# lukifer23/Matrix0

Hardware: AMD Instinct MI355X
Metric: self-play games/sec at 800 sims/move, ResNet-24 53M; 1/2/4/8 MI355X (higher is better)
Workload: dtype f16

## Files before the change

include/m0_engine.h:

```cpp
#ifndef M0_ENGINE_H
#define M0_ENGINE_H

#include <stdint.h>

#ifdef __cplusplus
extern "C" {
#endif

#define M0_OK 0
#define M0_ERR_INVALID (-1)
#define M0_ERR_UNSUPPORTED (-2)
#define M0_ERR_HIP (-3)
#define M0_ERR_STATE (-4)
#define M0_ERR_NONFINITE (-5)

#define M0_POLICY_SIZE 4672
#define M0_PLANES 19

#define M0_ACT_RELU 1
#define M0_ACT_SILU 2
#define M0_ACT_LEAKY 3

#define M0_SSL_PIECE 1
#define M0_SSL_THREAT 2
#define M0_SSL_PIN 4
#define M0_SSL_FORK 8
#define M0_SSL_CONTROL 16

typedef struct m0_net_cfg {
    int planes;
    int channels;
    int blocks;
    int attention;
    int attention_heads;
    int attention_every_k;
    int attention_relbias;
    float attention_unmasked_mix;
    int se;
    float se_ratio;
    int chess_features;
    int piece_square_tables;
    int policy_factor_rank;
    int norm_group;
    int activation;
    int value_activation;
    int preact;
    int self_supervised;
    int ssl_tasks;
    int infer_attention_stride;
} m0_net_cfg;

typedef struct m0_net m0_net;

const char* m0_last_error(void);
const char* m0_version(void);
int m0_device_count(void);

m0_net* m0_net_create(const m0_net_cfg* cfg, int hip_device);
void m0_net_destroy(m0_net* net);
int m0_net_load_weight(m0_net* net, const char* name, const void* data, int dtype, const int64_t* shape, int ndim);
int m0_net_finalize(m0_net* net);
int m0_net_infer(m0_net* net, const float* planes, int B, float* policy, float* value, float* ssl);
int m0_net_ssl_channels(const m0_net* net);
int64_t m0_net_param_count(const m0_net* net);
double m0_net_flops_per_position(const m0_net* net, int with_ssl);
int m0_net_bench_forward(m0_net* net, int B, int iters, int with_ssl, float* ms_per_forward);
int m0_net_profile_enable(m0_net* net, int on);
int m0_net_profile_get(m0_net* net, double* conv_ms, double* conv_flop, int64_t* launches, int reset);
int m0_net_profile_get_tail(m0_net* net, double* tail_ms, int64_t* tail_launches);


typedef struct m0_dist m0_dist;
int m0_dist_unique_id(void* id128);
m0_dist* m0_dist_create(int rank, int world, const void* id128, int hip_device);
void m0_dist_destroy(m0_dist* d);
int m0_dist_rank(const m0_dist* d);
int m0_dist_world(const m0_dist* d);
int m0_net_broadcast_weights(m0_net* net, m0_dist* d, int root);

int m0_encode_fens(int hip_device, const char* const* fens, int n, float* planes, uint8_t* mask, int32_t* nlegal,
                   uint16_t* moves, int32_t* idx);
int m0_encode_fens_nhwc(int hip_device, const char* const* fens, int n, uint16_t* nhwc);
int m0_decode_move_fen(int hip_device, const char* fen, int action_idx, char* uci_out);
int m0_ssl_targets_fens(int hip_device, const char* const* fens, int n, float* out);
int m0_move_to_index_fen(int hip_device, const char* fen, const char* uci, int32_t* idx);

typedef struct m0_selfplay_cfg {
    int num_simulations;
    double cpuct, cpuct_start, cpuct_end;
    int cpuct_plies;
    int use_c_base; double cpuct_c_base, cpuct_c_init;
    double dirichlet_alpha, dirichlet_frac;
    int dirichlet_plies;
    double selection_jitter, fpu_reduction, draw_penalty, virtual_loss;
    int legal_softmax, enable_entropy_noise, no_instant_backtrack, value_from_white;
    int inference_batch_size;
    double playout_random_frac;
    int max_game_len, min_resign_plies, opening_random_plies;
    double resign_threshold; int resign_window, resign_consecutive_bad; double resign_min_entropy, resign_value_margin;
    double temperature_start, temperature_end; int temperature_moves;
    int low_visit_threshold;
    int draw_enabled, draw_min_plies, draw_window, draw_min_unique, draw_halfmove_cap, draw_material_threshold, draw_stalemate;
    int concurrent_games;
    int total_games;
    int first_game_index;
    int arena_nodes;
    uint64_t seed;
    int virtual_loss_active;
    int ssl_in_forward;
    int ssl_targets;
    int record_games;
    int arena_mode;
    double arena_temp;
    int arena_temp_plies;
    int fresh_tree_per_move;
    int tt_merge;
    int raw_legal_priors;
    int max_children;
    double min_child_prior;
    int root_reinfer;
    int eval_cache;
    int eval_cache_entries;
    int tail_split;
} m0_selfplay_cfg;

typedef struct m0_selfplay m0_selfplay;

typedef struct m0_selfplay_stats {
    uint64_t steps, evals, sims, plies, games_finished, games_started;
    double ms_total, ms_net, ms_tree, ms_host;
    uint64_t arena_overflows;
    uint64_t ssl_dropped;
    uint64_t evals_cached;
    int active_games;
    uint64_t rows_tail;
} m0_selfplay_stats;

typedef struct m0_game_record {
    int game_index, moves, resigned, resigner , draw, total_plies ;
    float result;
    float avg_policy_entropy, avg_sims;
    double secs;
    const float* s;
    const float* pi;
    const float* z;
    const uint8_t* legal_mask;
    const float* search_values;
    const uint16_t* played;
    const float* ssl;
    void* owner;
} m0_game_record;

m0_selfplay* m0_selfplay_create(m0_net* net, const m0_selfplay_cfg* cfg);
void m0_selfplay_destroy(m0_selfplay* sp);
int m0_selfplay_step(m0_selfplay* sp, int steps);
int m0_selfplay_stats_get(m0_selfplay* sp, m0_selfplay_stats* out);
int m0_selfplay_poll(m0_selfplay* sp, m0_game_record* out);
void m0_game_record_free(m0_game_record* rec);
int m0_selfplay_running(m0_selfplay* sp);
int m0_selfplay_set_openings(m0_selfplay* sp, const char* const* fens, int n);
int m0_selfplay_ext_select(m0_selfplay* sp, int* rows, float* planes, int max_rows);
int m0_selfplay_ext_expand(m0_selfplay* sp, const float* logits, const float* values, int rows);
int m0_selfplay_last_batch_nhwc(m0_selfplay* sp, uint16_t* nhwc, int max_rows, int* rows);

m0_selfplay* m0_arena_create(m0_net* net_a, m0_net* net_b, const m0_selfplay_cfg* cfg);
m0_selfplay* m0_arena_create_ext(const m0_selfplay_cfg* cfg);
int m0_arena_ext_select(m0_selfplay* sp, int* rows_a, int* rows_b, float* planes_a, float* planes_b, int max_rows);
int m0_arena_ext_expand(m0_selfplay* sp, const float* logits_a, const float* values_a, int rows_a, const float* logits_b,
                        const float* values_b, int rows_b);
int m0_arena_choose_move(const int32_t* visits, int n, double temp, int ply, int temp_plies, double u);
int m0_san_legal_fen(const char* fen, uint16_t* moves, char* san, int* nlegal);
int m0_san_game(const uint16_t* moves, int n, char* out, int cap);
int m0_fen_after(const char* fen, const char* const* ucis, int n, char* fen_out, int cap);

int m0_search_begin(m0_selfplay* sp, int g, const char* fen, int sims, int dirichlet, int game_uid);
int m0_search_select(m0_selfplay* sp, int* rows, float* planes, int max_rows);
int m0_search_expand(m0_selfplay* sp, const float* logits, const float* values, int rows);
int m0_search_result(m0_selfplay* sp, int g, int* nchild, int32_t* child_n, uint16_t* child_mv, int32_t* child_idx,
                     double* child_prior, double* child_q, double* root_q, int* root_n, int* finished);
int m0_search_advance(m0_selfplay* sp, int g, int slot, int sims, int dirichlet);

int m0_sample_move_index(const int32_t* visits, int n, double temperature, double u);
int m0_playout_cap(int sims, double frac, double u);
double m0_temperature_for(int fullmove_number, double t_start, double t_end, int t_moves);
int m0_rules_probe(const m0_selfplay_cfg* cfg, const char* fen, const char* const* ucis, int n, int* flags, float* result);

#ifdef __cplusplus
}
#endif
#endif
```

matrix0_amd/csrc/capi_selfplay.hip:

```cpp
#include <string.h>
#include <algorithm>
#include <memory>
#include "selfplay_engine.h"

using namespace m0;

static void fill_tree_cfg(const m0_selfplay_cfg& c, TreeCfg& t) {
    t.fpu_reduction = c.fpu_reduction; t.draw_penalty = c.draw_penalty; t.virtual_loss = c.virtual_loss;
    t.selection_jitter = c.selection_jitter; t.cpuct = c.cpuct; t.cpuct_start = c.cpuct_start; t.cpuct_end = c.cpuct_end;
    t.cpuct_plies = c.cpuct_plies; t.use_c_base = c.use_c_base; t.cpuct_c_base = c.cpuct_c_base; t.cpuct_c_init = c.cpuct_c_init;
    t.dirichlet_alpha = c.dirichlet_alpha; t.dirichlet_frac = c.dirichlet_frac; t.legal_softmax = c.legal_softmax;
    t.enable_entropy_noise = c.enable_entropy_noise; t.no_instant_backtrack = c.no_instant_backtrack;
    t.virtual_loss_active = c.virtual_loss_active; t.leaves_per_step = c.inference_batch_size;
    t.tt_merge = c.tt_merge; t.raw_legal_priors = c.raw_legal_priors; t.max_children = c.max_children;
    t.min_child_prior = c.min_child_prior;
    t.eval_cache = (c.eval_cache && c.legal_softmax && !c.raw_legal_priors && !c.tt_merge) ? 1 : 0;
}

static void alloc_tree_arenas(m0_selfplay* sp) {
    const m0_selfplay_cfg& c = sp->cfg;
    long want = c.arena_nodes > 0 ? c.arena_nodes : (long)(c.num_simulations * 1.3 + 64) * 96;
    if (want < 4096) want = 4096;
    sp->cap = (int)want;
    const size_t N = (size_t)sp->G * 2 * sp->cap;
    TreeArrays& t = sp->d.t;
    t.cap = sp->cap;
    t.prior = dalloc<double>(sp, N); t.w = dalloc<double>(sp, N); t.q = dalloc<double>(sp, N);
    t.n = dalloc<int>(sp, N); t.vl = dalloc<int>(sp, N); t.cbase = dalloc<int>(sp, N);
    t.nch = dalloc<int16_t>(sp, N); t.mv = dalloc<uint16_t>(sp, N); t.midx = dalloc<uint16_t>(sp, N);
    sp->d.games = dalloc<GameDev>(sp, sp->G);
    const size_t LS = (size_t)sp->L + 1;
    sp->d.samples = dalloc<Sample>(sp, (size_t)sp->G * LS);
    sp->d.paths = dalloc<int>(sp, (size_t)sp->G * LS * M0_MAX_DEPTH);
    sp->d.leaf_moves = dalloc<uint16_t>(sp, (size_t)sp->G * LS * M0_MAX_CHILDREN);
}

static bool alloc_position_tables(m0_selfplay* sp) {
    sp->d.tt_sides = 1;
    if (!sp->cfg.tt_merge) return true;
    const size_t LS = (size_t)sp->L + 1;
    int tc = 1024;
    while (tc < 2 * sp->cap) tc <<= 1;
    sp->d.tt_cap = tc;
    sp->d.tt_sides = sp->cfg.arena_mode ? 2 : 1;
    sp->d.search_nodes = (int)std::min<long>((long)sp->cfg.num_simulations * 48 + 4 * M0_MAX_CHILDREN, (long)sp->cap / 2);
    sp->d.epaths = dalloc<int>(sp, (size_t)sp->G * LS * M0_MAX_DEPTH);
    sp->d.tt_keys = dalloc<uint64_t>(sp, (size_t)sp->G * sp->d.tt_sides * tc);
    sp->d.tt_nodes = dalloc<int>(sp, (size_t)sp->G * sp->d.tt_sides * tc);
    if (sp->d.epaths && sp->d.tt_keys && sp->d.tt_nodes) return true;
    m0_set_error("hipMalloc failed for the position tables (tt_merge): lower concurrent_games or arena_nodes");
    return false;
}

static bool alloc_eval_cache(m0_selfplay* sp) {
    if (!sp->tc.eval_cache) return true;
    const size_t LS = (size_t)sp->L + 1;
    int entries = sp->cfg.eval_cache_entries > 0 ? sp->cfg.eval_cache_entries : 16384;
    int sets = 64;
    while (sets * 4 < entries) sets <<= 1;
    EvalCache& ec = sp->d.ec;
    ec.sets = sets;
    ec.keys = dalloc<uint64_t>(sp, (size_t)sp->G * sets * 4);
    ec.stamps = dalloc<uint32_t>(sp, (size_t)sp->G * sets * 4);
    ec.payload = dalloc<float>(sp, (size_t)sp->G * sets * 4 * M0_EC_WORDS);
    ec.hit_stage = dalloc<float>(sp, (size_t)sp->G * LS * M0_EC_WORDS);
    if (ec.keys && ec.stamps && ec.payload && ec.hit_stage) return true;
    m0_set_error("hipMalloc failed for the evaluation cache: lower eval_cache_entries or concurrent_games");
    return false;
}

static bool alloc_batch_buffers(m0_selfplay* sp) {
    const int nreg = sp->cfg.arena_mode ? 2 : 1;
    sp->d.hist = dalloc<uint64_t>(sp, (size_t)sp->G * M0_HIST_CAP);
    sp->d.results = dalloc<RootResult>(sp, sp->G);
    sp->d.row_counter = dalloc<int>(sp, 4);
    sp->d.x0 = dalloc<_Float16>(sp, (size_t)(nreg * sp->rows_max + 4) * 64 * 32);
    sp->logits_dev = dalloc<float>(sp, (size_t)nreg * sp->rows_max * 4672);
    sp->values_dev = dalloc<float>(sp, (size_t)nreg * sp->rows_max + 4);
    sp->d.net_row_base = sp->rows_max;
    if (sp->cfg.ssl_in_forward && sp->net && sp->net->ssl_channels_total() > 0)
        sp->ssl_dev = dalloc<float>(sp, (size_t)sp->rows_max * sp->net->ssl_channels_total() * 64);
    if (sp->cfg.ssl_targets) {
        sp->ssl_cap = sp->cfg.max_game_len > 0 ? sp->cfg.max_game_len + 1 : 513;
        sp->ssl_pos_dev = dalloc<Pos>(sp, sp->ssl_cap);
        sp->ssl_out_dev = dalloc<float>(sp, (size_t)sp->ssl_cap * 17 * 64);
        if (!sp->ssl_pos_dev || !sp->ssl_out_dev) {
            m0_set_error("hipMalloc failed for the SSL target staging buffers");
            return false;
        }
    }
    sp->ids_dev = dalloc<int>(sp, sp->G);
    sp->slots_dev = dalloc<int>(sp, sp->G);
    sp->d.logits = sp->logits_dev; sp->d.values = sp->values_dev;
    sp->d.G = sp->G; sp->d.L = sp->L;
    return true;
}

static bool make_tail_view(m0_selfplay* sp) {
    if (!(sp->cfg.tail_split && sp->net && !sp->cfg.arena_mode && sp->net->cfg().channels > 256 && sp->net->cfg().channels <= 320 &&
          sp->rows_max >= 2048)) return true;
    if (create_stream_cu_mask_env("M0_TAIL_CU_MASK", &sp->stream_tail) != hipSuccess ||
        hipEventCreateWithFlags(&sp->ev_sel, hipEventDisableTiming) != hipSuccess ||
        hipEventCreateWithFlags(&sp->ev_tail, hipEventDisableTiming) != hipSuccess) {
        m0_set_error("hipStreamCreate / hipEventCreate failed (tail split)");
        return false;
    }
    sp->net_tail = sp->net->shared_view(sp->stream_tail);
    std::string werr;
    sp->half_split = sp->cfg.tail_split == 2;
    if (sp->net_tail->ensure_workspace(sp->half_split ? sp->rows_max / 2 + 1024 : 1023, werr) != M0_OK) {
        m0_set_error("tail split: " + werr);
        return false;
    }
    return true;
}

static bool build_engine(m0_selfplay* sp) {
    alloc_tree_arenas(sp);
    if (!alloc_position_tables(sp) || !alloc_eval_cache(sp) || !alloc_batch_buffers(sp)) return false;
    if (sp->alloc_failed) {
        m0_set_error("hipMalloc failed for the search arenas (lower concurrent_games or arena_nodes)");
        return false;
    }
    sp->hg.assign(sp->G, GameDev());
    for (auto& g : sp->hg) memset(&g, 0, sizeof(GameDev));
    sp->games.assign(sp->G, HostGame());
    sp->hres.resize(sp->G);
    sp->hsamples.resize((size_t)sp->G * (sp->L + 1));
    sp->prev_done.assign(sp->G, 0);
    (void)hipEventCreate(&sp->ev0); (void)hipEventCreate(&sp->ev1); (void)hipEventCreate(&sp->ev2); (void)hipEventCreate(&sp->ev3);
    if (!make_tail_view(sp)) return false;
    std::string err;
    if (sp->net && sp->net->ensure_workspace(sp->rows_max, err) != M0_OK) { m0_set_error(err); return false; }
    if (sp->net && sp->net_b && sp->net_b->ensure_workspace(sp->rows_max, err) != M0_OK) { m0_set_error(err); return false; }
    if (hipStreamSynchronize(sp->stream) != hipSuccess) {
        m0_set_error(std::string("clearing the search arenas failed: ") + hipGetErrorString(hipGetLastError()));
        return false;
    }
    return true;
}

extern "C" {

static m0_selfplay* selfplay_create_impl(m0_net* nh, m0_net* nh_b, const m0_selfplay_cfg* cfg, bool arena = false) {
    if (!cfg) { m0_set_error("cfg is null"); return nullptr; }
    if (cfg->concurrent_games <= 0 || cfg->inference_batch_size <= 0 || cfg->num_simulations <= 0) {
        m0_set_error("concurrent_games, inference_batch_size and num_simulations must be positive");
        return nullptr;
    }
    int ndev = 0;
    if (hipGetDeviceCount(&ndev) != hipSuccess || ndev <= 0) { m0_set_error("no HIP device available (no CPU fallback)"); return nullptr; }
    std::unique_ptr<m0_selfplay, decltype(&m0_selfplay_destroy)> owner(new m0_selfplay(), &m0_selfplay_destroy);
    m0_selfplay* sp = owner.get();
    sp->cfg = *cfg;
    fill_tree_cfg(*cfg, sp->tc);
    sp->nethandle = nh;
    sp->nethandle_b = nh_b;
    sp->net = m0_net_impl(nh);
    sp->net_b = m0_net_impl(nh_b);
    sp->cfg.arena_mode = (nh_b || arena) ? 1 : 0;
    if (sp->cfg.arena_mode) { sp->cfg.eval_cache = 0; sp->tc.eval_cache = 0; }
    sp->device = nh ? m0_net_device(nh) : 0;
    if (nh) forward_gate_join(sp);
    (void)hipSetDevice(sp->device);
    if (nh) sp->stream = m0_net_stream(nh);
    else { (void)hipStreamCreateWithFlags(&sp->stream, hipStreamNonBlocking); sp->own_stream = true; }
    sp->G = cfg->concurrent_games;
    sp->L = cfg->inference_batch_size;
    sp->rows_max = (sp->G * (sp->L + 1) + 3) & ~3;
    memset(&sp->stats, 0, sizeof(sp->stats));
    memset(&sp->d, 0, sizeof(sp->d));
    return build_engine(sp) ? owner.release() : nullptr;
}

m0_selfplay* m0_selfplay_create(m0_net* nh, const m0_selfplay_cfg* cfg) { return selfplay_create_impl(nh, nullptr, cfg); }

m0_selfplay* m0_arena_create(m0_net* net_a, m0_net* net_b, const m0_selfplay_cfg* cfg) {
    if (!net_a || !net_b) { m0_set_error("m0_arena_create needs two networks"); return nullptr; }
    if (m0_net_device(net_a) != m0_net_device(net_b)) { m0_set_error("both networks must live on the same HIP device"); return nullptr; }
    if (cfg && (cfg->ssl_in_forward || cfg->ssl_targets)) { m0_set_error("arena games carry no SSL outputs"); return nullptr; }
    return selfplay_create_impl(net_a, net_b, cfg);
}

m0_selfplay* m0_arena_create_ext(const m0_selfplay_cfg* cfg) {
    if (cfg && (cfg->ssl_in_forward || cfg->ssl_targets)) { m0_set_error("arena games carry no SSL outputs"); return nullptr; }
    return selfplay_create_impl(nullptr, nullptr, cfg, true);
}

void m0_selfplay_destroy(m0_selfplay* sp) {
    if (!sp) return;
    forward_gate_leave(sp);
    (void)hipSetDevice(sp->device);
    if (sp->stream) (void)hipStreamSynchronize(sp->stream);
    if (sp->stream_tail) (void)hipStreamSynchronize(sp->stream_tail);
    delete sp->net_tail;
    if (sp->ev_sel) (void)hipEventDestroy(sp->ev_sel);
    if (sp->ev_tail) (void)hipEventDestroy(sp->ev_tail);
    if (sp->stream_tail) (void)hipStreamDestroy(sp->stream_tail);
    for (void* p : sp->allocs) (void)hipFree(p);
    for (auto& r : sp->done_meta) delete (GameRecordOwner*)r.owner;
    if (sp->ev0) { (void)hipEventDestroy(sp->ev0); (void)hipEventDestroy(sp->ev1); (void)hipEventDestroy(sp->ev2); (void)hipEventDestroy(sp->ev3); }
    if (sp->own_stream && sp->stream) (void)hipStreamDestroy(sp->stream);
    delete sp;
}

int m0_selfplay_set_openings(m0_selfplay* sp, const char* const* fens, int n) {
    if (!sp || n < 0 || (n > 0 && !fens)) { m0_set_error("invalid argument"); return M0_ERR_INVALID; }
    std::lock_guard<std::mutex> lk(sp->mu);
    if (sp->stats.games_started != 0) { m0_set_error("set the opening book before the first step"); return M0_ERR_STATE; }
    std::vector<Pos> book(n);
    for (int i = 0; i < n; ++i)
        if (!fens[i] || parse_fen(fens[i], book[i]) != 0) { m0_set_error(std::string("bad FEN at index ") + std::to_string(i)); return M0_ERR_INVALID; }
    sp->book.swap(book);
    return M0_OK;
}

static int leaf_planes(m0_selfplay* sp, int rows_a, float* planes_a, int rows_b, float* planes_b) {
    if (sync_games_d2h(sp) != 0) { m0_set_error("device sync failed"); return M0_ERR_HIP; }
    (void)hipMemcpy(sp->hsamples.data(), sp->d.samples, sizeof(Sample) * (size_t)sp->G * (sp->L + 1), hipMemcpyDeviceToHost);
    const int base = sp->d.net_row_base;
    for (int g = 0; g < sp->G; ++g) {
        if (!sp->hg[g].active) continue;
        for (int s = 0; s < sp->hg[g].nsamples; ++s) {
            const Sample& smp = sp->hsamples[(size_t)g * (sp->L + 1) + s];
            if (!sample_owns_row(smp.kind) || smp.row < 0) continue;
            if (smp.row < rows_a) encode_planes_f32(smp.pos, planes_a + (size_t)smp.row * 19 * 64);
            else if (smp.row >= base && smp.row < base + rows_b) encode_planes_f32(smp.pos, planes_b + (size_t)(smp.row - base) * 19 * 64);
        }
    }
    return M0_OK;
}

static void upload_eval(m0_selfplay* sp, size_t row_base, const float* logits, const float* values, int rows) {
    if (rows <= 0) return;
    (void)hipMemcpyAsync(sp->logits_dev + row_base * 4672, logits, (size_t)rows * 4672 * 4, hipMemcpyHostToDevice, sp->stream);
    (void)hipMemcpyAsync(sp->values_dev + row_base, values, (size_t)rows * 4, hipMemcpyHostToDevice, sp->stream);
}

static int ext_select_impl(m0_selfplay* sp, int* rows_a, int* rows_b, float* planes_a, float* planes_b, int max_rows) {
    (void)hipSetDevice(sp->device);
    if (sp->ext_pending) { m0_set_error("m0_selfplay_ext_expand outstanding"); return M0_ERR_STATE; }
    if (!planes_a || (sp->cfg.arena_mode && !planes_b) || max_rows < sp->G * (sp->L + 1)) {
        m0_set_error("planes buffer too small: concurrent_games * (inference_batch_size + 1) rows are required");
        return M0_ERR_INVALID;
    }
    int rc = start_first_games(sp);
    if (rc != M0_OK) return rc;
    int r = 0;
    if (run_select(sp, &r) != 0) { m0_set_error(std::string("select failed: ") + hipGetErrorString(hipGetLastError())); return M0_ERR_HIP; }
    const int rb = sp->cfg.arena_mode ? sp->rows2[1] : 0;
    if (r > sp->rows_max || rb > sp->rows_max) { m0_set_error("row counter overflow"); return M0_ERR_STATE; }
    *rows_a = r;
    if (rows_b) *rows_b = rb;
    sp->last_rows = r;
    sp->last_rows_b = rb;
    sp->ext_pending = true;
    if (r + rb > 0) return leaf_planes(sp, r, planes_a, rb, planes_b);
    return M0_OK;
}

static int ext_expand_impl(m0_selfplay* sp, const float* logits_a, const float* values_a, int rows_a, const float* logits_b,
                           const float* values_b, int rows_b) {
    (void)hipSetDevice(sp->device);
    if (!sp->ext_pending) { m0_set_error("no m0_selfplay_ext_select outstanding"); return M0_ERR_STATE; }
    if (rows_a != sp->last_rows || rows_b != sp->last_rows_b) { m0_set_error("rows does not match the last select"); return M0_ERR_INVALID; }
    if ((rows_a > 0 && (!logits_a || !values_a)) || (rows_b > 0 && (!logits_b || !values_b))) { m0_set_error("null argument"); return M0_ERR_INVALID; }
    upload_eval(sp, 0, logits_a, values_a, rows_a);
    upload_eval(sp, (size_t)sp->d.net_row_base, logits_b, values_b, rows_b);
    sp->ext_pending = false;
    std::string err;
    (void)hipEventRecord(sp->ev0, sp->stream); (void)hipEventRecord(sp->ev1, sp->stream);
    int rc = step_back(sp, rows_a + rows_b, now_ms(), err);
    if (rc != M0_OK) m0_set_error(err);
    return rc;
}

int m0_selfplay_ext_select(m0_selfplay* sp, int* rows, float* planes, int max_rows) {
    if (!sp || !rows) { m0_set_error("null argument"); return M0_ERR_INVALID; }
    std::lock_guard<std::mutex> lk(sp->mu);
    if (sp->cfg.arena_mode) { m0_set_error("a match engine has two evaluators: use m0_arena_ext_select"); return M0_ERR_STATE; }
    return ext_select_impl(sp, rows, nullptr, planes, nullptr, max_rows);
}

int m0_selfplay_ext_expand(m0_selfplay* sp, const float* logits, const float* values, int rows) {
    if (!sp) { m0_set_error("null argument"); return M0_ERR_INVALID; }
    std::lock_guard<std::mutex> lk(sp->mu);
    if (sp->cfg.arena_mode) { m0_set_error("a match engine has two evaluators: use m0_arena_ext_expand"); return M0_ERR_STATE; }
    return ext_expand_impl(sp, logits, values, rows, nullptr, nullptr, 0);
}

int m0_arena_ext_select(m0_selfplay* sp, int* rows_a, int* rows_b, float* planes_a, float* planes_b, int max_rows) {
    if (!sp || !rows_a || !rows_b) { m0_set_error("null argument"); return M0_ERR_INVALID; }
    std::lock_guard<std::mutex> lk(sp->mu);
    if (!sp->cfg.arena_mode) { m0_set_error("not a match engine"); return M0_ERR_STATE; }
    return ext_select_impl(sp, rows_a, rows_b, planes_a, planes_b, max_rows);
}

int m0_arena_ext_expand(m0_selfplay* sp, const float* logits_a, const float* values_a, int rows_a, const float* logits_b,
                        const float* values_b, int rows_b) {
    if (!sp) { m0_set_error("null argument"); return M0_ERR_INVALID; }
    std::lock_guard<std::mutex> lk(sp->mu);
    if (!sp->cfg.arena_mode) { m0_set_error("not a match engine"); return M0_ERR_STATE; }
    return ext_expand_impl(sp, logits_a, values_a, rows_a, logits_b, values_b, rows_b);
}

int m0_selfplay_step(m0_selfplay* sp, int steps) {
    if (!sp) { m0_set_error("sp is null"); return M0_ERR_INVALID; }
    std::lock_guard<std::mutex> lk(sp->mu);
    (void)hipSetDevice(sp->device);
    std::string err;
    if (sp->ext_pending) { m0_set_error("m0_selfplay_ext_expand outstanding"); return M0_ERR_STATE; }
    { int rc0 = start_first_games(sp); if (rc0 != M0_OK) return rc0; }
    for (int i = 0; i < steps; ++i) {
        if (sp->stats.active_games == 0 && sp->stats.steps > 0) break;
        int rc = one_step(sp, err);
        if (rc != M0_OK) { m0_set_error(err); return rc; }
    }
    return M0_OK;
}

int m0_selfplay_stats_get(m0_selfplay* sp, m0_selfplay_stats* out) {
    if (!sp || !out) { m0_set_error("null argument"); return M0_ERR_INVALID; }
    std::lock_guard<std::mutex> lk(sp->mu);
    *out = sp->stats;
    return M0_OK;
}

int m0_selfplay_poll(m0_selfplay* sp, m0_game_record* out) {
    if (!sp || !out) { m0_set_error("null argument"); return M0_ERR_INVALID; }
    std::lock_guard<std::mutex> lk(sp->mu);
    if (sp->done_meta.empty()) return 0;
    *out = sp->done_meta.front();
    sp->done_meta.pop_front();
    return 1;
}

void m0_game_record_free(m0_game_record* rec) {
    if (rec && rec->owner) { delete (GameRecordOwner*)rec->owner; rec->owner = nullptr; }
}

int m0_selfplay_running(m0_selfplay* sp) {
    if (!sp) return 0;
    std::lock_guard<std::mutex> lk(sp->mu);
    if (sp->stats.games_started == 0) return 1;
    if (sp->stats.active_games > 0) return 1;
    return (sp->cfg.total_games <= 0 || sp->next_game < sp->cfg.total_games) ? 1 : 0;
}

int m0_search_begin(m0_selfplay* sp, int g, const char* fen, int sims, int dirichlet, int game_uid) {
    if (!sp || !fen || g < 0 || g >= sp->G || sims <= 0) { m0_set_error("invalid argument"); return M0_ERR_INVALID; }
    std::lock_guard<std::mutex> lk(sp->mu);
    (void)hipSetDevice(sp->device);
    Pos p;
    if (parse_fen(fen, p) != 0) { m0_set_error("bad FEN"); return M0_ERR_INVALID; }
    if (sync_games_d2h(sp) != 0) { m0_set_error("device sync failed"); return M0_ERR_HIP; }
    HostGame& hgm = sp->games[g];
    hgm = HostGame();
    hgm.in_use = true; hgm.pos = p; hgm.game_index = game_uid;
    seed_game_dev(sp->hg[g], sp->cfg.seed, game_uid);
    sp->hg[g].evals = 0;
    arm_search(sp, g, p, hgm.win, sims, dirichlet != 0, true);
    std::vector<int> ids{g}, slots{-1};
    if (apply_advances(sp, ids, slots) != 0) { m0_set_error("advance failed"); return M0_ERR_HIP; }
    return M0_OK;
}

int m0_search_select(m0_selfplay* sp, int* rows, float* planes, int max_rows) {
    if (!sp || !rows) { m0_set_error("null argument"); return M0_ERR_INVALID; }
    std::lock_guard<std::mutex> lk(sp->mu);
    (void)hipSetDevice(sp->device);
    int r = 0;
    if (run_select(sp, &r) != 0) { m0_set_error(std::string("select failed: ") + hipGetErrorString(hipGetLastError())); return M0_ERR_HIP; }
    *rows = r;
    sp->last_rows = r;
    if (planes && r > 0) {
        if (r > max_rows) { m0_set_error("planes buffer too small"); return M0_ERR_INVALID; }
        return leaf_planes(sp, r, planes, 0, nullptr);
    }
    return M0_OK;
}

int m0_search_expand(m0_selfplay* sp, const float* logits, const float* values, int rows) {
    if (!sp) { m0_set_error("null argument"); return M0_ERR_INVALID; }
    std::lock_guard<std::mutex> lk(sp->mu);
    (void)hipSetDevice(sp->device);
    if (rows != sp->last_rows || rows > sp->rows_max) { m0_set_error("rows does not match the last select"); return M0_ERR_INVALID; }
    if (rows > 0 && (!logits || !values)) { m0_set_error("null argument"); return M0_ERR_INVALID; }
    upload_eval(sp, 0, logits, values, rows);
    if (launch_expand(sp->d, sp->tc, sp->stream) != hipSuccess) { m0_set_error("expand launch failed"); return M0_ERR_HIP; }
    if (sync_games_d2h(sp) != 0) { m0_set_error(std::string("expand failed: ") + hipGetErrorString(hipGetLastError())); return M0_ERR_HIP; }
    sp->stats.evals += (uint64_t)rows;
    return M0_OK;
}

int m0_search_result(m0_selfplay* sp, int g, int* nchild, int32_t* child_n, uint16_t* child_mv, int32_t* child_idx,
                     double* child_prior, double* child_q, double* root_q, int* root_n, int* finished) {
    if (!sp || g < 0 || g >= sp->G) { m0_set_error("invalid argument"); return M0_ERR_INVALID; }
    std::lock_guard<std::mutex> lk(sp->mu);
    (void)hipSetDevice(sp->device);
    if (finished) *finished = sp->hg[g].finished;
    if (!sp->hg[g].finished) { if (nchild) *nchild = 0; return M0_OK; }
    (void)hipMemcpy(&sp->hres[g], sp->d.results + g, sizeof(RootResult), hipMemcpyDeviceToHost);
    const RootResult& R = sp->hres[g];
    if (nchild) *nchild = R.nchild;
    for (int i = 0; i < R.nchild; ++i) {
        if (child_n) child_n[i] = R.child_n[i];
        if (child_mv) child_mv[i] = R.child_mv[i];
        if (child_idx) child_idx[i] = R.child_idx[i];
        if (child_prior) child_prior[i] = R.child_prior[i];
        if (child_q) child_q[i] = R.child_q[i];
    }
    if (root_q) *root_q = R.root_n > 0 ? R.root_q : sp->hg[g].root_v;
    if (root_n) *root_n = R.root_n;
    return M0_OK;
}

int m0_search_advance(m0_selfplay* sp, int g, int slot, int sims, int dirichlet) {
    if (!sp || g < 0 || g >= sp->G || sims <= 0) { m0_set_error("invalid argument"); return M0_ERR_INVALID; }
    std::lock_guard<std::mutex> lk(sp->mu);
    (void)hipSetDevice(sp->device);
    if (sync_games_d2h(sp) != 0) { m0_set_error("device sync failed"); return M0_ERR_HIP; }
    if (!sp->hg[g].finished) { m0_set_error("search not finished"); return M0_ERR_STATE; }
    (void)hipMemcpy(&sp->hres[g], sp->d.results + g, sizeof(RootResult), hipMemcpyDeviceToHost);
    const RootResult& R = sp->hres[g];
    if (slot < 0 || slot >= R.nchild) { m0_set_error("child slot out of range"); return M0_ERR_INVALID; }
    HostGame& hgm = sp->games[g];
    hgm.play(R.child_mv[slot]);
    const bool fresh = sp->cfg.fresh_tree_per_move || sp->cfg.tt_merge;
    arm_search(sp, g, hgm.pos, hgm.win, sims, dirichlet != 0, fresh);
    std::vector<int> ids{g}, slots{fresh ? -1 : slot};
    if (apply_advances(sp, ids, slots) != 0) { m0_set_error("advance failed"); return M0_ERR_HIP; }
    return M0_OK;
}

int m0_selfplay_last_batch_nhwc(m0_selfplay* sp, uint16_t* out, int max_rows, int* rows) {
    if (!sp || !out || !rows) { m0_set_error("null argument"); return M0_ERR_INVALID; }
    std::lock_guard<std::mutex> lk(sp->mu);
    (void)hipSetDevice(sp->device);
    const int r = sp->last_rows;
    if (r > max_rows) { m0_set_error("output buffer too small"); return M0_ERR_INVALID; }
    *rows = r;
    if (r > 0) {
        if (hipMemcpyAsync(out, sp->d.x0, (size_t)r * 64 * 32 * 2, hipMemcpyDeviceToHost, sp->stream) != hipSuccess ||
            hipStreamSynchronize(sp->stream) != hipSuccess) { m0_set_error("copy failed"); return M0_ERR_HIP; }
    }
    return M0_OK;
}

}
```

matrix0_amd/csrc/net.h:

```cpp
#pragma once
#include <hip/hip_runtime.h>
#include <stdint.h>
#include <map>
#include <string>
#include <vector>
#include "../../include/m0_engine.h"
#include "net_kernels.h"

struct HostTensor {
    std::vector<float> data;
    std::vector<int64_t> shape;
};

struct PackedGemm {
    _Float16* w = nullptr;
    float* bias = nullptr;
    int taps = 1, Cin = 0, N = 0;
    bool pp = false;
};

struct NormParams {
    float* gamma = nullptr;
    float* beta = nullptr;
};

struct ResBlockW {
    PackedGemm conv1, conv2;
    NormParams bn1, bn2;
    float *se_w1 = nullptr, *se_b1 = nullptr, *se_w2 = nullptr, *se_b2 = nullptr;
    void* se_wf = nullptr;
    int se_hidden = 0;
};

struct AttnW {
    PackedGemm qkv, proj;
    NormParams ln;
    float* rel_bias = nullptr;
    void* blk_w = nullptr;
    _Float16* blk_bias = nullptr;
};

struct TowerLayer {
    int kind;
    int index;
    bool skip;
    int next_bn1 = -1;
};

struct SslHeadW {
    PackedGemm c0, c1;
    NormParams n;
    int out_ch = 0;
};

struct ConvNormOpts {
    const float* posenc = nullptr;
    const _Float16* res = nullptr;
    const NormParams* next_bn1 = nullptr;
};

class Net {
public:
    explicit Net(const m0_net_cfg& cfg, int device, hipStream_t stream);
    ~Net();
    Net* shared_view(hipStream_t stream) const;
    static const char* check_supported(const m0_net_cfg& cfg);
    int load(const char* name, const void* data, int dtype, const int64_t* shape, int ndim, std::string& err);
    int finalize(std::string& err);
    bool ready() const { return finalized_; }
    const std::vector<void*>& device_buffers() const { return dev_allocs_; }
    const std::vector<size_t>& device_buffer_bytes() const { return dev_sizes_; }

    int forward(const float* planes_dev, const _Float16* nhwc_dev, int B, float* logits_dev, float* value_dev,
                float* ssl_dev, hipStream_t st, std::string& err);
    int ensure_workspace(int B, std::string& err);
    int ssl_channels_total() const;
    const m0_net_cfg& cfg() const { return cfg_; }
    size_t param_count() const { return nparams_; }
    double flops_per_position(bool with_ssl) const;
    _Float16* input_nhwc() { return X0_; }
    void set_profile(bool on) { profile_ = on; }
    void harvest_profile();
    double prof_conv_ms() const { return prof_ms_; }
    double prof_conv_flop() const { return prof_flop_; }
    long prof_conv_launches() const { return prof_launches_; }
    void reset_profile() { prof_ms_ = 0; prof_flop_ = 0; prof_launches_ = 0; prof_tail_ms_ = 0; prof_tail_launches_ = 0; }
    double prof_tail_ms() const { return prof_tail_ms_; }
    long prof_tail_launches() const { return prof_tail_launches_; }

private:
    m0_net_cfg cfg_;
    int device_;
    hipStream_t stream_ = nullptr;
    struct Switches { bool fuse_tail = true, fuse_attn = true; } sw_;
    struct Plan {
        bool fuse_tail = false;
        bool fuse_attn = false;
        bool gn_small = false;
        int act = 0, vact = 0;
        int first_bn1 = -1;
    } plan_;
    bool finalized_ = false;
    size_t nparams_ = 0;
    std::map<std::string, HostTensor> sd_;
    std::vector<void*> dev_allocs_;
    std::vector<size_t> dev_sizes_;
    std::vector<void*> ws_allocs_;

    int C_ = 0, Cs_ = 0 ;
    int Cp_ = 0;
    PackedGemm stem_;
    NormParams stem_n_;
    float* posenc_ = nullptr;
    PackedGemm pst_, inter_;
    NormParams pst_n_, inter_n_;
    std::vector<ResBlockW> res_;
    std::vector<AttnW> att_;
    std::vector<TowerLayer> tower_;
    PackedGemm ph_conv_, pfc1_, pfc2_;
    PackedGemm hv_;
    NormParams hv_n_;
    NormParams ph_n_;
    float logit_scale_ = 1.f;
    PackedGemm vh0_, vh3_, vfc1_, vfc2_, vgate_, vfc3_;
    NormParams vh1_n_, vh4_n_;
    std::vector<SslHeadW> ssl_;
    uint64_t* mask_dev_ = nullptr;

    bool profile_ = false;
    std::vector<hipEvent_t> pev_;
    std::vector<double> pflop_;
    std::vector<char> ptail_;
    size_t pev_used_ = 0;
    double prof_ms_ = 0, prof_flop_ = 0, prof_tail_ms_ = 0;
    long prof_launches_ = 0, prof_tail_launches_ = 0;

    int wsB_ = 0, wsM_ = 0;
    _Float16 *X0_ = nullptr, *XA_ = nullptr, *XB_ = nullptr, *T1_ = nullptr, *T2_ = nullptr, *QKV_ = nullptr,
             *O_ = nullptr, *AA_ = nullptr;
    float *S1_ = nullptr, *S2_ = nullptr, *G_ = nullptr;
    _Float16 *PH_ = nullptr, *PH2_ = nullptr, *VH_ = nullptr, *VH2_ = nullptr, *F1_ = nullptr, *F2_ = nullptr,
             *F3_ = nullptr, *F4_ = nullptr, *SH_ = nullptr, *SH2_ = nullptr, *SO_ = nullptr;
    float* VAL_ = nullptr;
    float* SPK_ = nullptr;

    const HostTensor* get(const std::string& k, std::string& err);
    int pack_gemm(PackedGemm& g, const std::string& wkey, const std::string& bkey, int taps, int Cin_real,
                  int Cin_pad, int N_real, int N_pad, int k_perm_ch, std::string& err, int qkv_heads = 0,
                  int qkv_heads_pad = 0);
    int pack_attn_block(AttnW& a, const std::string& prefix, std::string& err);
    int pack_chess_features(std::string& err);
    int pack_se(ResBlockW& r, const std::string& prefix, std::string& err);
    int pack_attn(AttnW& a, bool skip, const std::string& prefix, std::string& err);
    void upload_attn_mask();
    int pack_joint_head(std::string& err);
    int pack_ssl_heads(std::string& err);
    void make_plan();
    int upload_norm(NormParams& n, const std::string& prefix, int C_real, int C_pad, std::string& err);
    float* upload_f32(const std::vector<float>& v);
    void* dalloc(size_t bytes, bool ws);
    const NormParams* bn1(int res_index) const { return res_index < 0 ? nullptr : &res_[res_index].bn1; }
    template <class Launch>
    hipError_t profiled(bool on, hipStream_t st, double flop, bool tail, Launch&& launch);
    hipError_t run_gemm(const PackedGemm& g, GemmArgs a, hipStream_t st);
    hipError_t conv_norm_act(const PackedGemm& g, const NormParams& n, const _Float16* in, _Float16* out, _Float16* scratch,
                             int Mrows, hipStream_t st, const ConvNormOpts& o = ConvNormOpts());
    hipError_t se_gate(const ResBlockW& r, const float* stats, int boards, hipStream_t st);
};
```

matrix0_amd/csrc/net.hip:

```cpp
#include "net.h"
#include <math.h>
#include <string.h>
#include <algorithm>
#include <stdlib.h>

static inline int ceil_to(int v, int m) { return (v + m - 1) / m * m; }

static const char* kSslNames[5] = {"piece", "threat", "pin", "fork", "control"};
static const int kSslOut[5] = {13, 1, 1, 1, 3};

const char* Net::check_supported(const m0_net_cfg& c) {
    if (!c.norm_group) return "HIP path supports norm='group' only (BatchNorm configs are not built)";
    if (!c.preact) return "HIP path supports preact=true only";
    if (c.channels % 32 != 0 || c.channels < 32 || c.channels > 384) return "channels must be a multiple of 32 in [32,384]";
    if (c.planes < 1 || c.planes > 32) return "planes must be in [1,32]";
    if (c.attention && (c.attention_heads <= 0 || c.channels % c.attention_heads != 0 ||
                        c.channels / c.attention_heads != 16))
        return "attention head_dim (channels/attention_heads) must be 16";
    if (c.activation != M0_ACT_SILU && c.activation != M0_ACT_RELU) return "activation must be silu or relu";
    if (c.blocks < 1) return "blocks must be >= 1";
    if (c.policy_factor_rank < 0) return "policy_factor_rank must be >= 0";
    if (c.self_supervised && c.ssl_tasks && (c.channels / 2) % 16 != 0) return "ssl heads need channels/2 % 16 == 0";
    return nullptr;
}
// ... 171 lines not shown
    (void)hipMemcpy(a.blk_w, buf.data(), buf.size() * 2, hipMemcpyHostToDevice);
    std::vector<_Float16> bb((size_t)20 * 2 * 64 * 32, (_Float16)0.f);
    if (cfg_.attention_relbias) {
        const HostTensor* rb = get(prefix + ".rel_bias", err); if (!rb) return M0_ERR_INVALID;
        for (int h = 0; h < Hr; ++h)
            for (int qt = 0; qt < 2; ++qt)
                for (int lane = 0; lane < 64; ++lane)
                    for (int e = 0; e < 32; ++e) {
                        const int kt = e >> 4, r = e & 15;
                        const int q = qt * 32 + (lane & 31), key = kt * 32 + 8 * (r >> 2) + 4 * (lane >> 5) + (r & 3);
                        bb[(((size_t)h * 2 + qt) * 64 + lane) * 32 + e] =
                            (_Float16)(rb->data[((size_t)h * 64 + q) * 64 + key] * 1.44269504088896f);
                    }
    }
    a.blk_bias = (_Float16*)dalloc(bb.size() * 2, false);
    if (!a.blk_bias) { err = "hipMalloc failed"; return M0_ERR_HIP; }
    (void)hipMemcpy(a.blk_bias, bb.data(), bb.size() * 2, hipMemcpyHostToDevice);
    return M0_OK;
}

int Net::upload_norm(NormParams& n, const std::string& prefix, int C_real, int C_pad, std::string& err) {
    const HostTensor* g = get(prefix + ".weight", err);
    if (!g) return M0_ERR_INVALID;
    const HostTensor* b = get(prefix + ".bias", err);
    if (!b) return M0_ERR_INVALID;
    if ((int)g->data.size() != C_real || (int)b->data.size() != C_real) { err = "shape mismatch for " + prefix; return M0_ERR_INVALID; }
    nparams_ += 2 * (size_t)C_real;
    std::vector<float> gp(C_pad, 0.f), bp(C_pad, 0.f);
    std::copy(g->data.begin(), g->data.end(), gp.begin());
    std::copy(b->data.begin(), b->data.end(), bp.begin());
    n.gamma = upload_f32(gp);
    n.beta = upload_f32(bp);
    return M0_OK;
}

#define TRY(x) do { int rc_ = (x); if (rc_ != M0_OK) return rc_; } while (0)

int Net::pack_chess_features(std::string& err) {
    const int C = C_, P = Cp_;
    const HostTensor* pe = get("chess_features.position_encoding", err);
    if (!pe) return M0_ERR_INVALID;
    if ((int)pe->data.size() != C * 64) { err = "shape mismatch for position_encoding"; return M0_ERR_INVALID; }
    nparams_ += pe->data.size();
    std::vector<float> t((size_t)64 * P, 0.f);
    for (int c = 0; c < C; ++c)
        for (int n = 0; n < 64; ++n) t[(size_t)n * P + c] = pe->data[(size_t)c * 64 + n];
    posenc_ = upload_f32(t);
    if (cfg_.piece_square_tables) {
        TRY(pack_gemm(pst_, "chess_features.pst_conv.weight", "", 1, C, P, C, P, 0, err));
        TRY(upload_norm(pst_n_, "chess_features.pst_norm", C, P, err));
    }
    TRY(pack_gemm(inter_, "chess_features.interaction_conv.weight", "", 9, C, P, C, P, 0, err));
    return upload_norm(inter_n_, "chess_features.interaction_norm", C, P, err);
}

int Net::pack_se(ResBlockW& r, const std::string& p, std::string& err) {
    const int C = C_, P = Cp_;
    const int hd = std::max(8, (int)(C * cfg_.se_ratio));
    r.se_hidden = hd;
    const HostTensor* w1 = get(p + ".se_fc1.weight", err); if (!w1) return M0_ERR_INVALID;
    const HostTensor* b1 = get(p + ".se_fc1.bias", err); if (!b1) return M0_ERR_INVALID;
    const HostTensor* w2 = get(p + ".se_fc2.weight", err); if (!w2) return M0_ERR_INVALID;
    const HostTensor* b2 = get(p + ".se_fc2.bias", err); if (!b2) return M0_ERR_INVALID;
    if ((int)w1->data.size() != hd * C || (int)w2->data.size() != hd * C || (int)b1->data.size() != hd ||
        (int)b2->data.size() != C) { err = "shape mismatch for " + p + ".se_*"; return M0_ERR_INVALID; }
    nparams_ += (size_t)2 * hd * C + hd + C;
    std::vector<float> w1t((size_t)P * hd, 0.f);
    for (int j = 0; j < hd; ++j)
        for (int c = 0; c < C; ++c) w1t[(size_t)c * hd + j] = w1->data[(size_t)j * C + c];
    r.se_w1 = upload_f32(w1t);
    r.se_b1 = upload_f32(b1->data);
    std::vector<float> w2t((size_t)hd * P, 0.f);
    for (int c = 0; c < C; ++c)
        for (int j = 0; j < hd; ++j) w2t[(size_t)j * P + c] = w2->data[(size_t)c * hd + j];
    r.se_w2 = upload_f32(w2t);
    if (P == 320 && hd <= TAIL_SE_HMAX) {
        const int NT1 = (hd + 15) / 16, KS2 = (hd + 31) / 32;
        std::vector<_Float16> wf((size_t)(10 * NT1 + 20 * KS2) * 512, (_Float16)0.f);
        for (int nt = 0; nt < NT1; ++nt)
            for (int ks = 0; ks < 10; ++ks)
                for (int l = 0; l < 64; ++l)
                    for (int e = 0; e < 8; ++e) {
                        const int c = 32 * ks + 8 * (l >> 4) + e, j = 16 * nt + (l & 15);
                        if (j < hd) wf[((size_t)(nt * 10 + ks) * 64 + l) * 8 + e] = (_Float16)w1t[(size_t)c * hd + j];
                    }
        for (int nt = 0; nt < 20; ++nt)
            for (int ks = 0; ks < KS2; ++ks)
                for (int l = 0; l < 64; ++l)
                    for (int e = 0; e < 8; ++e) {
                        const int j = 32 * ks + 8 * (l >> 4) + e, c = 16 * nt + (l & 15);
                        if (j < hd) wf[((size_t)(10 * NT1 + nt * KS2 + ks) * 64 + l) * 8 + e] = (_Float16)w2t[(size_t)j * P + c];
                    }
        r.se_wf = dalloc(wf.size() * 2, false);
        if (!r.se_wf) { err = "hipMalloc failed"; return M0_ERR_HIP; }
        (void)hipMemcpy(r.se_wf, wf.data(), wf.size() * 2, hipMemcpyHostToDevice);
    }
    std::vector<float> b2p(P, 0.f);
    std::copy(b2->data.begin(), b2->data.end(), b2p.begin());
    r.se_b2 = upload_f32(b2p);
    return M0_OK;
}

int Net::pack_attn(AttnW& a, bool skip, const std::string& p, std::string& err) {
    const int C = C_, P = Cp_;
    if (skip) {
        for (const char* k : {".qkv.weight", ".proj.weight", ".norm.weight", ".norm.bias", ".rel_bias"}) {
            auto it = sd_.find(p + k);
            if (it != sd_.end()) nparams_ += it->second.data.size();
        }
        return M0_OK;
    }
    TRY(pack_gemm(a.qkv, p + ".qkv.weight", "", 1, C, P, 3 * C, 3 * P, 0, err, P != C ? cfg_.attention_heads : 0, P / 16));
    TRY(pack_gemm(a.proj, p + ".proj.weight", "", 1, C, P, C, P, 0, err));
    TRY(upload_norm(a.ln, p + ".norm", C, P, err));
    if (P == 320) TRY(pack_attn_block(a, p, err));
    if (cfg_.attention_relbias) {
        const HostTensor* rb = get(p + ".rel_bias", err); if (!rb) return M0_ERR_INVALID;
        if ((int)rb->data.size() != cfg_.attention_heads * 4096) { err = "shape mismatch for rel_bias"; return M0_ERR_INVALID; }
        nparams_ += rb->data.size();
        std::vector<float> rbs((size_t)(P / 16) * 4096, 0.f);
        for (size_t i = 0; i < rb->data.size(); ++i) rbs[i] = rb->data[i] * 1.44269504088896f;
        a.rel_bias = upload_f32(rbs);
    }
    return M0_OK;
}

void Net::upload_attn_mask() {
    std::vector<uint64_t> m(64, 0);
    for (int i = 0; i < 64; ++i)
        for (int j = 0; j < 64; ++j) {
            int dr = i / 8 - j / 8, dc = i % 8 - j % 8;
            int adr = abs(dr), adc = abs(dc);
            bool vis = dr == 0 || dc == 0 || adr == adc || (adr == 2 && adc == 1) || (adr == 1 && adc == 2) ||
                       (adr <= 1 && adc <= 1);
            if (vis) m[i] |= (1ull << j);
        }
    mask_dev_ = (uint64_t*)dalloc(64 * 8, false);
    (void)hipMemcpy(mask_dev_, m.data(), 64 * 8, hipMemcpyHostToDevice);
}

int Net::pack_joint_head(std::string& err) {
    const int nch = Cp_ / 32;
    std::vector<_Float16> a((size_t)nch * 64 * 32), b((size_t)nch * 128 * 32), c((size_t)nch * 192 * 32);
    (void)hipMemcpy(a.data(), ph_conv_.w, a.size() * 2, hipMemcpyDeviceToHost);
    (void)hipMemcpy(b.data(), vh0_.w, b.size() * 2, hipMemcpyDeviceToHost);
    for (int ch = 0; ch < nch; ++ch) {
        std::copy(a.begin() + (size_t)ch * 64 * 32, a.begin() + (size_t)(ch + 1) * 64 * 32, c.begin() + (size_t)ch * 192 * 32);
        std::copy(b.begin() + (size_t)ch * 128 * 32, b.begin() + (size_t)(ch + 1) * 128 * 32, c.begin() + ((size_t)ch * 192 + 64) * 32);
    }
    hv_.w = (_Float16*)dalloc(c.size() * 2, false);
    if (!hv_.w) { err = "hipMalloc failed"; return M0_ERR_HIP; }
    (void)hipMemcpy(hv_.w, c.data(), c.size() * 2, hipMemcpyHostToDevice);
    hv_.taps = 1; hv_.Cin = Cp_; hv_.N = 192; hv_.pp = false; hv_.bias = nullptr;
    std::vector<float> g(192), be(192);
    (void)hipMemcpy(g.data(), ph_n_.gamma, 64 * 4, hipMemcpyDeviceToHost);
    (void)hipMemcpy(g.data() + 64, vh1_n_.gamma, 128 * 4, hipMemcpyDeviceToHost);
    (void)hipMemcpy(be.data(), ph_n_.beta, 64 * 4, hipMemcpyDeviceToHost);
    (void)hipMemcpy(be.data() + 64, vh1_n_.beta, 128 * 4, hipMemcpyDeviceToHost);
    hv_n_.gamma = upload_f32(g); hv_n_.beta = upload_f32(be);
    if (!hv_n_.gamma || !hv_n_.beta) { err = "hipMalloc failed"; return M0_ERR_HIP; }
    return M0_OK;
}

int Net::pack_ssl_heads(std::string& err) {
    for (int t = 0; t < 5; ++t) {
        if (!(cfg_.ssl_tasks & (1 << t))) continue;
        SslHeadW h;
        h.out_ch = kSslOut[t];
        std::string p = std::string("ssl_heads.") + kSslNames[t];
        TRY(pack_gemm(h.c0, p + ".0.weight", "", 1, C_, Cp_, C_ / 2, Cs_, 0, err));
        TRY(upload_norm(h.n, p + ".1", C_ / 2, Cs_, err));
        TRY(pack_gemm(h.c1, p + ".3.weight", "", 1, C_ / 2, Cs_, h.out_ch, 32, 0, err));
        ssl_.push_back(h);
    }
    return M0_OK;
}

void Net::make_plan() {
    const bool big = conv_gemm_tile_n(Cp_, Cp_) == 320;
    plan_.fuse_tail = big && sw_.fuse_tail &&
                      (!cfg_.se || (res_[0].se_hidden <= TAIL_SE_HMAX && res_[0].se_hidden % 4 == 0));
    plan_.fuse_attn = big && sw_.fuse_attn;
    plan_.gn_small = Cp_ % 64 == 0;
    plan_.act = cfg_.activation == M0_ACT_SILU ? ACT_SILU : ACT_RELU;
    plan_.vact = cfg_.value_activation == M0_ACT_SILU ? ACT_SILU : (cfg_.value_activation == M0_ACT_LEAKY ? ACT_LEAKY : ACT_RELU);
    int next = -1;
    for (size_t i = tower_.size(); i-- > 0;) {
        TowerLayer& L = tower_[i];
        if (L.kind == 1 && L.skip) continue;
        L.next_bn1 = next;
        next = L.kind == 0 ? L.index : -1;
    }
    plan_.first_bn1 = next;
}

int Net::finalize(std::string& err) {
    if (finalized_) return M0_OK;
    if (hipSetDevice(device_) != hipSuccess) { err = "hipSetDevice failed"; return M0_ERR_HIP; }
    const int C = C_, P = Cp_;
    nparams_ = 0;
    TRY(pack_gemm(stem_, "stem.0.weight", "", 9, cfg_.planes, 32, C, P, 0, err));
    TRY(upload_norm(stem_n_, "stem.1", C, P, err));
    if (cfg_.chess_features) TRY(pack_chess_features(err));
    int ti = 0;
    for (auto& L : tower_) {
        std::string p = "tower." + std::to_string(ti++);
        if (L.kind == 0) {
            ResBlockW& r = res_[L.index];
            TRY(pack_gemm(r.conv1, p + ".conv1.weight", "", 9, C, P, C, P, 0, err));
            TRY(pack_gemm(r.conv2, p + ".conv2.weight", "", 9, C, P, C, P, 0, err));
            TRY(upload_norm(r.bn1, p + ".bn1", C, P, err));
            TRY(upload_norm(r.bn2, p + ".bn2", C, P, err));
            if (cfg_.se) TRY(pack_se(r, p, err));
        } else {
            TRY(pack_attn(att_[L.index], L.skip, p, err));
        }
    }
    upload_attn_mask();
    TRY(pack_gemm(ph_conv_, "policy_head.0.weight", "", 1, C, P, 64, 64, 0, err));
    TRY(upload_norm(ph_n_, "policy_head.1", 64, 64, err));
    if (cfg_.policy_factor_rank > 0) {
        int r = cfg_.policy_factor_rank, rp = ceil_to(r, 32);
        TRY(pack_gemm(pfc1_, "policy_fc1.weight", "policy_fc1.bias", 1, 4096, 4096, r, rp, 64, err));
        TRY(pack_gemm(pfc2_, "policy_fc2.weight", "policy_fc2.bias", 1, r, rp, M0_POLICY_SIZE, M0_POLICY_SIZE, 0, err));
    } else {
        TRY(pack_gemm(pfc1_, "policy_fc.weight", "policy_fc.bias", 1, 4096, 4096, M0_POLICY_SIZE, M0_POLICY_SIZE, 64, err));
    }
    {
        const HostTensor* ls = get("_policy_logit_scale_raw", err); if (!ls) return M0_ERR_INVALID;
        nparams_ += 1;
        double raw = ls->data.empty() ? 0.0 : ls->data[0];
        double sp = raw > 20.0 ? raw : log1p(exp(raw));
        logit_scale_ = (float)std::min(5.0, sp + 1e-3);
    }
    TRY(pack_gemm(vh0_, "value_head.0.weight", "", 1, C, P, 128, 128, 0, err));
    TRY(upload_norm(vh1_n_, "value_head.1", 128, 128, err));
    TRY(pack_gemm(vh3_, "value_head.3.weight", "", 1, 128, 128, 128, 128, 0, err));
    TRY(upload_norm(vh4_n_, "value_head.4", 128, 128, err));
    TRY(pack_joint_head(err));
    const int h1 = 2 * C, h1p = ceil_to(h1, 32), h2 = C, h2p = ceil_to(C, 32);
    TRY(pack_gemm(vfc1_, "value_fc1.weight", "value_fc1.bias", 1, 8192, 8192, h1, h1p, 128, err));
    TRY(pack_gemm(vfc2_, "value_fc2.weight", "value_fc2.bias", 1, h1, h1p, h2, h2p, 0, err));
    TRY(pack_gemm(vgate_, "value_gate.0.weight", "value_gate.0.bias", 1, h2, h2p, h2, h2p, 0, err));
    TRY(pack_gemm(vfc3_, "value_fc3.weight", "value_fc3.bias", 1, h2, h2p, 1, 32, 0, err));
    if (cfg_.self_supervised) TRY(pack_ssl_heads(err));
    sd_.clear();
    (void)hipDeviceSynchronize();
    make_plan();
    finalized_ = true;
    return M0_OK;
}

int Net::ssl_channels_total() const {
    int n = 0;
    for (auto& h : ssl_) n += h.out_ch;
    return n;
}

double Net::flops_per_position(bool with_ssl) const {
    const double C = C_;
    double mac = 64.0 * cfg_.planes * 9 * C;
    if (cfg_.chess_features) mac += 64.0 * C * C * (cfg_.piece_square_tables ? 1 : 0) + 64.0 * C * C * 9;
    for (auto& L : tower_) {
        if (L.kind == 0) {
            mac += 2 * 64.0 * C * C * 9;
            if (cfg_.se) mac += 2.0 * C * res_[L.index].se_hidden;
        } else if (!L.skip) {
            mac += 64.0 * C * 3 * C + 64.0 * C * C;
            double nb = (cfg_.attention_unmasked_mix > 0.f && cfg_.attention_unmasked_mix < 1.f) ? 2.0 : 1.0;
            mac += 64.0 * 64.0 * C * (1.0 + nb);
        }
    }
    mac += 64.0 * C * 64;
    if (cfg_.policy_factor_rank > 0) mac += 4096.0 * cfg_.policy_factor_rank + (double)cfg_.policy_factor_rank * M0_POLICY_SIZE;
    else mac += 4096.0 * M0_POLICY_SIZE;
    mac += 64.0 * C * 128 + 64.0 * 128 * 128 + 8192.0 * 2 * C + 2.0 * C * C + C * C + C;
    if (with_ssl) for (auto& h : ssl_) mac += 64.0 * C * (C / 2) + 64.0 * (C / 2) * h.out_ch;
    return 2.0 * mac;
}

int Net::ensure_workspace(int B, std::string& err) {
    const int Bp = ceil_to(B, 4);
    const int Mfc = ceil_to(B, 256);
    if (Bp <= wsB_ && Mfc <= wsM_) return M0_OK;
    if (hipSetDevice(device_) != hipSuccess) { err = "hipSetDevice failed"; return M0_ERR_HIP; }
    (void)hipDeviceSynchronize();
    for (void* p : ws_allocs_) (void)hipFree(p);
    ws_allocs_.clear();
    const size_t C = Cp_;
    const size_t nb = Bp, nh = std::max(Bp, Mfc);
    const size_t Cst = std::max<size_t>(C, 128);
    auto H = [&](size_t elems) { return (_Float16*)dalloc(elems * 2, true); };
    auto F = [&](size_t elems) { return (float*)dalloc(elems * 4, true); };
    X0_ = H(nb * 64 * 32);
    XA_ = H(nb * 64 * C); XB_ = H(nb * 64 * C); T1_ = H(nb * 64 * C); T2_ = H(nb * 64 * C); AA_ = H(nb * 64 * C);
    QKV_ = H(nb * 64 * 3 * C); O_ = H(nb * 64 * C);
    S1_ = F(nb * Cst * 2); S2_ = F(nb * Cst * 2); G_ = F(nb * Cst);
    PH_ = H(nh * 64 * 64); PH2_ = H(nh * 64 * 64);
    VH_ = H(nh * 64 * 128); VH2_ = H(nh * 64 * 128);
    const size_t rp = cfg_.policy_factor_rank > 0 ? ceil_to(cfg_.policy_factor_rank, 32) : 32;
    F1_ = H((size_t)Mfc * rp);
    F2_ = H((size_t)Mfc * ceil_to(2 * C_, 32)); F3_ = H((size_t)Mfc * ceil_to(C_, 32)); F4_ = H((size_t)Mfc * ceil_to(C_, 32));
    SH_ = H(nb * 64 * Cs_); SH2_ = H(nb * 64 * Cs_); SO_ = H(nb * 64 * 32);
    VAL_ = F((size_t)Mfc * 32);
    SPK_ = F((size_t)8 * Mfc * ceil_to(2 * C_, 32));
    if (!X0_ || !XA_ || !XB_ || !AA_ || !T1_ || !T2_ || !QKV_ || !O_ || !S1_ || !S2_ || !PH_ || !PH2_ || !VH_ ||
        !VH2_ || !F1_ || !F2_ || !F3_ || !F4_ || !SH_ || !SH2_ || !SO_ || !VAL_ || !SPK_) {
        err = "workspace hipMalloc failed";
        wsB_ = wsM_ = 0;
        return M0_ERR_HIP;
    }
    if (hipStreamSynchronize(stream_) != hipSuccess || hipGetLastError() != hipSuccess) {
        err = "workspace clear failed"; wsB_ = wsM_ = 0; return M0_ERR_HIP;
    }
    wsB_ = Bp; wsM_ = Mfc;
    return M0_OK;
}

static GemmArgs gemm_args(const PackedGemm& g, const _Float16* in, void* out, int Mrows, int epi_act = ACT_NONE) {
    GemmArgs a;
    memset(&a, 0, sizeof(a));
    a.in = in; a.w = g.w; a.out = out; a.bias = g.bias;
    a.Mrows = Mrows; a.Mvalid = Mrows; a.Cin = g.Cin; a.N = g.N; a.Npad = g.N; a.ldo = g.N;
    a.epi_act = epi_act; a.out_scale = 1.f; a.w_pp = g.pp ? 1 : 0;
    return a;
}

static EwArgs ew_args(const _Float16* t, _Float16* y, int C, int act) {
    EwArgs e;
    memset(&e, 0, sizeof(e));
    e.t = t; e.y = y; e.C = C; e.act = act;
    return e;
}
static void ew_next_bn1(EwArgs& e, const NormParams* next_bn1, _Float16* y2) {
    if (next_bn1) { e.y2 = y2; e.gn2_gamma = next_bn1->gamma; e.gn2_beta = next_bn1->beta; }
}

static double conv3x3_flop(const PackedGemm& g, int rows) { return 2.0 * (double)rows * (double)g.N * (double)g.Cin * 9.0; }

template <class Launch>
hipError_t Net::profiled(bool on, hipStream_t st, double flop, bool tail, Launch&& launch) {
    if (!on) return launch();
    if (pev_used_ + 2 > pev_.size()) {
        for (int i = 0; i < 2; ++i) { hipEvent_t e; if (hipEventCreate(&e) != hipSuccess) return hipErrorOutOfMemory; pev_.push_back(e); }
    }
    (void)hipEventRecord(pev_[pev_used_], st);
    hipError_t rc = launch();
    (void)hipEventRecord(pev_[pev_used_ + 1], st);
    pev_used_ += 2;
    pflop_.push_back(flop);
    ptail_.push_back(tail ? 1 : 0);
    return rc;
}

hipError_t Net::run_gemm(const PackedGemm& g, GemmArgs a, hipStream_t st) {
    const bool big = conv_gemm_tile_n(g.Cin, g.N) == 320;
    const bool splitk = g.taps == 1 && big && g.Cin >= 4096 && (g.Cin >> 6) % 8 == 0 && !a.gn_gamma && !a.mul && !a.out_stats &&
                        !a.out_f32 && a.out_scale == 1.f && SPK_ != nullptr && (size_t)g.N <= (size_t)ceil_to(2 * C_, 32) &&
                        a.Mrows <= wsM_;
    return profiled(profile_ && g.taps == 9 && big, st, conv3x3_flop(g, a.Mvalid), false, [&]() -> hipError_t {
        if (!splitk) return launch_conv_gemm(a, g.taps, st);
        _Float16* out = (_Float16*)a.out;
        const int act = a.epi_act;
        a.out = SPK_; a.bias = nullptr; a.epi_act = ACT_NONE; a.out_f32 = 1; a.ksplit = 8;
        hipError_t rc = launch_conv_gemm(a, g.taps, st);
        return rc != hipSuccess ? rc : launch_splitk_reduce(SPK_, 8, a.Mrows, g.N, g.bias, act, out, st);
    });
}

hipError_t Net::se_gate(const ResBlockW& r, const float* stats, int boards, hipStream_t st) {
    SeGateArgs g;
    g.t_stats = stats; g.w1 = r.se_w1; g.b1 = r.se_b1; g.w2 = r.se_w2; g.b2 = r.se_b2;
    g.gate = G_; g.B = boards; g.C = Cp_; g.hidden = r.se_hidden; g.act = plan_.act;
    return launch_se_gate(g, st);
}

hipError_t Net::conv_norm_act(const PackedGemm& g, const NormParams& n, const _Float16* in, _Float16* out, _Float16* scratch,
                              int Mrows, hipStream_t st, const ConvNormOpts& o) {
    const bool big = conv_gemm_tile_n(g.Cin, g.N) == 320;
    GemmArgs a = gemm_args(g, in, out, Mrows);
    if (big && o.res && plan_.fuse_tail) {
        a.epi_act = plan_.act; a.res = o.res; a.pre_gamma = n.gamma; a.pre_beta = n.beta;
        if (o.next_bn1) { a.y2 = AA_; a.gn_gamma = o.next_bn1->gamma; a.gn_beta = o.next_bn1->beta; }
        return launch_conv_gemm(a, g.taps, st);
    }
    const bool epilogue = big ? g.taps == 9
                              : plan_.gn_small && (g.taps == 9 ? g.Cin == 32 : g.N == 32 || g.N == 64 || g.N == 128 || g.N == 160);
    if (epilogue && !o.res && !o.next_bn1) {
        a.gn_gamma = n.gamma; a.gn_beta = n.beta; a.epi_act = plan_.act; a.posenc = o.posenc;
        return run_gemm(g, a, st);
    }
    a.out = scratch; a.out_stats = S1_;
    hipError_t rc = run_gemm(g, a, st);
    if (rc != hipSuccess) return rc;
    EwArgs e = ew_args(scratch, out, g.N, plan_.act);
    e.t_stats = S1_; e.gn_gamma = n.gamma; e.gn_beta = n.beta; e.res = o.res; e.posenc = o.posenc;
    ew_next_bn1(e, o.next_bn1, AA_);
    return launch_ew_board(e, Mrows / 64, st);
}

void Net::harvest_profile() {
    for (size_t i = 0; i + 1 < pev_used_; i += 2) {
        float ms = 0.f;
        if (hipEventElapsedTime(&ms, pev_[i], pev_[i + 1]) == hipSuccess) {
            prof_ms_ += ms; prof_flop_ += pflop_[i / 2]; prof_launches_++;
            if (ptail_[i / 2]) { prof_tail_ms_ += ms; prof_tail_launches_++; }
        }
    }
    pev_used_ = 0;
    pflop_.clear();
    ptail_.clear();
}

#define KCHK(x)                                                                           \
    do {                                                                                  \
        hipError_t e_ = (x);                                                              \
        if (e_ != hipSuccess) {                                                           \
            err = std::string("kernel launch failed: ") + #x + ": " + hipGetErrorString(e_); \
            return M0_ERR_HIP;                                                            \
        }                                                                                 \
    } while (0)

int Net::forward(const float* planes_dev, const _Float16* nhwc_dev, int B, float* logits_dev, float* value_dev,
                 float* ssl_dev, hipStream_t st, std::string& err) {
    if (!finalized_) { err = "weights not finalized"; return M0_ERR_STATE; }
    if (B <= 0) { err = "batch must be positive"; return M0_ERR_INVALID; }
    TRY(ensure_workspace(B, err));
    const int Bp = ceil_to(B, 4);
    const int Mc = Bp * 64;
    const int Mfc = ceil_to(B, 256);
    const int act = plan_.act, vact = plan_.vact;
    const int C = Cp_;

    const _Float16* x0 = nhwc_dev;
    if (!x0) {
        if (!planes_dev) { err = "no input"; return M0_ERR_INVALID; }
        KCHK(launch_planes_to_nhwc(planes_dev, X0_, B, cfg_.planes, st));
        x0 = X0_;
    }
    _Float16* xa = XA_;
    _Float16* xb = XB_;
    const NormParams* first_bn1 = bn1(plan_.first_bn1);
    ConvNormOpts so;
    if (cfg_.chess_features) so.posenc = posenc_; else so.next_bn1 = first_bn1;
    KCHK(conv_norm_act(stem_, stem_n_, x0, xa, T1_, Mc, st, so));
    if (cfg_.chess_features) {
        if (cfg_.piece_square_tables) {
            ConvNormOpts po;
            po.res = xa;
            KCHK(conv_norm_act(pst_, pst_n_, xa, xb, T1_, Mc, st, po));
            std::swap(xa, xb);
        }
        ConvNormOpts io;
        io.res = xa; io.next_bn1 = first_bn1;
        KCHK(conv_norm_act(inter_, inter_n_, xa, xb, T1_, Mc, st, io));
        std::swap(xa, xb);
    }
    for (const TowerLayer& L : tower_) {
        const NormParams* next_bn1 = bn1(L.next_bn1);
        if (L.kind == 0) {
            const ResBlockW& r = res_[L.index];
            KCHK(conv_norm_act(r.conv1, r.bn2, AA_, T1_, T2_, Mc, st));
            if (plan_.fuse_tail) {
                GemmArgs a = gemm_args(r.conv2, T1_, xb, Mc, act);
                a.res = xa;
                if (next_bn1) { a.y2 = AA_; a.gn_gamma = next_bn1->gamma; a.gn_beta = next_bn1->beta; }
                if (cfg_.se) { a.se_w1 = r.se_w1; a.se_b1 = r.se_b1; a.se_w2 = r.se_w2; a.se_b2 = r.se_b2; a.se_hidden = r.se_hidden;
                               a.se_wf = r.se_wf; }
                KCHK(profiled(profile_, st, conv3x3_flop(r.conv2, Mc), true, [&] { return launch_conv_gemm(a, 9, st); }));
            } else {
                GemmArgs a = gemm_args(r.conv2, T1_, T2_, Mc);
                a.out_stats = S2_;
                KCHK(run_gemm(r.conv2, a, st));
                EwArgs e = ew_args(T2_, xb, C, act);
                e.t_stats = S2_; e.res = xa;
                if (cfg_.se) { KCHK(se_gate(r, S2_, Bp, st)); e.gate = G_; }
                ew_next_bn1(e, next_bn1, AA_);
                KCHK(launch_ew_board(e, Bp, st));
            }
        } else {
            if (L.skip) continue;
            const AttnW& w = att_[L.index];
            const float inv_sqrt_d = 1.f / sqrtf((float)(C_ / cfg_.attention_heads));
            if (plan_.fuse_attn && w.blk_w != nullptr) {
                AttnBlockArgs ab;
                memset(&ab, 0, sizeof(ab));
                ab.x = xa; ab.wpack = w.blk_w; ab.bias = w.blk_bias; ab.mask = mask_dev_;
                ab.ln_g = w.ln.gamma; ab.ln_b = w.ln.beta; ab.y = xb;
                if (next_bn1) { ab.y2 = AA_; ab.gn2_gamma = next_bn1->gamma; ab.gn2_beta = next_bn1->beta; }
                ab.B = Bp; ab.ln_count = C_; ab.act = act; ab.mix = cfg_.attention_unmasked_mix; ab.inv_sqrt_d = inv_sqrt_d;
                KCHK(launch_attn_block(ab, st));
            } else {
                KCHK(run_gemm(w.qkv, gemm_args(w.qkv, xa, QKV_, Mc), st));
                AttnArgs aa;
                aa.qkv = QKV_; aa.rel_bias = w.rel_bias; aa.mask = mask_dev_; aa.o = O_;
                aa.B = Bp; aa.H = C / 16; aa.C = C; aa.mix = cfg_.attention_unmasked_mix;
                aa.inv_sqrt_d = inv_sqrt_d;
                KCHK(launch_attn_core(aa, st));
                KCHK(run_gemm(w.proj, gemm_args(w.proj, O_, T1_, Mc), st));
                EwArgs e = ew_args(T1_, xb, C, act);
                e.res = xa; e.ln_g = w.ln.gamma; e.ln_b = w.ln.beta; e.ln_count = C_;
                ew_next_bn1(e, next_bn1, AA_);
                KCHK(launch_ew_board(e, Bp, st));
            }
        }
        std::swap(xa, xb);
    }
    const bool joint = plan_.gn_small;
    if (joint) {
        GemmArgs a = gemm_args(hv_, xa, PH2_, Mc, act);
        a.gn_gamma = hv_n_.gamma; a.gn_beta = hv_n_.beta;
        a.ldo = 64; a.out2 = VH2_; a.ldo2 = 128; a.nsplit = 64;
        KCHK(launch_conv_gemm(a, 1, st));
    } else {
        KCHK(conv_norm_act(ph_conv_, ph_n_, xa, PH2_, PH_, Mc, st));
    }
    const bool factored = cfg_.policy_factor_rank > 0;
    if (factored) KCHK(run_gemm(pfc1_, gemm_args(pfc1_, PH2_, F1_, Mfc, ACT_RELU), st));
    const PackedGemm& plast = factored ? pfc2_ : pfc1_;
    GemmArgs pl = gemm_args(plast, factored ? F1_ : PH2_, logits_dev, Mfc);
    pl.Mvalid = B; pl.out_f32 = 1; pl.out_scale = logit_scale_;
    KCHK(run_gemm(plast, pl, st));
    if (!joint) KCHK(conv_norm_act(vh0_, vh1_n_, xa, VH2_, VH_, Mc, st));
    _Float16* vflat = joint ? VH_ : VH2_;
    KCHK(conv_norm_act(vh3_, vh4_n_, VH2_, vflat, VH_, Mc, st));
    KCHK(run_gemm(vfc1_, gemm_args(vfc1_, vflat, F2_, Mfc, vact), st));
    KCHK(run_gemm(vfc2_, gemm_args(vfc2_, F2_, F3_, Mfc, vact), st));
    GemmArgs vg = gemm_args(vgate_, F3_, F4_, Mfc, ACT_SIGMOID);
    vg.mul = F3_;
    KCHK(run_gemm(vgate_, vg, st));
    GemmArgs v3 = gemm_args(vfc3_, F4_, VAL_, Mfc, ACT_TANH);
    v3.out_f32 = 1;
    KCHK(run_gemm(vfc3_, v3, st));
    KCHK(hipMemcpy2DAsync(value_dev, 4, VAL_, 32 * 4, 4, B, hipMemcpyDeviceToDevice, st));
    if (ssl_dev && !ssl_.empty()) {
        const int ctot = ssl_channels_total();
        int coff = 0;
        for (auto& h : ssl_) {
            KCHK(conv_norm_act(h.c0, h.n, xa, SH2_, SH_, Mc, st));
            KCHK(run_gemm(h.c1, gemm_args(h.c1, SH2_, SO_, Mc), st));
            KCHK(launch_nhwc_to_nchw_f32(SO_, ssl_dev, B, 32, h.out_ch, ctot, coff, st));
            coff += h.out_ch;
        }
    }
    return M0_OK;
}
```

matrix0_amd/csrc/net_kernels.h:

```cpp
#pragma once
#include <hip/hip_runtime.h>
#include <stdint.h>

enum { ACT_NONE = 0, ACT_RELU = 1, ACT_SILU = 2, ACT_LEAKY = 3, ACT_SIGMOID = 4, ACT_TANH = 5 };

constexpr int TAIL_SE_HMAX = 96;

struct GemmArgs {
    const _Float16* in;
    const _Float16* w;
    void* out;
    const float* gn_gamma;
    const float* gn_beta;
    const float* bias;
    const _Float16* mul;
    float* out_stats;
    int Mrows;
    int Mvalid;
    int Cin;
    int N;
    int Npad;
    int ldo;
    int epi_act;
    int out_f32;
    float out_scale;
    int ksplit;
    int w_pp;
    const _Float16* res;
    const float* pre_gamma;
    const float* pre_beta;
    _Float16* y2;
    const float* se_w1;
    const float* se_b1;
    const float* se_w2;
    const float* se_b2;
    int se_hidden;
    const void* se_wf;
    const float* posenc;
    void* out2;
    int ldo2;
    int nsplit;
};

struct EwArgs {
    const _Float16* t;
    const float* t_stats;
    const float* gn_gamma;
    const float* gn_beta;
    const float* gate;
    const _Float16* res;
    const float* posenc;
    const float* ln_g;
    const float* ln_b;
    int ln_count;
    _Float16* y;
    float* out_stats;
    _Float16* y2;
    const float* gn2_gamma;
    const float* gn2_beta;
    int C;
    int act;
};

struct SeGateArgs {
    const float* t_stats;
    const float* w1;
    const float* b1;
    const float* w2;
    const float* b2;
    float* gate;
    int B, C, hidden, act;
};

struct AttnArgs {
    const _Float16* qkv;
    const float* rel_bias;
    const uint64_t* mask;
    _Float16* o;
    int B, H, C;
    float mix;
    float inv_sqrt_d;
};

struct AttnBlockArgs {
    const _Float16* x;
    const void* wpack;
    const _Float16* bias;
    const uint64_t* mask;
    const float* ln_g;
    const float* ln_b;
    const float* gn2_gamma;
    const float* gn2_beta;
    _Float16* y;
    _Float16* y2;
    int B;
    int ln_count;
    int act;
    float mix;
    float inv_sqrt_d;
};
hipError_t launch_attn_block(const AttnBlockArgs& a, hipStream_t st);
hipError_t launch_splitk_reduce(const float* part, int splits, int M, int N, const float* bias, int act, _Float16* out,
                                hipStream_t st);
size_t attn_block_pack_bytes();

hipError_t launch_conv_gemm(const GemmArgs& a, int taps, hipStream_t st);
int conv_gemm_tile_n(int Cin, int Npad);
int conv_gemm_kc(int Cin, int Npad);
hipError_t launch_ew_board(const EwArgs& a, int boards, hipStream_t st);
hipError_t launch_se_gate(const SeGateArgs& a, hipStream_t st);
hipError_t launch_attn_core(const AttnArgs& a, hipStream_t st);
hipError_t launch_planes_to_nhwc(const float* x, void* y, int B, int P, hipStream_t st);
hipError_t launch_nhwc_to_nchw_f32(const void* x, float* y, int B, int ld, int n, int ctot, int coff, hipStream_t st);
```

matrix0_amd/csrc/net_kernels.hip:

```cpp
#include "kernel_common.h"
#include "conv_epilogue.h"

template <int TAPS, int WN, int NT, int KC, int EPI = 0, int ACT = 0>
__global__ __launch_bounds__(256 * WN) void conv_gemm_kernel(GemmArgs a) {
    constexpr int NB = WN * NT * 32;
    constexpr int NTHR = 256 * WN;
    constexpr int AST = KC + 8;
    constexpr int APIX = (TAPS == 9) ? 100 : 64;
    constexpr int A_ELEMS = 4 * APIX * AST;
    constexpr int W_ELEMS = NB * AST;
    constexpr int A_PIECES = 4 * 64 * KC / 8;
    constexpr int W_PIECES = NB * KC / 8;
    constexpr int A_PER = (A_PIECES + NTHR - 1) / NTHR;
    constexpr int W_PER = (W_PIECES + NTHR - 1) / NTHR;
    constexpr int K8 = KC / 8;

    extern __shared__ __attribute__((aligned(16))) char smem[];
    _Float16* A_lds = reinterpret_cast<_Float16*>(smem);
    _Float16* W_lds = A_lds + A_ELEMS;

    const int tid = threadIdx.x;
    const int lane = tid & 63;
    const int wave = tid >> 6;
    const int wm = wave % 4;
    const int wn = wave / 4;
    const int m0 = blockIdx.x * 256;
    const int n0 = blockIdx.y * NB;
    const int Cin = a.Cin;
    const int nchunk = Cin / KC;
    const int Npad = a.Npad;

    if (TAPS == 9) {
        for (int i = tid; i < A_ELEMS / 8; i += NTHR)
            reinterpret_cast<uint4*>(A_lds)[i] = make_uint4(0, 0, 0, 0);
    }
    __syncthreads();

    float16v acc[2][NT];
    static_for<0, 2>([&](auto mi) __attribute__((always_inline)) {
        static_for<0, NT>([&](auto ni) __attribute__((always_inline)) {
            acc[decltype(mi)::value][decltype(ni)::value] = float16v{0.f, 0.f, 0.f, 0.f, 0.f, 0.f, 0.f, 0.f,
                                                                      0.f, 0.f, 0.f, 0.f, 0.f, 0.f, 0.f, 0.f};
        });
    });

    int apix[2];
#pragma unroll
    for (int mi = 0; mi < 2; ++mi) {
        int px = mi * 32 + (lane & 31);
        if (TAPS == 9) apix[mi] = wm * 100 + ((px >> 3) + 1) * 10 + (px & 7) + 1;
        else apix[mi] = wm * 64 + px;
    }
    const int khalf = 8 * (lane >> 5);

    uint4 areg[A_PER];
    uint4 wreg[W_PER];

    auto load_A = [&](int chunk) {
#pragma unroll
        for (int i = 0; i < A_PER; ++i) {
            int p = tid + i * NTHR;
            if (A_PIECES % NTHR == 0 || p < A_PIECES) {
                int row = p / K8, c8 = p % K8;
                areg[i] = *reinterpret_cast<const uint4*>(a.in + (size_t)(m0 + row) * Cin + chunk * KC + c8 * 8);
            }
        }
    };
    auto store_A = [&](int chunk) {
#pragma unroll
        for (int i = 0; i < A_PER; ++i) {
            int p = tid + i * NTHR;
            if (A_PIECES % NTHR == 0 || p < A_PIECES) {
                int row = p / K8, c8 = p % K8;
                int b = row >> 6, px = row & 63;
                uint4 v = areg[i];
                int pix = (TAPS == 9) ? (b * 100 + ((px >> 3) + 1) * 10 + (px & 7) + 1) : row;
                *reinterpret_cast<uint4*>(A_lds + pix * AST + c8 * 8) = v;
            }
        }
    };
    auto load_W = [&](int step) {
        int chunk = step / TAPS, tap = step % TAPS;
        const _Float16* src = a.w + ((size_t)(tap * nchunk + chunk) * Npad + n0) * KC;
#pragma unroll
        for (int i = 0; i < W_PER; ++i) {
            int p = tid + i * NTHR;
            if (W_PIECES % NTHR == 0 || p < W_PIECES)
                wreg[i] = *reinterpret_cast<const uint4*>(src + (size_t)p * 8);
        }
    };
    auto store_W = [&](int buf) {
#pragma unroll
        for (int i = 0; i < W_PER; ++i) {
            int p = tid + i * NTHR;
            if (W_PIECES % NTHR == 0 || p < W_PIECES) {
                int n = p / K8, k8 = p % K8;
                *reinterpret_cast<uint4*>(W_lds + buf * W_ELEMS + n * AST + k8 * 8) = wreg[i];
            }
        }
    };

    const int nsteps = nchunk * TAPS;
    load_A(0);
    load_W(0);
    for (int s = 0; s < nsteps; ++s) {
        const int chunk = s / TAPS, tap = s % TAPS;
        if (tap == 0) {
            if (s > 0) __syncthreads();
            store_A(chunk);
        }
        store_W(s & 1);
        __syncthreads();
        if (s + 1 < nsteps) {
            load_W(s + 1);
            if ((s + 1) % TAPS == 0) load_A((s + 1) / TAPS);
        }
        const int tapoff = (TAPS == 9) ? ((tap / 3 - 1) * 10 + (tap % 3 - 1)) : 0;
        const _Float16* Wb = W_lds + (s & 1) * W_ELEMS + (wn * NT * 32 + (lane & 31)) * AST + khalf;
        static_for<0, KC / 16>([&](auto kk_) __attribute__((always_inline)) {
            constexpr int kk = decltype(kk_)::value;
            half8 af0 = *reinterpret_cast<const half8*>(A_lds + (apix[0] + tapoff) * AST + kk * 16 + khalf);
            half8 af1 = *reinterpret_cast<const half8*>(A_lds + (apix[1] + tapoff) * AST + kk * 16 + khalf);
            static_for<0, NT>([&](auto ni_) __attribute__((always_inline)) {
                constexpr int ni = decltype(ni_)::value;
                half8 bf = *reinterpret_cast<const half8*>(Wb + ni * 32 * AST + kk * 16);
                acc[0][ni] = __builtin_amdgcn_mfma_f32_32x32x16_f16(af0, bf, acc[0][ni], 0, 0, 0);
                acc[1][ni] = __builtin_amdgcn_mfma_f32_32x32x16_f16(af1, bf, acc[1][ni], 0, 0, 0);
            });
        });
    }

    if constexpr (EPI == 1) {
        __syncthreads();
        char* lds_wave = smem + wave * (64 * 64 * NT);
        const int cb = n0 + wn * NT * 32;
        const int r31 = lane & 31, half = lane >> 5;
        GemmArgs o = a;
        int lc = cb;
        if (a.out2 != nullptr && cb >= a.nsplit) { o.out = a.out2; o.ldo = a.ldo2; lc = cb - a.nsplit; }
        o.out = reinterpret_cast<_Float16*>(o.out) + lc;
        char* wbase = conv_stage_base<NT>(lds_wave, lane);
        static_for<0, NT>([&](auto ni_) __attribute__((always_inline)) {
            constexpr int ni = decltype(ni_)::value;
            const int col = cb + ni * 32 + r31;
            float s = 0.f, ss = 0.f;
            static_for<0, 2>([&](auto mi_) __attribute__((always_inline)) {
                const float16v av = acc[decltype(mi_)::value][ni];
                static_for<0, 16>([&](auto r_) __attribute__((always_inline)) { const float v = av[decltype(r_)::value]; s += v; ss += v * v; });
            });
#pragma unroll
            for (int o2 = 1; o2 <= 8; o2 <<= 1) { s += __shfl_xor(s, o2); ss += __shfl_xor(ss, o2); }
            s += __shfl_xor(s, 32); ss += __shfl_xor(ss, 32);
            const float mean = s * (1.f / 1024.f);
            float var = ss * (1.f / 1024.f) - mean * mean;
            var = var > 0.f ? var : 0.f;
            const float g = rsqrtf(var + 1e-5f) * a.gn_gamma[col];
            const float sh = a.gn_beta[col] - mean * g;
            static_for<0, 2>([&](auto mi_) __attribute__((always_inline)) {
                constexpr int mi = decltype(mi_)::value;
                float v[16];
                static_for<0, 16>([&](auto r_) __attribute__((always_inline)) {
                    constexpr int r = decltype(r_)::value;
                    v[r] = act_fast<ACT>(acc[mi][ni][r] * g + sh);
                });
                if (a.posenc != nullptr) {
                    static_for<0, 16>([&](auto r_) __attribute__((always_inline)) {
                        constexpr int r = decltype(r_)::value;
                        const int sq = mi * 32 + (r & 3) + 8 * (r >> 2) + 4 * half;
                        v[r] += a.posenc[(size_t)sq * a.N + col];
                    });
                }
                conv_stage_tile<NT, mi, ni>(v, wbase, lane);
            });
        });
        conv_stage_flush<NT>(o, lds_wave, m0, 0, wm, 0, lane);
        return;
    }
    const int ldo = a.ldo;
    const int rowbase = m0 + wm * 64 + 4 * (lane >> 5);
    const int colbase = n0 + wn * NT * 32 + (lane & 31);
    const int epi_act = a.epi_act;
    const float oscale = a.out_scale;
    const bool has_mul = a.mul != nullptr;
    const bool f32out = a.out_f32 != 0;
    const bool want_stats = a.out_stats != nullptr;
    static_for<0, NT>([&](auto ni_) __attribute__((always_inline)) {
        constexpr int ni = decltype(ni_)::value;
        const int col = colbase + ni * 32;
        const float bias = a.bias != nullptr ? a.bias[col] : 0.f;
        float s = 0.f, ss = 0.f;
        static_for<0, 2>([&](auto mi_) __attribute__((always_inline)) {
            constexpr int mi = decltype(mi_)::value;
            const float16v av = acc[mi][ni];
            static_for<0, 16>([&](auto r_) __attribute__((always_inline)) {
                constexpr int r = decltype(r_)::value;
                const int row = rowbase + mi * 32 + (r & 3) + 8 * (r >> 2);
                float v = av[r] + bias;
                if (epi_act != ACT_NONE) v = act_apply(v, epi_act);
                if (has_mul) v *= (float)a.mul[(size_t)row * ldo + col];
                v *= oscale;
                s += v; ss += v * v;
                if (row < a.Mvalid) {
                    if (f32out) reinterpret_cast<float*>(a.out)[(size_t)row * ldo + col] = v;
                    else reinterpret_cast<_Float16*>(a.out)[(size_t)row * ldo + col] = (_Float16)v;
                }
            });
        });
        if (want_stats) {
            s += __shfl_xor(s, 32);
            ss += __shfl_xor(ss, 32);
            if (lane < 32) {
                float* st = a.out_stats + ((size_t)(m0 / 64 + wm) * a.N + col) * 2;
                st[0] = s; st[1] = ss;
            }
        }
    });
}


template <int TAPS, int WN, int NT, int KC>
static size_t conv_gemm_lds(int Cin) {
    constexpr int NB = WN * NT * 32;
    constexpr int AST = KC + 8;
    constexpr int APIX = (TAPS == 9) ? 100 : 64;
    (void)Cin;
    const size_t main_loop = (size_t)(4 * APIX * AST + 2 * NB * AST) * 2 + 64;
    const size_t staging = (size_t)WN * 4 * 64 * 64 * NT;
    return main_loop > staging ? main_loop : staging;
}

template <int TAPS, int WN, int NT, int KC, int EPI = 0, int ACT = 0>
static hipError_t launch_conv_gemm_t(const GemmArgs& a, hipStream_t st) {
    constexpr int NB = WN * NT * 32;
    size_t lds = conv_gemm_lds<TAPS, WN, NT, KC>(a.Cin);
    static DeviceOnce once;
    hipError_t e = once.run([] {
        return hipFuncSetAttribute(reinterpret_cast<const void*>(&conv_gemm_kernel<TAPS, WN, NT, KC, EPI, ACT>),
                                   hipFuncAttributeMaxDynamicSharedMemorySize, 160 * 1024);
    });
    if (e != hipSuccess) return e;
    dim3 grid(a.Mrows / 256, a.Npad / NB);
    hipLaunchKernelGGL((conv_gemm_kernel<TAPS, WN, NT, KC, EPI, ACT>), grid, dim3(256 * WN), lds, st, a);
    return hipGetLastError();
}
template <int ACT>
static hipError_t launch_conv_gemm_gn(const GemmArgs& a, int taps, hipStream_t st) {
    if (a.bias != nullptr || a.mul != nullptr || a.out_stats != nullptr || a.out_f32 || a.out_scale != 1.f || a.Npad != a.N)
        return hipErrorInvalidValue;
    if (taps == 9) return a.Npad % 64 == 0 && a.out2 == nullptr ? launch_conv_gemm_t<9, 1, 2, 32, 1, ACT>(a, st) : hipErrorInvalidValue;
    if (a.posenc != nullptr) return hipErrorInvalidValue;
    if (a.out2 != nullptr) return a.Npad == 192 && a.nsplit == 64 ? launch_conv_gemm_t<1, 3, 2, 32, 1, ACT>(a, st) : hipErrorInvalidValue;
    if (a.Npad == 160) return launch_conv_gemm_t<1, 1, 5, 32, 1, ACT>(a, st);
    if (a.Npad == 128) return launch_conv_gemm_t<1, 2, 2, 32, 1, ACT>(a, st);
    if (a.Npad == 64) return launch_conv_gemm_t<1, 1, 2, 32, 1, ACT>(a, st);
    if (a.Npad == 32) return launch_conv_gemm_t<1, 1, 1, 32, 1, ACT>(a, st);
    return hipErrorInvalidValue;
}

hipError_t launch_conv_big(const GemmArgs& a, int taps, hipStream_t st);
hipError_t launch_conv_zs(const GemmArgs& a, hipStream_t st);

int conv_gemm_tile_n(int Cin, int Npad) {
    return (Npad % 320 == 0 && Cin % 64 == 0) ? 320 : 32;
}
int conv_gemm_kc(int Cin, int Npad) {
    return (Npad % 320 == 0 && Cin % 64 == 0) ? 64 : 32;
}

hipError_t launch_conv_gemm(const GemmArgs& a, int taps, hipStream_t st) {
    if (a.Mrows % 256 != 0 || a.Cin % 32 != 0 || a.Npad % 32 != 0) return hipErrorInvalidValue;
    const bool big = conv_gemm_tile_n(a.Cin, a.Npad) == 320;
    if (a.gn_gamma != nullptr && !big) {
        if (a.epi_act == ACT_SILU) return launch_conv_gemm_gn<ACT_SILU>(a, taps, st);
        if (a.epi_act == ACT_RELU) return launch_conv_gemm_gn<ACT_RELU>(a, taps, st);
        return hipErrorInvalidValue;
    }
    if (taps == 9) {
        if (big) {
            if (!a.w_pp) return hipErrorInvalidValue;
            return launch_conv_zs(a, st);
        }
        return launch_conv_gemm_t<9, 1, 1, 32>(a, st);
    } else if (taps == 1) {
        if (big) return a.w_pp ? hipErrorInvalidValue : launch_conv_big(a, 1, st);
        if (a.Mrows / 256 >= 256 && a.Npad % 64 == 0) return launch_conv_gemm_t<1, 1, 2, 32>(a, st);
        return launch_conv_gemm_t<1, 1, 1, 32>(a, st);
    }
    return hipErrorInvalidValue;
}

__global__ __launch_bounds__(768) void ew_board_kernel(EwArgs a) {
    extern __shared__ __attribute__((aligned(16))) char smem[];
    const int C = a.C, NC = C >> 3;
    float* sc = reinterpret_cast<float*>(smem);
    float* sh = sc + C;
    float* tot = sh + C;
    float* rowbuf = tot + 2 * C;
    float* red = rowbuf + 128;
    const int tid = threadIdx.x, lane = tid & 63, wave = tid >> 6;
    const int nthr = blockDim.x, nw = nthr >> 6;
    const int chunk = tid % NC, sg = tid / NC;
    const int c0 = chunk * 8;
    const int b = blockIdx.x;
    const _Float16* t = a.t + (size_t)b * 64 * C + (size_t)(sg * 4) * C + c0;
    const _Float16* res = a.res ? a.res + (size_t)b * 64 * C + (size_t)(sg * 4) * C + c0 : nullptr;
    const float* tst = a.t_stats ? a.t_stats + (size_t)b * C * 2 : nullptr;

    const bool gn = a.gn_gamma != nullptr;
    const bool se = (!gn) && a.gate != nullptr;
    float gatev[8];
    {
        const float4 g0 = se ? *reinterpret_cast<const float4*>(a.gate + (size_t)b * C + c0) : make_float4(1.f, 1.f, 1.f, 1.f);
        const float4 g1 = se ? *reinterpret_cast<const float4*>(a.gate + (size_t)b * C + c0 + 4) : make_float4(1.f, 1.f, 1.f, 1.f);
        gatev[0] = g0.x; gatev[1] = g0.y; gatev[2] = g0.z; gatev[3] = g0.w;
        gatev[4] = g1.x; gatev[5] = g1.y; gatev[6] = g1.z; gatev[7] = g1.w;
    }
    float g2w = 0.f, g2b = 0.f;
    if (a.y2 != nullptr && tid < C) { g2w = a.gn2_gamma[tid]; g2b = a.gn2_beta[tid]; }
    half8 tv[4], rv[4];
    static_for<0, 4>([&](auto k_) __attribute__((always_inline)) {
        constexpr int k = decltype(k_)::value;
        tv[k] = *reinterpret_cast<const half8*>(t + k * C);
        rv[k] = res ? *reinterpret_cast<const half8*>(res + k * C) : half8{0, 0, 0, 0, 0, 0, 0, 0};
    });

    if (gn) {
        for (int c = tid; c < C; c += nthr) {
            const int g0 = (c >> 4) << 4;
            float s = 0.f, ss = 0.f;
            for (int j = 0; j < 16; ++j) { s += tst[2 * (g0 + j)]; ss += tst[2 * (g0 + j) + 1]; }
            const float mean = s * (1.f / 1024.f);
            float var = ss * (1.f / 1024.f) - mean * mean;
            var = var > 0.f ? var : 0.f;
            const float g = a.gn_gamma[c] * rsqrtf(var + 1e-5f);
            sc[c] = g;
            sh[c] = a.gn_beta[c] - mean * g;
        }
    }
    __syncthreads();

    float scl[8], shl[8];
    static_for<0, 8>([&](auto i_) __attribute__((always_inline)) {
        constexpr int i = decltype(i_)::value;
        scl[i] = gn ? sc[c0 + i] : gatev[i];
        shl[i] = gn ? sh[c0 + i] : 0.f;
    });
    float x[4][8];
    float pe[4][8];
    if (a.posenc) {
        static_for<0, 4>([&](auto k_) __attribute__((always_inline)) {
            constexpr int k = decltype(k_)::value;
            const float4 p0 = *reinterpret_cast<const float4*>(a.posenc + (sg * 4 + k) * C + c0);
            const float4 p1 = *reinterpret_cast<const float4*>(a.posenc + (sg * 4 + k) * C + c0 + 4);
            pe[k][0] = p0.x; pe[k][1] = p0.y; pe[k][2] = p0.z; pe[k][3] = p0.w;
            pe[k][4] = p1.x; pe[k][5] = p1.y; pe[k][6] = p1.z; pe[k][7] = p1.w;
        });
    }
    static_for<0, 4>([&](auto k_) __attribute__((always_inline)) {
        constexpr int k = decltype(k_)::value;
        static_for<0, 8>([&](auto i_) __attribute__((always_inline)) {
            constexpr int i = decltype(i_)::value;
            float v = (float)tv[k][i];
            if (gn) v = act_apply(v * scl[i] + shl[i], a.act);
            else if (se) v *= scl[i];
            v += (float)rv[k][i];
            if (a.posenc) v += pe[k][i];
            x[k][i] = v;
        });
    });
    if (a.ln_g != nullptr) {
        float2* part = reinterpret_cast<float2*>(red);
        static_for<0, 4>([&](auto k_) __attribute__((always_inline)) {
            constexpr int k = decltype(k_)::value;
            float rs = 0.f, rss = 0.f;
            static_for<0, 8>([&](auto i_) __attribute__((always_inline)) { const float v = x[k][decltype(i_)::value]; rs += v; rss += v * v; });
            part[(sg * 4 + k) * NC + chunk] = make_float2(rs, rss);
        });
        __syncthreads();
        float2* rowp = reinterpret_cast<float2*>(rowbuf);
        for (int u = tid; u < 512; u += nthr) {
            const int sq = u >> 3, p8 = u & 7;
            float rs = 0.f, rss = 0.f;
            for (int ch = p8; ch < NC; ch += 8) { const float2 v = part[sq * NC + ch]; rs += v.x; rss += v.y; }
#pragma unroll
            for (int o = 1; o < 8; o <<= 1) { rs += __shfl_xor(rs, o); rss += __shfl_xor(rss, o); }
            if (p8 == 0) {
                const float cnt = (float)(a.ln_count > 0 ? a.ln_count : C);
                const float mean = rs / cnt;
                float var = rss / cnt - mean * mean;
                var = var > 0.f ? var : 0.f;
                rowp[sq] = make_float2(mean, rsqrtf(var + 1e-5f));
            }
        }
        __syncthreads();
        float lg[8], lb[8];
        static_for<0, 8>([&](auto i_) __attribute__((always_inline)) {
            constexpr int i = decltype(i_)::value;
            lg[i] = a.ln_g[c0 + i]; lb[i] = a.ln_b[c0 + i];
        });
        static_for<0, 4>([&](auto k_) __attribute__((always_inline)) {
            constexpr int k = decltype(k_)::value;
            const float2 mr = rowp[sg * 4 + k];
            static_for<0, 8>([&](auto i_) __attribute__((always_inline)) {
                constexpr int i = decltype(i_)::value;
                x[k][i] = (x[k][i] - mr.x) * mr.y * lg[i] + lb[i];
            });
        });
        __syncthreads();
    }

    _Float16* y = a.y + (size_t)b * 64 * C + (size_t)(sg * 4) * C + c0;
    half8 yv[4];
    float csum[8], csq[8];
    static_for<0, 8>([&](auto i_) __attribute__((always_inline)) { csum[decltype(i_)::value] = 0.f; csq[decltype(i_)::value] = 0.f; });
    static_for<0, 4>([&](auto k_) __attribute__((always_inline)) {
        constexpr int k = decltype(k_)::value;
        static_for<0, 8>([&](auto i_) __attribute__((always_inline)) {
            constexpr int i = decltype(i_)::value;
            yv[k][i] = (_Float16)x[k][i];
            csum[i] += x[k][i]; csq[i] += x[k][i] * x[k][i];
        });
        *reinterpret_cast<half8*>(y + k * C) = yv[k];
    });
    if (a.out_stats == nullptr && a.y2 == nullptr) return;
    static_for<0, 8>([&](auto i_) __attribute__((always_inline)) {
        constexpr int i = decltype(i_)::value;
        reinterpret_cast<float2*>(red)[sg * C + c0 + i] = make_float2(csum[i], csq[i]);
    });
    __syncthreads();
    for (int c = tid; c < C; c += nthr) {
        float s = 0.f, ss = 0.f;
        for (int g = 0; g < 16; ++g) { const float2 v = reinterpret_cast<const float2*>(red)[g * C + c]; s += v.x; ss += v.y; }
        tot[2 * c] = s; tot[2 * c + 1] = ss;
        if (a.out_stats != nullptr) {
            a.out_stats[((size_t)b * C + c) * 2] = s;
            a.out_stats[((size_t)b * C + c) * 2 + 1] = ss;
        }
    }
    if (a.y2 == nullptr) return;
    __syncthreads();
    if (tid < C) {
        const int c = tid, g0 = (c >> 4) << 4;
        float s = 0.f, ss = 0.f;
        for (int j = 0; j < 16; ++j) { s += tot[2 * (g0 + j)]; ss += tot[2 * (g0 + j) + 1]; }
        const float mean = s * (1.f / 1024.f);
        float var = ss * (1.f / 1024.f) - mean * mean;
        var = var > 0.f ? var : 0.f;
        const float g = g2w * rsqrtf(var + 1e-5f);
        sc[c] = g;
        sh[c] = g2b - mean * g;
    }
    __syncthreads();
    _Float16* y2 = a.y2 + (size_t)b * 64 * C + (size_t)(sg * 4) * C + c0;
    static_for<0, 8>([&](auto i_) __attribute__((always_inline)) { constexpr int i = decltype(i_)::value; scl[i] = sc[c0 + i]; shl[i] = sh[c0 + i]; });
    static_for<0, 4>([&](auto k_) __attribute__((always_inline)) {
        constexpr int k = decltype(k_)::value;
        half8 ov;
        static_for<0, 8>([&](auto i_) __attribute__((always_inline)) {
            constexpr int i = decltype(i_)::value;
            ov[i] = (_Float16)act_apply((float)yv[k][i] * scl[i] + shl[i], a.act);
        });
        *reinterpret_cast<half8*>(y2 + k * C) = ov;
    });
}

hipError_t launch_ew_board(const EwArgs& a, int boards, hipStream_t st) {
    if (a.C > 384 || a.C % 32 != 0) return hipErrorInvalidValue;
    const int nthr = 2 * a.C;
    const size_t lds = (size_t)(4 * a.C + 128 + 32 * a.C) * 4;
    hipLaunchKernelGGL(ew_board_kernel, dim3(boards), dim3(nthr), lds, st, a);
    return hipGetLastError();
}

__global__ __launch_bounds__(384) void se_gate_kernel(SeGateArgs a) {
    extern __shared__ __attribute__((aligned(16))) char smem[];
    const int C = a.C, Hd = a.hidden;
    float* pool = reinterpret_cast<float*>(smem);
    float* part = pool + 8 * C;
    float* hid = part + 8 * C;
    const int tid = threadIdx.x, nthr = blockDim.x;
    const int b0 = blockIdx.x * 8;
    const int nb = a.B - b0 < 8 ? a.B - b0 : 8;
    for (int q = 0; q < 8; ++q)
        pool[q * C + tid] = q < nb ? a.t_stats[((size_t)(b0 + q) * C + tid) * 2] * (1.f / 64.f) : 0.f;
    __syncthreads();
    const int parts = nthr / Hd;
    {
        const int j = tid % Hd, p = tid / Hd;
        if (p < parts) {
            const int cpp = (C + parts - 1) / parts;
            const int cbeg = p * cpp, cend = cbeg + cpp < C ? cbeg + cpp : C;
            float s[8] = {0.f, 0.f, 0.f, 0.f, 0.f, 0.f, 0.f, 0.f};
            for (int cb = cbeg; cb < cend; cb += 16) {
                float w[16];
#pragma unroll
                for (int u = 0; u < 16; ++u) w[u] = cb + u < cend ? a.w1[(size_t)(cb + u) * Hd + j] : 0.f;
#pragma unroll
                for (int u = 0; u < 16; ++u) {
                    const int c = cb + u < cend ? cb + u : cbeg;
#pragma unroll
                    for (int q = 0; q < 8; ++q) s[q] = __builtin_fmaf(w[u], pool[q * C + c], s[q]);
                }
            }
#pragma unroll
            for (int q = 0; q < 8; ++q) part[(p * 8 + q) * Hd + j] = s[q];
        }
    }
    __syncthreads();
    for (int i = tid; i < 8 * Hd; i += nthr) {
        const int q = i / Hd, j = i - q * Hd;
        float s = a.b1[j];
        for (int p = 0; p < parts; ++p) s += part[(p * 8 + q) * Hd + j];
        hid[q * Hd + j] = act_apply(s, a.act);
    }
    __syncthreads();
    {
        const int c = tid;
        const float bias = a.b2[c];
        float s[8] = {bias, bias, bias, bias, bias, bias, bias, bias};
        for (int jb = 0; jb < Hd; jb += 16) {
            float w[16];
#pragma unroll
            for (int u = 0; u < 16; ++u) w[u] = jb + u < Hd ? a.w2[(size_t)(jb + u) * C + c] : 0.f;
#pragma unroll
            for (int u = 0; u < 16; ++u) {
                const int j = jb + u < Hd ? jb + u : 0;
#pragma unroll
                for (int q = 0; q < 8; ++q) s[q] = __builtin_fmaf(w[u], hid[q * Hd + j], s[q]);
            }
        }
        for (int q = 0; q < nb; ++q) a.gate[(size_t)(b0 + q) * C + c] = 1.f / (1.f + __expf(-s[q]));
    }
}

hipError_t launch_se_gate(const SeGateArgs& a, hipStream_t st) {
    if (a.C > 384 || a.C % 32 != 0 || a.hidden < 1 || a.hidden > a.C) return hipErrorInvalidValue;
    const size_t lds = (size_t)(8 * a.C + 8 * a.C + 8 * a.hidden) * 4;
    hipLaunchKernelGGL(se_gate_kernel, dim3((a.B + 7) / 8), dim3(a.C), lds, st, a);
    return hipGetLastError();
}

#define ATT_BOARDS 16
__global__ __launch_bounds__(256) void attn_core_kernel(AttnArgs a) {
    constexpr int VROW = 68;
    __shared__ __attribute__((aligned(16))) _Float16 Vt[4][16][VROW];
    __shared__ __attribute__((aligned(16))) _Float16 Bs[4][64][VROW];
    __shared__ __attribute__((aligned(16))) _Float16 Ms[64][VROW];
    const int tid = threadIdx.x, lane = tid & 63, wave = tid >> 6;
    const int H = a.H, C = a.C;
    const int hgroups = (H + 3) >> 2;
    const int hg = blockIdx.x % hgroups, bgroup = blockIdx.x / hgroups;
    const int h = hg * 4 + wave;
    const bool hlive = h < H;
    const int r31 = lane & 31, half = lane >> 5;
    if (a.rel_bias != nullptr) {
        for (int i = tid; i < 4 * 64 * 16; i += 256) {
            const int hh = i >> 10, q = (i >> 4) & 63, k4 = (i & 15) * 4;
            if (hg * 4 + hh < H) {
                const float4 v = *reinterpret_cast<const float4*>(a.rel_bias + ((size_t)(hg * 4 + hh) * 64 + q) * 64 + k4);
                typedef _Float16 half4s __attribute__((ext_vector_type(4)));
                *reinterpret_cast<half4s*>(&Bs[hh][q][k4]) = half4s{(_Float16)v.x, (_Float16)v.y, (_Float16)v.z, (_Float16)v.w};
            }
        }
    }
    for (int i = tid; i < 64 * 16; i += 256) {
        const int q = i >> 4, k4 = (i & 15) * 4;
        const uint64_t m = a.mask[q] >> k4;
        typedef _Float16 half4s __attribute__((ext_vector_type(4)));
        *reinterpret_cast<half4s*>(&Ms[q][k4]) = half4s{(_Float16)(float)(m & 1), (_Float16)(float)((m >> 1) & 1),
                                                        (_Float16)(float)((m >> 2) & 1), (_Float16)(float)((m >> 3) & 1)};
    }
    __syncthreads();
    for (int it = 0; it < ATT_BOARDS; ++it) {
    const int b = bgroup * ATT_BOARDS + it;
// ... 143 lines not shown
```

matrix0_amd/csrc/selfplay.hip:

```cpp
#include <math.h>
#include <string.h>
#include <atomic>
#include "selfplay_engine.h"

namespace m0 {

static bool nn_cache_miss(m0_selfplay* sp, uint64_t key) {
    auto it = sp->nn_map.find(key);
    if (it != sp->nn_map.end()) {
        sp->nn_lru.splice(sp->nn_lru.end(), sp->nn_lru, it->second);
        return false;
    }
    sp->nn_lru.push_back(key);
    sp->nn_map[key] = std::prev(sp->nn_lru.end());
    if (sp->nn_lru.size() > 10000) { sp->nn_map.erase(sp->nn_lru.front()); sp->nn_lru.pop_front(); }
    return true;
}

void seed_game_dev(GameDev& g, uint64_t base, int uid) {
    g.seed_jitter = derive_seed(base, uid, PURPOSE_JITTER);
    g.seed_noise = derive_seed(base, uid, PURPOSE_NOISE);
    g.seed_dir = derive_seed(base, uid, PURPOSE_DIRICHLET);
    g.ctr_jitter = g.ctr_noise = g.ctr_dir = 0;
}
// ... 57 lines not shown
                (void)hipMemcpyAsync(sp->ssl_pos_dev, hgm.rec_pos.data(), sizeof(Pos) * T, hipMemcpyHostToDevice, sp->stream);
                (void)launch_ssl_targets(sp->ssl_pos_dev, T, sp->ssl_out_dev, sp->stream);
                (void)hipMemcpyAsync(o->ssl.data(), sp->ssl_out_dev, (size_t)T * 17 * 64 * 4, hipMemcpyDeviceToHost, sp->stream);
                (void)hipStreamSynchronize(sp->stream);
            }
        }
        m0_game_record r;
        memset(&r, 0, sizeof(r));
        r.game_index = hgm.game_index; r.moves = hgm.nstates; r.resigned = resigned ? 1 : 0; r.resigner = resigner;
        r.draw = z == 0.0f ? 1 : 0; r.total_plies = (int)hgm.history.size(); r.result = z;
        r.avg_policy_entropy = (float)(hgm.entropy_sum / (double)(hgm.entropy_count > 0 ? hgm.entropy_count : 1));
        double ss = 0; for (int v : hgm.sims_used) ss += v;
        r.avg_sims = hgm.sims_used.empty() ? 0.f : (float)(ss / (double)hgm.sims_used.size());
        r.secs = (now_ms() - hgm.t0) / 1000.0;
        r.s = o->s.data(); r.pi = o->pi.data(); r.z = o->z.data(); r.legal_mask = o->legal_mask.data();
        r.search_values = o->search_values.data(); r.played = o->played.data(); r.owner = o;
        r.ssl = o->ssl.empty() ? nullptr : o->ssl.data();
        sp->done_meta.push_back(r);
    }
    hgm.in_use = false;
    sp->hg[slot].active = 0;
}

static void begin_move(m0_selfplay* sp, int slot, int child_slot, std::vector<int>& adv_ids, std::vector<int>& adv_slots) {
    HostGame& hgm = sp->games[slot];
    const m0_selfplay_cfg& c = sp->cfg;
    DrawCfg dc = draw_cfg_from(c);
    if (is_game_over(hgm.pos, hgm.win, c.arena_mode != 0) || hgm.nstates >= c.max_game_len ||
        should_adjudicate_draw(hgm.pos, hgm.win, hgm.history, dc)) {
        finish_game(sp, slot, false, 0, false, 0.f);
        return;
    }
    if (c.arena_mode) {
        child_slot = -1;
        sp->hg[slot].net_id = ((hgm.pos.turn == WHITE) == hgm.a_is_white) ? 0 : 1;
    }
    const bool cap_draws = c.playout_random_frac > 0.0 && c.num_simulations > 0;
    int sims = playout_cap(c.num_simulations, c.playout_random_frac, cap_draws ? hgm.rng.next() : 0.0);
    hgm.cur_sims = sims;
    if (c.fresh_tree_per_move || c.tt_merge) child_slot = -1;
    if (c.arena_mode && c.tt_merge) child_slot = hgm.nstates == 0 ? -3 : -2;
    const bool dir = c.dirichlet_plies < 0 || hgm.nstates < c.dirichlet_plies;
    arm_search(sp, slot, hgm.pos, hgm.win, sims, dir, child_slot < 0);
    adv_ids.push_back(slot);
    adv_slots.push_back(child_slot);
}

static void start_game(m0_selfplay* sp, int slot, std::vector<int>& adv_ids, std::vector<int>& adv_slots) {
    HostGame& hgm = sp->games[slot];
    hgm = HostGame();
    hgm.in_use = true;
    hgm.game_index = sp->cfg.first_game_index + sp->next_game++;
    sp->stats.games_started++;
    parse_fen(START_FEN, hgm.pos);
    hgm.rng = HStream(derive_seed(sp->cfg.seed, hgm.game_index, PURPOSE_GAME));
    if (!sp->book.empty()) {
        size_t k = (size_t)(hgm.rng.next() * (double)sp->book.size());
        if (k >= sp->book.size()) k = sp->book.size() - 1;
        hgm.pos = sp->book[k];
    }
    hgm.t0 = now_ms();
    hgm.a_is_white = (hgm.game_index % 2) == 0;
    seed_game_dev(sp->hg[slot], sp->cfg.seed, hgm.game_index);
    sp->hg[slot].evals = 0;
    for (int i = 0; i < sp->cfg.opening_random_plies; ++i) {
        if (is_game_over(hgm.pos, hgm.win, false)) break;
        Move mv[M0_MAX_MOVES];
        int n = gen_legal(hgm.pos, mv);
        if (n <= 0) break;
        int k = (int)(hgm.rng.next() * n);
        if (k >= n) k = n - 1;
        hgm.play(mv[k]);
    }
    begin_move(sp, slot, -1, adv_ids, adv_slots);
}

static void finish_search(m0_selfplay* sp, int slot, std::vector<int>& adv_ids, std::vector<int>& adv_slots) {
    HostGame& hgm = sp->games[slot];
    const m0_selfplay_cfg& c = sp->cfg;
    const RootResult& R = sp->hres[slot];
    const GameDev& g = sp->hg[slot];
    const int k = R.nchild;
    long total = 0;
    int maxv = 0;
    for (int i = 0; i < k; ++i) { total += R.child_n[i]; if (R.child_n[i] > maxv) maxv = R.child_n[i]; }
    if (k <= 0 || total <= 0) {
        sp->stats.arena_overflows++;
        hgm.nstates = 0;
        hgm.states.clear(); hgm.pis.clear(); hgm.masks.clear(); hgm.search_values.clear(); hgm.turns.clear();
        hgm.sims_used.clear(); hgm.rec_pos.clear();
        finish_game(sp, slot, false, 0, true, 0.f);
        return;
    }
    const double root_q = R.root_n > 0 ? R.root_q : g.root_v;
    const size_t T = (size_t)hgm.nstates;
    if (c.record_games) {
        hgm.pis.resize((T + 1) * 4672, 0.f);
        float* pi = hgm.pis.data() + T * 4672;
        for (int i = 0; i < k; ++i) pi[R.child_idx[i]] = (float)((double)R.child_n[i] / (double)total);
        hgm.states.resize((T + 1) * 19 * 64);
        encode_planes_f32(hgm.pos, hgm.states.data() + T * 19 * 64);
        if (c.ssl_targets) hgm.rec_pos.push_back(hgm.pos);
        hgm.masks.resize((T + 1) * 4672, 0);
        uint8_t* mk = hgm.masks.data() + T * 4672;
        if (c.max_children > 0 || c.min_child_prior > 0.0) {
            Move lm[M0_MAX_MOVES];
            const int nl = gen_legal(hgm.pos, lm);
            for (int i = 0; i < nl; ++i) mk[move_to_index(hgm.pos, lm[i])] = 1;
        } else {
            for (int i = 0; i < k; ++i) mk[R.child_idx[i]] = 1;
        }
    }
    {
        double ent = 0.0;
        for (int i = 0; i < k; ++i) {
            double p = (double)(float)((double)R.child_n[i] / (double)total);
            if (p < 1e-12) p = 1e-12;
            ent -= p * log(p);
        }
        ent -= (double)(4672 - k) * (1e-12 * log(1e-12));
        hgm.entropy_sum += ent; hgm.entropy_count++;
        hgm.resign.recent_entropies.push_back(ent);
        if ((int)hgm.resign.recent_entropies.size() > c.resign_window) hgm.resign.recent_entropies.erase(hgm.resign.recent_entropies.begin());
    }
    double temp = temperature_for(hgm.pos.fullmove, c.temperature_start, c.temperature_end, c.temperature_moves);
    if (c.low_visit_threshold > 0 && maxv < c.low_visit_threshold && temp < 0.8) temp = 0.8;
    std::vector<int32_t> visits(R.child_n, R.child_n + k);
    int pick;
    if (c.arena_mode) {
        const bool sampling = c.arena_temp > 1e-3 && hgm.nstates < c.arena_temp_plies;
        pick = arena_choose_move(visits.data(), k, c.arena_temp, hgm.nstates, c.arena_temp_plies, sampling ? hgm.rng.next() : 0.0);
    } else {
        pick = sample_move_index(visits.data(), k, temp, sample_move_draws(visits.data(), k, temp) ? hgm.rng.next() : 0.0);
    }
    const Move mv = R.child_mv[pick];
    hgm.search_values.push_back((float)root_q);
    hgm.turns.push_back(hgm.pos.turn == WHITE ? 1 : -1);
    hgm.sims_used.push_back(hgm.cur_sims);
    hgm.nstates++;
    sp->stats.plies++;
    if (!c.arena_mode && resign_update(hgm.resign, root_q, hgm.nstates, c)) {
        const bool white = hgm.pos.turn == WHITE;
        finish_game(sp, slot, true, white ? 1 : 2, true, white ? -1.f : 1.f);
        return;
    }
    hgm.play(mv);
    begin_move(sp, slot, pick, adv_ids, adv_slots);
}

int run_select(m0_selfplay* sp, int* rows_out) {
    if (hipMemsetAsync(sp->d.row_counter, 0, 8, sp->stream) != hipSuccess) return -1;
    if (launch_select(sp->d, sp->tc, sp->stream) != hipSuccess) return -1;
    if (hipMemcpyAsync(sp->rows2, sp->d.row_counter, 8, hipMemcpyDeviceToHost, sp->stream) != hipSuccess) return -1;
    if (hipStreamSynchronize(sp->stream) != hipSuccess) return -1;
    *rows_out = sp->rows2[0];
    return 0;
}

int apply_advances(m0_selfplay* sp, std::vector<int>& ids, std::vector<int>& slots) {
    if (sync_games_h2d(sp) != 0) return -1;
    if (!ids.empty()) {
        (void)hipMemcpyAsync(sp->ids_dev, ids.data(), ids.size() * 4, hipMemcpyHostToDevice, sp->stream);
        (void)hipMemcpyAsync(sp->slots_dev, slots.data(), slots.size() * 4, hipMemcpyHostToDevice, sp->stream);
        if (launch_advance(sp->d, sp->ids_dev, sp->slots_dev, (int)ids.size(), sp->stream) != hipSuccess) return -1;
        if (hipStreamSynchronize(sp->stream) != hipSuccess) return -1;
        if (sp->d.tt_sides == 2) {
            if (sync_games_d2h(sp) != 0) return -1;
            bool any = false;
            for (size_t k = 0; k < ids.size(); ++k) {
                if (slots[k] > -2) continue;
                GameDev& g = sp->hg[ids[k]];
                const uint64_t salt = (g.net_id & 1) ? 0x9E3779B97F4A7C15ull : 0ull;
                const uint64_t gsalt = (uint64_t)(uint32_t)sp->games[ids[k]].game_index * 0xD6E8FEB86659FD93ull;
                g.reinfer = (g.root_found && nn_cache_miss(sp, tkey(g.root_pos) ^ salt ^ gsalt)) ? 1 : 0;
                any = any || g.reinfer;
            }
            if (any && sync_games_h2d(sp) != 0) return -1;
        }
    }
    return 0;
}

static void count_active_games(m0_selfplay* sp) {
    int act = 0;
    for (int s = 0; s < sp->G; ++s) act += sp->games[s].in_use ? 1 : 0;
    sp->stats.active_games = act;
}

int start_first_games(m0_selfplay* sp) {
    if (sp->stats.games_started != 0) return M0_OK;
    std::vector<int> ids, slots;
    if (sync_games_d2h(sp) != 0) { m0_set_error("device sync failed"); return M0_ERR_HIP; }
    for (int s = 0; s < sp->G; ++s) {
        if (sp->cfg.total_games > 0 && sp->next_game >= sp->cfg.total_games) break;
        start_game(sp, s, ids, slots);
    }
    if (apply_advances(sp, ids, slots) != 0) { m0_set_error("advance failed"); return M0_ERR_HIP; }
    count_active_games(sp);
    return M0_OK;
}

static constexpr int M0_MAX_DEVICES = 16;
static std::mutex g_forward_gate[M0_MAX_DEVICES];
static std::atomic<int> g_engines_with_net[M0_MAX_DEVICES];
static bool forward_gate_enabled() {
    static const bool on = [] { const char* v = getenv("M0_FORWARD_GATE"); return v && v[0] == '1'; }();
    return on;
}

struct ForwardGate {
    std::mutex* m = nullptr;
    hipStream_t st = nullptr;
    ForwardGate(int device, hipStream_t stream, bool has_rows) : st(stream) {
        if (has_rows && forward_gate_enabled() && (unsigned)device < (unsigned)M0_MAX_DEVICES &&
            g_engines_with_net[device].load(std::memory_order_relaxed) > 1) {
            m = &g_forward_gate[device];
            m->lock();
        }
    }
    void release() {
        if (m) { (void)hipStreamSynchronize(st); m->unlock(); m = nullptr; }
    }
    ~ForwardGate() { release(); }
};

void forward_gate_join(m0_selfplay* sp) {
    if ((unsigned)sp->device < (unsigned)M0_MAX_DEVICES) { g_engines_with_net[sp->device].fetch_add(1); sp->counted = true; }
}
void forward_gate_leave(m0_selfplay* sp) {
    if (sp->counted) g_engines_with_net[sp->device].fetch_sub(1);
}

int step_back(m0_selfplay* sp, int rows, double t0, std::string& err) {
    (void)hipEventRecord(sp->ev2, sp->stream);
    if (launch_expand(sp->d, sp->tc, sp->stream) != hipSuccess) { err = "expand launch failed"; return M0_ERR_HIP; }
    (void)hipEventRecord(sp->ev3, sp->stream);
    if (sync_games_d2h(sp) != 0) { err = std::string("step failed: ") + hipGetErrorString(hipGetLastError()); return M0_ERR_HIP; }
    if (sp->net) sp->net->harvest_profile();
    if (sp->net_b) sp->net_b->harvest_profile();
    float ms_sel = 0, ms_net = 0, ms_exp = 0;
    (void)hipEventElapsedTime(&ms_sel, sp->ev0, sp->ev1);
    (void)hipEventElapsedTime(&ms_net, sp->ev1, sp->ev2);
    (void)hipEventElapsedTime(&ms_exp, sp->ev2, sp->ev3);
    sp->stats.ms_net += ms_net; sp->stats.ms_tree += ms_sel + ms_exp;
    sp->stats.steps++; sp->stats.evals += (uint64_t)rows;
    const double t1 = now_ms();
    bool any = false;
    if (sp->tc.eval_cache) {
        uint64_t h = 0;
        for (int s = 0; s < sp->G; ++s) h += sp->hg[s].cache_hits;
        sp->stats.evals_cached = h;
    }
    for (int s = 0; s < sp->G; ++s) {
        if (!sp->hg[s].active) continue;
        const int delta = sp->hg[s].sims_done - sp->prev_done[s];
        if (delta > 0) { sp->stats.sims += (uint64_t)delta; sp->prev_done[s] = sp->hg[s].sims_done; }
        if (sp->hg[s].finished) any = true;
    }
    std::vector<int> ids, slots;
    if (any) {
        (void)hipMemcpy(sp->hres.data(), sp->d.results, sizeof(RootResult) * sp->G, hipMemcpyDeviceToHost);
        for (int s = 0; s < sp->G; ++s) {
            if (!(sp->hg[s].active && sp->hg[s].finished)) continue;
            if (sp->hg[s].overflow) sp->stats.arena_overflows++;
            finish_search(sp, s, ids, slots);
        }
        for (int s = 0; s < sp->G; ++s) {
            if (sp->games[s].in_use) continue;
            if (sp->cfg.total_games > 0 && sp->next_game >= sp->cfg.total_games) continue;
            start_game(sp, s, ids, slots);
        }
        if (apply_advances(sp, ids, slots) != 0) { err = "advance failed"; return M0_ERR_HIP; }
    }
    count_active_games(sp);
    const double t2 = now_ms();
    sp->stats.ms_host += t2 - t1;
    sp->stats.ms_total += t2 - t0;
    return M0_OK;
}

struct RowSplit { int main_rows, tail_rows; };
static RowSplit split_rows(int rows, bool have_tail, bool half_split) {
    int main_rows = rows;
    if (have_tail && rows >= 2048 && (rows & 1023) != 0) main_rows = rows & ~1023;
    if (have_tail && half_split && rows >= 4096) main_rows = ((rows / 2) + 1023) & ~1023;
    return {main_rows, rows - main_rows};
}

int one_step(m0_selfplay* sp, std::string& err) {
    const double t0 = now_ms();
    (void)hipEventRecord(sp->ev0, sp->stream);
    int rows = 0;
    if (run_select(sp, &rows) != 0) { err = std::string("select failed: ") + hipGetErrorString(hipGetLastError()); return M0_ERR_HIP; }
    (void)hipEventRecord(sp->ev1, sp->stream);
    if (rows > sp->rows_max || sp->rows2[1] > sp->rows_max) { err = "row counter overflow"; return M0_ERR_STATE; }
    ForwardGate gate(sp->device, sp->stream, rows > 0 || sp->rows2[1] > 0);
    if (rows > 0) {
        if (!sp->net) { err = "m0_selfplay_step needs a network (use the split-step API without one)"; return M0_ERR_STATE; }
        const auto [main_rows, tail_rows] = split_rows(rows, sp->net_tail != nullptr, sp->half_split);
        float* ssl = sp->cfg.ssl_in_forward ? sp->ssl_dev : nullptr;
        m0_net_lock(sp->nethandle);
        int rc = M0_OK;
        if (tail_rows > 0) (void)hipEventRecord(sp->ev_sel, sp->stream);
        rc = sp->net->forward(nullptr, sp->d.x0, main_rows, sp->logits_dev, sp->values_dev, ssl, sp->stream, err);
        if (rc == M0_OK && tail_rows > 0) {
            (void)hipStreamWaitEvent(sp->stream_tail, sp->ev_sel, 0);
            const size_t sslw = ssl ? (size_t)sp->net->ssl_channels_total() * 64 : 0;
            rc = sp->net_tail->forward(nullptr, sp->d.x0 + (size_t)main_rows * 64 * 32, tail_rows, sp->logits_dev + (size_t)main_rows * 4672,
                                       sp->values_dev + main_rows, ssl ? ssl + (size_t)main_rows * sslw : nullptr, sp->stream_tail, err);
            (void)hipEventRecord(sp->ev_tail, sp->stream_tail);
            (void)hipStreamWaitEvent(sp->stream, sp->ev_tail, 0);
        }
        m0_net_unlock(sp->nethandle);
        if (rc != M0_OK) return rc;
        sp->stats.rows_tail += (uint64_t)tail_rows;
    }
    if (sp->rows2[1] > 0) {
        if (!sp->net_b) { err = "rows for a second network without one"; return M0_ERR_STATE; }
        const size_t b = (size_t)sp->d.net_row_base;
        m0_net_lock(sp->nethandle_b);
        int rc = sp->net_b->forward(nullptr, sp->d.x0 + b * 64 * 32, sp->rows2[1], sp->logits_dev + b * 4672,
                                    sp->values_dev + b, nullptr, sp->stream, err);
        m0_net_unlock(sp->nethandle_b);
        if (rc != M0_OK) return rc;
        rows += sp->rows2[1];
    }
    gate.release();
    return step_back(sp, rows, t0, err);
}

}
```

matrix0_amd/csrc/selfplay_engine.h:

```cpp
#pragma once
#include <hip/hip_runtime.h>
#include <chrono>
#include <deque>
#include <list>
#include <mutex>
#include <string>
#include <unordered_map>
#include <vector>
#include "../../include/m0_engine.h"
#include "capi_common.h"
#include "chess_core.h"
#include "host_rules.h"
#include "net.h"
#include "tree.h"

namespace m0 {

inline double now_ms() {
    return std::chrono::duration<double, std::milli>(std::chrono::steady_clock::now().time_since_epoch()).count();
}

struct GameRecordOwner {
    std::vector<float> s, pi, z, search_values, ssl;
    std::vector<uint8_t> legal_mask;
    std::vector<uint16_t> played;
};

struct HostGame : Line {
    bool in_use = false;
    int game_index = 0;
    std::vector<Pos> rec_pos;
    std::vector<float> states, pis, search_values;
    std::vector<int8_t> turns;
    std::vector<uint8_t> masks;
    std::vector<int> sims_used;
    int nstates = 0;
    double entropy_sum = 0.0;
    int entropy_count = 0;
    ResignState resign;
    HStream rng;
    double t0 = 0.0;
    int cur_sims = 0;
    bool a_is_white = true;
};

}

struct m0_selfplay {
    m0_selfplay_cfg cfg;
    TreeCfg tc;
    m0_net* nethandle = nullptr;
    m0_net* nethandle_b = nullptr;
    Net* net = nullptr;
    Net* net_b = nullptr;
    Net* net_tail = nullptr;
    hipStream_t stream_tail = nullptr;
    hipEvent_t ev_sel = nullptr, ev_tail = nullptr;
    bool half_split = false;
    int device = 0;
    hipStream_t stream = nullptr;
    bool own_stream = false;
    int G = 0, L = 0, cap = 0, rows_max = 0;
    TreeDev d;
    std::vector<void*> allocs;
    bool alloc_failed = false;
    std::vector<GameDev> hg;
    std::vector<m0::HostGame> games;
    std::vector<RootResult> hres;
    float* logits_dev = nullptr;
    float* values_dev = nullptr;
    float* ssl_dev = nullptr;
    m0::Pos* ssl_pos_dev = nullptr;
    float* ssl_out_dev = nullptr;
    int ssl_cap = 0;
    int* ids_dev = nullptr;
    int* slots_dev = nullptr;
    std::deque<m0_game_record> done_meta;
    m0_selfplay_stats stats;
    int next_game = 0;
    hipEvent_t ev0 = nullptr, ev1 = nullptr, ev2 = nullptr, ev3 = nullptr;
    std::mutex mu;
    std::vector<Sample> hsamples;
    std::vector<int> prev_done;
    int last_rows = 0, last_rows_b = 0;
    int rows2[2] = {0, 0};
    std::vector<m0::Pos> book;
    std::list<uint64_t> nn_lru;
    std::unordered_map<uint64_t, std::list<uint64_t>::iterator> nn_map;
    bool ext_pending = false;
    bool counted = false;
};

namespace m0 {

template <typename T>
T* dalloc(m0_selfplay* sp, size_t count) {
    void* p = nullptr;
    size_t bytes = count * sizeof(T);
    if (bytes == 0) bytes = 16;
    if (hipMalloc(&p, bytes) != hipSuccess) { sp->alloc_failed = true; return nullptr; }
    (void)hipMemsetAsync(p, 0, bytes, sp->stream);
    sp->allocs.push_back(p);
    return (T*)p;
}

void forward_gate_join(m0_selfplay* sp);
void forward_gate_leave(m0_selfplay* sp);
void seed_game_dev(GameDev& g, uint64_t base, int uid);
int sync_games_d2h(m0_selfplay* sp);
void arm_search(m0_selfplay* sp, int slot, const Pos& pos, const RepWindow& win, int sims, bool dirichlet, bool fresh);
int apply_advances(m0_selfplay* sp, std::vector<int>& ids, std::vector<int>& slots);
int start_first_games(m0_selfplay* sp);
int run_select(m0_selfplay* sp, int* rows_out);
int one_step(m0_selfplay* sp, std::string& err);
int step_back(m0_selfplay* sp, int rows, double t0, std::string& err);

}
```

matrix0_amd/csrc/tree.h:

```cpp
#pragma once
#include <hip/hip_runtime.h>
#include <stdint.h>
#include "chess_core.h"
#include "../../include/m0_engine.h"

#define M0_MAX_DEPTH 256
#define M0_HIST_CAP 192
#define M0_MAX_CHILDREN 256
constexpr int M0_NHWC_C = 32;

struct TreeCfg {
    double fpu_reduction;
    double draw_penalty;
    double virtual_loss;
    double selection_jitter;
    double cpuct;
    double cpuct_start, cpuct_end;
    int cpuct_plies;
    int use_c_base;
    double cpuct_c_base, cpuct_c_init;
    double dirichlet_alpha, dirichlet_frac;
    int legal_softmax;
    int enable_entropy_noise;
    int no_instant_backtrack;
    int virtual_loss_active;
    int leaves_per_step;
    int tt_merge;
    int raw_legal_priors;
    int max_children;
    double min_child_prior;
    int eval_cache;
};

#define M0_EC_MAXLEGAL 64
#define M0_EC_WORDS 66
struct EvalCache {
    uint64_t* keys;
    uint32_t* stamps;
    float* payload;
    float* hit_stage;
    int sets;
};

struct GameDev {
    m0::Pos root_pos;
    int root;
    int next;
    int arena;
    int active;
    int sims_done, sims_target;
    int need_dirichlet;
    int root_q_from_v;
    int flip_root_v;
    int root_fresh;
    int hist_len;
    int nsamples;
    int overflow;
    int finished;
    int root_n;
    double root_q;
    double root_v;
    uint64_t seed_jitter, seed_noise, seed_dir;
    uint64_t ctr_jitter, ctr_noise, ctr_dir;
    uint64_t evals;
    int net_id;
    int reinfer;
    uint64_t cache_hits;
    uint32_t cache_clock;
    int side_next[2];
    int root_found;
};

enum SampleKind : int {
    SK_NONE = 0,
    SK_EVAL = 1,
    SK_ROOT_INIT = 2,
    SK_TERMINAL = 3,
    SK_ROOT_VALUE = 4,
    SK_CACHED = 5,
    SK_SHARED = 6,
};
M0_HD bool sample_owns_row(int kind) { return kind == SK_EVAL || kind == SK_ROOT_INIT || kind == SK_ROOT_VALUE; }
M0_HD bool sample_holds_inflight(int kind) { return kind == SK_EVAL || kind == SK_TERMINAL || kind == SK_CACHED || kind == SK_SHARED; }

struct Sample {
    m0::Pos pos;
    int kind;
    uint64_t ckey;
    int leaf;
    int depth;
    int row;
    int nlegal;
};
static_assert(sizeof(Sample) == 104, "the host copies Sample arrays device-to-host: the layout must not move");

struct TreeArrays {
    double* prior;
    double* w;
    double* q;
    int* n;
    int* vl;
    int* cbase;
    int16_t* nch;
    uint16_t* mv;
    uint16_t* midx;
    int cap;
};

struct RootResult {
    int nchild;
    int root_n;
    double root_q;
    int child_node[M0_MAX_CHILDREN];
    int child_n[M0_MAX_CHILDREN];
    uint16_t child_mv[M0_MAX_CHILDREN];
    uint16_t child_idx[M0_MAX_CHILDREN];
    double child_prior[M0_MAX_CHILDREN];
    double child_q[M0_MAX_CHILDREN];
};

struct TreeDev {
    TreeArrays t;
    GameDev* games;
    Sample* samples;
    int* paths;
    int* epaths;
    uint64_t* tt_keys;
    int* tt_nodes;
    int tt_cap;
    EvalCache ec;
    int search_nodes;
    int tt_sides;
    uint16_t* leaf_moves;
    uint64_t* hist;
    RootResult* results;
    int* row_counter;
    int net_row_base;
    _Float16* x0;
    const float* logits;
    const float* values;
    int G;
    int L;
};

hipError_t launch_select(const TreeDev& d, const TreeCfg& c, hipStream_t st);
hipError_t launch_expand(const TreeDev& d, const TreeCfg& c, hipStream_t st);
hipError_t launch_advance(const TreeDev& d, const int* game_ids_dev, const int* child_slots_dev, int count, hipStream_t st);

hipError_t launch_encode_positions(const m0::Pos* pos_dev, int n, float* planes_f32_dev ,
                                   _Float16* nhwc_dev , uint8_t* mask_dev ,
                                   int32_t* nlegal_dev, uint16_t* moves_dev , int32_t* idx_dev ,
                                   hipStream_t st);

hipError_t launch_ssl_targets(const m0::Pos* pos_dev, int n, float* out_dev, hipStream_t st);
```

matrix0_amd/csrc/tree_expand.hip:

```cpp
#include "tree_device.h"
#include "eval_cache.h"

struct ExpandScratch {
    float pr[M0_MAX_CHILDREN];
    uint8_t keep[M0_MAX_CHILDREN];
    float total;
    int bad;
};

struct ExpandEnv {
    Arena A;
    int cap;
    GameDev* gd;
    uint64_t* TK; int* TN; int tt_cap;
    ExpandScratch* X;
    int lane;
};
struct LeafLogits {
    const float* row;
    const float* legal;
    float* store;
};
__device__ __forceinline__ LeafLogits logits_of_row(const float* row, float* store) { return LeafLogits{row, nullptr, store}; }
__device__ __forceinline__ LeafLogits logits_of_cache(const float* payload) { return LeafLogits{nullptr, payload + EC_LOGITS, nullptr}; }
constexpr int CPL = M0_MAX_CHILDREN / 64;
static_assert(M0_POLICY_SIZE % 4 == 0, "logit rows are read as 16-byte pieces");

static __device__ float np_sum_f32_dev(const float* a, int n) {
    auto block = [&](const float* b, int m) -> float {
        if (m < 8) { float r = 0.f; for (int i = 0; i < m; ++i) r += b[i]; return r; }
        float r[8];
        for (int j = 0; j < 8; ++j) r[j] = b[j];
        int i;
        for (i = 8; i < m - (m % 8); i += 8)
            for (int j = 0; j < 8; ++j) r[j] += b[i + j];
        float res = ((r[0] + r[1]) + (r[2] + r[3])) + ((r[4] + r[5]) + (r[6] + r[7]));
        for (; i < m; ++i) res += b[i];
        return res;
    };
    if (n <= 128) return block(a, n);
    int n2 = n / 2;
    n2 -= n2 % 8;
    return block(a, n2) + block(a + n2, n - n2);
}

__device__ __forceinline__ bool row_nonfinite(const float* lg, int lane) {
    constexpr int N4 = M0_POLICY_SIZE / 4, PER_LANE = (N4 + 63) / 64;
    const uint4* lg4 = reinterpret_cast<const uint4*>(lg);
    uint4 v[PER_LANE];
#pragma unroll
    for (int k = 0; k < PER_LANE; ++k) { const int j = lane + 64 * k; v[k] = lg4[j < N4 ? j : N4 - 1]; }
    uint32_t acc = 0;
#pragma unroll
    for (int k = 0; k < PER_LANE; ++k) {
        acc |= (uint32_t)((v[k].x & 0x7f800000u) == 0x7f800000u) | (uint32_t)((v[k].y & 0x7f800000u) == 0x7f800000u) |
               (uint32_t)((v[k].z & 0x7f800000u) == 0x7f800000u) | (uint32_t)((v[k].w & 0x7f800000u) == 0x7f800000u);
    }
    return acc != 0;
}

__device__ __forceinline__ void priors_raw(const float* lg, const int (&idx)[CPL], int n, int lane, ExpandScratch* X, float (&pr)[CPL]) {
#pragma unroll
    for (int k = 0; k < CPL; ++k) { const int i = lane + 64 * k; if (i < n) X->pr[i] = lg[idx[k]]; }
    __syncthreads();
    if (lane == 0) X->total = np_sum_f32_dev(X->pr, n);
    __syncthreads();
    const float total = X->total;
    const bool ok = isfinite(total) && total > 0.f;
#pragma unroll
    for (int k = 0; k < CPL; ++k) { const int i = lane + 64 * k; pr[k] = i < n ? (ok ? X->pr[i] / total : 1.0f / (float)n) : 0.f; }
    __syncthreads();
}

__device__ __forceinline__ void priors_uniform(int n, float (&pr)[CPL]) {
#pragma unroll
    for (int k = 0; k < CPL; ++k) pr[k] = 1.0f / (float)n;
}

__device__ __forceinline__ void priors_legal_softmax(const LeafLogits& src, const int (&idx)[CPL], int n, int lane, GameDev* gd,
                                                     const TreeCfg& c, float (&pr)[CPL]) {
    float mx = -3.0e38f;
    double ent = 0.0;
    float l[CPL];
#pragma unroll
    for (int k = 0; k < CPL; ++k) {
        const int i = lane + 64 * k;
        l[k] = i < n ? (src.legal ? src.legal[i] : src.row[idx[k]]) : -3.0e38f;
        mx = fmaxf(mx, l[k]);
        if (src.store && i < n && i < M0_EC_MAXLEGAL) src.store[EC_LOGITS + i] = l[k];
    }
    mx = wave_max_f(mx);
    double e[CPL], sum = 0.0;
#pragma unroll
    for (int k = 0; k < CPL; ++k) { const int i = lane + 64 * k; e[k] = i < n ? exp((double)(l[k] - mx)) : 0.0; sum += e[k]; }
    sum = wave_sum_d(sum);
#pragma unroll
    for (int k = 0; k < CPL; ++k) {
        const int i = lane + 64 * k;
        pr[k] = (float)(e[k] / sum);
        if (i < n) ent -= (double)pr[k] * log((double)pr[k] + 1e-8);
    }
    ent = wave_sum_d(ent);
    const double ratio = ent / fmax(1e-9, log((double)(n > 1 ? n : 1)));
    if (c.enable_entropy_noise && ratio > 0.9) {
        const uint64_t ctr = gd->ctr_noise;
        const uint64_t seed = gd->seed_noise;
        double dd[CPL], ds = 0.0;
#pragma unroll
        for (int k = 0; k < CPL; ++k) {
            const int i = lane + 64 * k;
            dd[k] = 0.0;
            if (i < n) { dd[k] = fmax((double)pr[k] + 0.1 * normal_at(seed, ctr + 2ull * (uint64_t)i), 1e-8); ds += dd[k]; }
        }
        ds = wave_sum_d(ds);
#pragma unroll
        for (int k = 0; k < CPL; ++k) pr[k] = (float)(dd[k] / ds);
        if (lane == 0) gd->ctr_noise = ctr + 2ull * (uint64_t)n;
    }
}

__device__ __forceinline__ void priors_full_softmax(const float* lg, const int (&idx)[CPL], int n, int lane, GameDev* gd,
                                                    const TreeCfg& c, float (&pr)[CPL]) {
    float mx = -3.0e38f;
    double ent = 0.0;
    for (int j = lane; j < M0_POLICY_SIZE; j += 64) mx = fmaxf(mx, lg[j]);
    mx = wave_max_f(mx);
    double sum = 0.0;
    for (int j = lane; j < M0_POLICY_SIZE; j += 64) sum += exp((double)(lg[j] - mx));
    sum = wave_sum_d(sum);
    const double fsum = sum;
    for (int j = lane; j < M0_POLICY_SIZE; j += 64) {
        const double pj = (double)(float)(exp((double)(lg[j] - mx)) / sum);
        ent -= pj * log(pj + 1e-8);
    }
#pragma unroll
    for (int k = 0; k < CPL; ++k) { const int i = lane + 64 * k; pr[k] = i < n ? (float)(exp((double)(lg[idx[k]] - mx)) / sum) : 0.f; }
    ent = wave_sum_d(ent);
    const double ratio = ent / fmax(1e-9, log((double)(n > 1 ? n : 1)));
    if (c.enable_entropy_noise && ratio > 0.9) {
        const uint64_t ctr = gd->ctr_noise;
        const uint64_t seed = gd->seed_noise;
        double ds = 0.0;
        for (int j = lane; j < M0_POLICY_SIZE; j += 64)
            ds += fmax((double)(float)(exp((double)(lg[j] - mx)) / fsum) + 0.1 * normal_at(seed, ctr + 2ull * (uint64_t)j), 1e-8);
        ds = wave_sum_d(ds);
#pragma unroll
        for (int k = 0; k < CPL; ++k) {
            const int i = lane + 64 * k;
            if (i < n) {
                const int j = idx[k];
                pr[k] = (float)(fmax((double)pr[k] + 0.1 * normal_at(seed, ctr + 2ull * (uint64_t)j), 1e-8) / ds);
            }
        }
        if (lane == 0) gd->ctr_noise = ctr + 2ull * (uint64_t)M0_POLICY_SIZE;
    }
}

__device__ __forceinline__ void priors_renormalise(int n, int lane, float (&pr)[CPL]) {
    double tot = 0.0;
#pragma unroll
    for (int k = 0; k < CPL; ++k) { const int i = lane + 64 * k; if (i < n) { if (!(pr[k] >= 0.f) || !isfinite(pr[k])) pr[k] = 0.f; tot += (double)pr[k]; } }
    tot = wave_sum_d(tot);
    const float totf = (float)tot;
    if (totf > 0.f && isfinite(totf)) {
#pragma unroll
        for (int k = 0; k < CPL; ++k) pr[k] = pr[k] / totf;
    } else priors_uniform(n, pr);
}

__device__ __forceinline__ int prune_children(const TreeCfg& c, const float (&pr)[CPL], int n, int lane, ExpandScratch* X, int (&slot)[CPL]) {
#pragma unroll
    for (int k = 0; k < CPL; ++k) slot[k] = lane + 64 * k;
    if (!(c.max_children > 0 || c.min_child_prior > 0.0)) return n;
#pragma unroll
    for (int k = 0; k < CPL; ++k) {
        const int i = lane + 64 * k;
        if (i < n) { X->pr[i] = pr[k]; X->keep[i] = (c.min_child_prior > 0.0 && !((double)pr[k] >= c.min_child_prior)) ? 0 : 1; }
    }
    __syncthreads();
    int kept = 0;
    for (int j = 0; j < n; ++j) kept += X->keep[j];
    const bool topk = c.max_children > 0 && kept > c.max_children;
    const int nkeep = topk ? c.max_children : kept;
#pragma unroll
    for (int k = 0; k < CPL; ++k) {
        const int i = lane + 64 * k;
        slot[k] = -1;
        if (i < n && X->keep[i]) {
            int r = 0;
            if (topk) { for (int j = 0; j < n; ++j) r += (X->keep[j] && (X->pr[j] > pr[k] || (X->pr[j] == pr[k] && j < i))) ? 1 : 0; }
            else { for (int j = 0; j < i; ++j) r += X->keep[j]; }
            if (r < nkeep) slot[k] = r;
        }
    }
    __syncthreads();
    return nkeep;
}

__device__ __forceinline__ bool write_children(const ExpandEnv& E, int leaf, const Pos& pos, const Move (&mvv)[CPL], const int (&idx)[CPL],
                                               const float (&pr)[CPL], const int (&slot)[CPL], int n, int nkeep, bool reg_children) {
    const Arena& A = E.A;
    GameDev* gd = E.gd;
    const int lane = E.lane;
    const int cb = gd->next;
    if (cb + nkeep > E.cap) { if (lane == 0) gd->overflow = 1; return false; }
#pragma unroll
    for (int k = 0; k < CPL; ++k) {
        const int i = lane + 64 * k;
        if (i < n && slot[k] >= 0) {
            const int ci = cb + slot[k];
            node_reset(A, ci, (double)pr[k], mvv[k], (uint16_t)idx[k]);
            if (E.TK && reg_children) {
                Pos q = pos;
                make_move(q, mvv[k]);
                tt_insert(E.TK, E.TN, E.tt_cap, tt_key_of(q), ci);
            }
        }
    }
    if (E.TK && !reg_children && lane == 0) tt_insert(E.TK, E.TN, E.tt_cap, tt_key_of(pos), leaf);
    if (lane == 0) { A.cbase[leaf] = cb; A.nch[leaf] = (int16_t)nkeep; gd->next = cb + nkeep; }
    __syncthreads();
    return true;
}

__device__ __forceinline__ bool expand_node(const ExpandEnv& E, const TreeCfg& c, int leaf, const Pos& pos, const uint16_t* smoves, int n,
                                   const LeafLogits& src, bool is_root, bool reg_children) {
    const int lane = E.lane;
    if (n <= 0) return true;
    bool bad = false;
    if (!src.legal) bad = row_nonfinite(src.row, lane);
    bad = __any(bad);
    if (lane == 0) E.X->bad = bad ? 1 : 0;
    float pr[CPL];
    int idx[CPL];
    Move mvv[CPL];
#pragma unroll
    for (int k = 0; k < CPL; ++k) {
        const int i = lane + 64 * k;
        pr[k] = 0.f; idx[k] = 0; mvv[k] = 0;
        if (i < n) { mvv[k] = smoves[i]; idx[k] = move_to_index(pos, mvv[k]); }
    }
    if (c.raw_legal_priors && c.legal_softmax && !is_root) priors_raw(src.row, idx, n, lane, E.X, pr);
    else if (bad) priors_uniform(n, pr);
    else {
        if (c.legal_softmax) priors_legal_softmax(src, idx, n, lane, E.gd, c, pr);
        else priors_full_softmax(src.row, idx, n, lane, E.gd, c, pr);
        priors_renormalise(n, lane, pr);
    }
    int slot[CPL];
    const int nkeep = prune_children(c, pr, n, lane, E.X, slot);
    return write_children(E, leaf, pos, mvv, idx, pr, slot, n, nkeep, reg_children);
}

__device__ __forceinline__ void expand_evaluated(const TreeDev& d, const TreeCfg& c, const ExpandEnv& E, int g, const Sample& smp,
                                                 const uint16_t* moves, const float* lg, float v) {
    const Arena& A = E.A;
    GameDev* gd = E.gd;
    const int lane = E.lane, kind = smp.kind, leaf = smp.leaf;
    const Pos pos = smp.pos;
    float* cw = nullptr;
    size_t ce = 0;
    const uint64_t ckey = kind == SK_EVAL ? smp.ckey : 0ull;
    if (ckey != 0 && isfinite(v)) {
        ce = ec_choose_victim(d.ec, g, ckey, lane);
        cw = ec_payload(d.ec, ce);
        ec_invalidate(d.ec, ce, lane);
    }
    const bool ok = expand_node(E, c, leaf, pos, moves, smp.nlegal, logits_of_row(lg, cw), kind == SK_ROOT_INIT,
                                !(kind == SK_ROOT_INIT && gd->root_fresh));
    if (c.eval_cache && kind == SK_EVAL && lane == 0 && A.nch[leaf] < 0) A.cbase[leaf] = -1;
    const int sig = cw ? legal_sig(moves, smp.nlegal, lane) : 0;
    if (cw && lane == 0) {
        if (ok && !E.X->bad) ec_publish(d.ec, gd, ce, ckey, v, sig);
    }
}

__device__ __forceinline__ void release_inflight(const TreeDev& d, const TreeCfg& c, const Arena& A, int g, const Sample* S, const int* P,
                                                 int ns, int lane) {
    for (int s = lane; s < ns; s += 64) {
        if (sample_holds_inflight(S[s].kind)) {
            const int* path = (c.tt_merge ? d.epaths + (size_t)g * (d.L + 1) * M0_MAX_DEPTH : P) + (size_t)s * M0_MAX_DEPTH;
            for (int dd = 1; dd <= S[s].depth; ++dd) atomicSub(&A.vl[path[dd]], 1);
        }
    }
}

__device__ __forceinline__ void write_root_result(RootResult* R, const Arena& A, int root, int lane) {
    const int k = A.nch[root] > 0 ? A.nch[root] : 0;
    const int cb = A.cbase[root];
    for (int i = lane; i < k; i += 64) {
        R->child_node[i] = cb + i; R->child_n[i] = A.n[cb + i];
        R->child_mv[i] = A.mv[cb + i]; R->child_idx[i] = A.midx[cb + i];
        R->child_prior[i] = A.prior[cb + i]; R->child_q[i] = A.q[cb + i];
    }
    if (lane == 0) { R->nchild = k; R->root_n = A.n[root]; R->root_q = A.q[root]; }
}

__global__ __launch_bounds__(64) void expand_kernel(TreeDev d, TreeCfg c) {
    __shared__ ExpandScratch X;
    const int g = blockIdx.x, lane = threadIdx.x;
    GameDev* gd = &d.games[g];
    if (!gd->active) return;
    uint64_t* TK = c.tt_merge ? d.tt_keys + tt_table_of(d, g, gd) : nullptr;
    int* TN = c.tt_merge ? d.tt_nodes + tt_table_of(d, g, gd) : nullptr;
    const uint16_t* LM = d.leaf_moves + (size_t)g * (d.L + 1) * M0_MAX_CHILDREN;
    const int ns = gd->nsamples;
    if (ns <= 0) return;
    const Arena A = arena_of(d.t, g, gd->arena);
    const ExpandEnv E{A, d.t.cap, gd, TK, TN, d.tt_cap, &X, lane};
    const Sample* S = d.samples + (size_t)g * (d.L + 1);
    const int* P = d.paths + (size_t)g * (d.L + 1) * M0_MAX_DEPTH;
    const bool may_repeat = c.tt_merge != 0;
    int sims = 0;
    uint64_t evals = 0, hits = 0;
    for (int s = 0; s < ns; ++s) {
        const int kind = S[s].kind;
        const int* path = P + (size_t)s * M0_MAX_DEPTH;
        const uint16_t* moves = LM + (size_t)s * M0_MAX_CHILDREN;
        if (kind == SK_SHARED) {
            const float v = d.values[S[s].row];
            backprop(A, path, S[s].depth, (double)v, lane, may_repeat, NoMirror{});
            ++sims; ++hits;
            __syncthreads();
        } else if (kind == SK_CACHED) {
            const int leaf = S[s].leaf, depth = S[s].depth;
            const float* pay = ec_hit_stage(d, g, s);
            const float v = pay[EC_VALUE];
            if (A.nch[leaf] < 0) {
                const Pos pos = S[s].pos;
                expand_node(E, c, leaf, pos, moves, S[s].nlegal, logits_of_cache(pay), false, true);
            }
            backprop(A, path, depth, (double)v, lane, may_repeat, NoMirror{});
            ++sims; ++hits;
            __syncthreads();
        } else if (kind == SK_EVAL || kind == SK_ROOT_INIT) {
            const int leaf = S[s].leaf, depth = S[s].depth, row = S[s].row;
            const float* lg = d.logits + (size_t)row * M0_POLICY_SIZE;
            const float v = d.values[row];
            if (A.nch[leaf] < 0) expand_evaluated(d, c, E, g, S[s], moves, lg, v);
            ++evals;
            if (kind == SK_EVAL) {
                backprop(A, path, depth, (double)v, lane, may_repeat, NoMirror{});
                ++sims;
            } else {
                const double rv = root_value(gd, v);
                if (lane == 0) {
                    gd->root_v = rv;
                    if (gd->root_q_from_v) { A.q[leaf] = rv; gd->root_q_from_v = 0; }
                }
            }
            __syncthreads();
        } else if (kind == SK_TERMINAL) {
            ++sims;
        } else if (kind == SK_ROOT_VALUE) {
            const double rv = root_value(gd, d.values[S[s].row]);
            if (lane == 0) gd->root_v = rv;
            ++evals;
        }
    }
    if (c.virtual_loss_active) release_inflight(d, c, A, g, S, P, ns, lane);
    __syncthreads();
    const int done = gd->sims_done + sims;
    const int root = gd->root;
    const bool fin = (A.nch[root] >= 0 || gd->overflow) && done >= gd->sims_target;
    if (lane == 0) {
        gd->sims_done = done;
        gd->evals += evals;
        gd->cache_hits += hits;
        gd->finished = fin ? 1 : 0;
        gd->root_n = A.n[root];
        gd->root_q = A.q[root];
    }
    if (fin) write_root_result(d.results + g, A, root, lane);
}

hipError_t launch_expand(const TreeDev& d, const TreeCfg& c, hipStream_t st) {
    hipLaunchKernelGGL(expand_kernel, dim3(d.G), dim3(64), 0, st, d, c);
    return hipGetLastError();
}
```

matrix0_amd/engine.py:

```python
from __future__ import annotations

import ctypes as C
from typing import Dict, List, Optional

import numpy as np

from . import _lib

c_double, c_int, c_u64 = C.c_double, C.c_int, C.c_uint64


class SelfplayCfg(C.Structure):
    _fields_ = [
        ("num_simulations", c_int), ("cpuct", c_double), ("cpuct_start", c_double), ("cpuct_end", c_double),
        ("cpuct_plies", c_int), ("use_c_base", c_int), ("cpuct_c_base", c_double), ("cpuct_c_init", c_double),
        ("dirichlet_alpha", c_double), ("dirichlet_frac", c_double), ("dirichlet_plies", c_int),
        ("selection_jitter", c_double), ("fpu_reduction", c_double), ("draw_penalty", c_double), ("virtual_loss", c_double),
        ("legal_softmax", c_int), ("enable_entropy_noise", c_int), ("no_instant_backtrack", c_int), ("value_from_white", c_int),
        ("inference_batch_size", c_int), ("playout_random_frac", c_double),
        ("max_game_len", c_int), ("min_resign_plies", c_int), ("opening_random_plies", c_int),
        ("resign_threshold", c_double), ("resign_window", c_int), ("resign_consecutive_bad", c_int),
        ("resign_min_entropy", c_double), ("resign_value_margin", c_double),
        ("temperature_start", c_double), ("temperature_end", c_double), ("temperature_moves", c_int),
        ("low_visit_threshold", c_int),
        ("draw_enabled", c_int), ("draw_min_plies", c_int), ("draw_window", c_int), ("draw_min_unique", c_int),
        ("draw_halfmove_cap", c_int), ("draw_material_threshold", c_int), ("draw_stalemate", c_int),
        ("concurrent_games", c_int), ("total_games", c_int), ("first_game_index", c_int), ("arena_nodes", c_int),
        ("seed", c_u64), ("virtual_loss_active", c_int), ("ssl_in_forward", c_int), ("ssl_targets", c_int), ("record_games", c_int),
        ("arena_mode", c_int), ("arena_temp", c_double), ("arena_temp_plies", c_int),
        ("fresh_tree_per_move", c_int), ("tt_merge", c_int), ("raw_legal_priors", c_int), ("max_children", c_int),
        ("min_child_prior", c_double), ("root_reinfer", c_int), ("eval_cache", c_int), ("eval_cache_entries", c_int),
        ("tail_split", c_int),
    ]


class SelfplayStats(C.Structure):
    _fields_ = [("steps", c_u64), ("evals", c_u64), ("sims", c_u64), ("plies", c_u64), ("games_finished", c_u64),
                ("games_started", c_u64), ("ms_total", c_double), ("ms_net", c_double), ("ms_tree", c_double),
                ("ms_host", c_double), ("arena_overflows", c_u64), ("ssl_dropped", c_u64), ("evals_cached", c_u64), ("active_games", c_int),
                ("rows_tail", c_u64)]


class GameRecord(C.Structure):
    _fields_ = [("game_index", c_int), ("moves", c_int), ("resigned", c_int), ("resigner", c_int), ("draw", c_int),
                ("total_plies", c_int), ("result", C.c_float), ("avg_policy_entropy", C.c_float), ("avg_sims", C.c_float),
                ("secs", c_double), ("s", C.POINTER(C.c_float)), ("pi", C.POINTER(C.c_float)), ("z", C.POINTER(C.c_float)),
                ("legal_mask", C.POINTER(C.c_uint8)), ("search_values", C.POINTER(C.c_float)),
                ("played", C.POINTER(C.c_uint16)), ("ssl", C.POINTER(C.c_float)), ("owner", C.c_void_p)]


_bound = False


def _bind():
    global _bound
    L = _lib.lib()
    if _bound:
        return L
    L.m0_selfplay_create.restype = C.c_void_p
    L.m0_selfplay_create.argtypes = [C.c_void_p, C.POINTER(SelfplayCfg)]
    L.m0_arena_create.restype = C.c_void_p
    L.m0_arena_create.argtypes = [C.c_void_p, C.c_void_p, C.POINTER(SelfplayCfg)]
    L.m0_arena_create_ext.restype = C.c_void_p
    L.m0_arena_create_ext.argtypes = [C.POINTER(SelfplayCfg)]
    L.m0_arena_ext_select.argtypes = [C.c_void_p, C.POINTER(c_int), C.POINTER(c_int), C.c_void_p, C.c_void_p, c_int]
    L.m0_arena_ext_expand.argtypes = [C.c_void_p, C.c_void_p, C.c_void_p, c_int, C.c_void_p, C.c_void_p, c_int]
    L.m0_san_legal_fen.argtypes = [C.c_char_p, C.c_void_p, C.c_void_p, C.POINTER(c_int)]
    L.m0_san_game.argtypes = [C.c_void_p, c_int, C.c_char_p, c_int]
    L.m0_fen_after.argtypes = [C.c_char_p, C.POINTER(C.c_char_p), c_int, C.c_char_p, c_int]
    L.m0_selfplay_destroy.argtypes = [C.c_void_p]
    L.m0_selfplay_destroy.restype = None
    L.m0_selfplay_step.argtypes = [C.c_void_p, c_int]
    L.m0_selfplay_stats_get.argtypes = [C.c_void_p, C.POINTER(SelfplayStats)]
    L.m0_selfplay_poll.argtypes = [C.c_void_p, C.POINTER(GameRecord)]
    L.m0_game_record_free.argtypes = [C.POINTER(GameRecord)]
    L.m0_game_record_free.restype = None
    L.m0_selfplay_running.argtypes = [C.c_void_p]
    L.m0_selfplay_set_openings.argtypes = [C.c_void_p, C.POINTER(C.c_char_p), c_int]
    L.m0_selfplay_ext_select.argtypes = [C.c_void_p, C.POINTER(c_int), C.c_void_p, c_int]
    L.m0_selfplay_ext_expand.argtypes = [C.c_void_p, C.c_void_p, C.c_void_p, c_int]
    L.m0_selfplay_last_batch_nhwc.argtypes = [C.c_void_p, C.c_void_p, c_int, C.POINTER(c_int)]
    L.m0_encode_fens_nhwc.argtypes = [c_int, C.POINTER(C.c_char_p), c_int, C.c_void_p]
    L.m0_search_begin.argtypes = [C.c_void_p, c_int, C.c_char_p, c_int, c_int, c_int]
    L.m0_search_select.argtypes = [C.c_void_p, C.POINTER(c_int), C.c_void_p, c_int]
    L.m0_search_expand.argtypes = [C.c_void_p, C.c_void_p, C.c_void_p, c_int]
    L.m0_search_result.argtypes = [C.c_void_p, c_int, C.POINTER(c_int)] + [C.c_void_p] * 5 + \
        [C.POINTER(c_double), C.POINTER(c_int), C.POINTER(c_int)]
    L.m0_search_advance.argtypes = [C.c_void_p, c_int, c_int, c_int, c_int]
    L.m0_encode_fens.argtypes = [c_int, C.POINTER(C.c_char_p), c_int] + [C.c_void_p] * 5
    L.m0_move_to_index_fen.argtypes = [c_int, C.c_char_p, C.c_char_p, C.POINTER(C.c_int32)]
    L.m0_decode_move_fen.argtypes = [c_int, C.c_char_p, c_int, C.c_char_p]
    L.m0_ssl_targets_fens.argtypes = [c_int, C.POINTER(C.c_char_p), c_int, C.c_void_p]
    L.m0_sample_move_index.argtypes = [C.c_void_p, c_int, c_double, c_double]
    L.m0_playout_cap.argtypes = [c_int, c_double, c_double]
    L.m0_temperature_for.argtypes = [c_int, c_double, c_double, c_int]
    L.m0_temperature_for.restype = c_double
    L.m0_rules_probe.argtypes = [C.POINTER(SelfplayCfg), C.c_char_p, C.POINTER(C.c_char_p), c_int, C.POINTER(c_int),
                                 C.POINTER(C.c_float)]
    L.m0_arena_choose_move.argtypes = [C.c_void_p, c_int, c_double, c_int, c_int, c_double]
    _bound = True
    return L


def selfplay_cfg_from_dict(cfg: dict, *, concurrent_games: int, total_games: int = 0, first_game_index: int = 0,
                           seed: Optional[int] = None, leaves_per_step: Optional[int] = None,
                           virtual_loss_active: bool = True, ssl_in_forward: bool = False,
                           record_games: bool = True, arena_nodes: int = 0, ssl_targets: bool = False,
                           compat: Optional[dict] = None, eval_cache: Optional[bool] = None,
                           tail_split=None) -> SelfplayCfg:
    m = dict(cfg.get("mcts", {}) or {})
    sp = dict(cfg.get("selfplay", {}) or {})
    draw = dict(cfg.get("draw", {}) or {})
    draw.update(sp.get("draw", {}) or {})
    c = SelfplayCfg()
    c.max_children = int(m.get("max_children", 0) or 0)
    c.min_child_prior = float(m.get("min_child_prior", 0.0) or 0.0)
    if c.max_children < 0 or c.max_children > 256 or c.min_child_prior < 0.0:
        raise ValueError("mcts.max_children must be in [0, 256] and mcts.min_child_prior >= 0")
    c.num_simulations = int(sp.get("num_simulations", m.get("num_simulations", 800)))
    c.cpuct = float(sp.get("cpuct", m.get("cpuct", 2.5)))
    cs, ce, cp = m.get("cpuct_start"), m.get("cpuct_end"), int(m.get("cpuct_plies", 0) or 0)
    if cs is not None and ce is not None and cp > 0:
        c.cpuct_start, c.cpuct_end, c.cpuct_plies = float(cs), float(ce), cp
    else:
        c.cpuct_start = c.cpuct_end = c.cpuct
        c.cpuct_plies = 0
    cb, ci = m.get("cpuct_c_base"), m.get("cpuct_c_init")
    c.use_c_base = int(cb is not None and ci is not None)
    c.cpuct_c_base = float(cb or 1.0)
    c.cpuct_c_init = float(ci or 0.0)
    c.dirichlet_alpha = float(sp.get("dirichlet_alpha", m.get("dirichlet_alpha", 0.3)))
    c.dirichlet_frac = float(sp.get("dirichlet_frac", m.get("dirichlet_frac", 0.25)))
    dp = m.get("dirichlet_plies", 16)
    c.dirichlet_plies = -1 if dp is None else int(dp)
    c.selection_jitter = float(sp.get("selection_jitter", m.get("selection_jitter", 0.01)))
    c.fpu_reduction = float(m.get("fpu_reduction", 0.15))
    c.draw_penalty = float(m.get("draw_penalty", -0.1))
    c.virtual_loss = float(m.get("virtual_loss", 1.0))
    c.legal_softmax = int(bool(m.get("legal_softmax", False)))
    c.enable_entropy_noise = int(bool(m.get("enable_entropy_noise", True)))
    c.no_instant_backtrack = int(bool(m.get("no_instant_backtrack", True)))
    c.value_from_white = int(bool(m.get("value_from_white", False)))
    ibs = int(m.get("inference_batch_size", m.get("simulation_batch_size", 96)) or 96)
    c.inference_batch_size = int(leaves_per_step if leaves_per_step else ibs)
    c.playout_random_frac = float(m.get("playout_random_frac", 0.0))
    c.max_game_len = int(sp.get("max_game_len", 200))
    c.min_resign_plies = int(sp.get("min_resign_plies", 24))
    c.opening_random_plies = int(sp.get("opening_random_plies", (cfg.get("openings", {}) or {}).get("random_plies", 0)))
    c.resign_threshold = float(sp.get("resign_threshold", -0.98))
    c.resign_window = int(sp.get("resign_window", 4))
    c.resign_consecutive_bad = int(sp.get("resign_consecutive_bad", 5))
    c.resign_min_entropy = float(sp.get("resign_min_entropy", 0.3))
    c.resign_value_margin = float(sp.get("resign_value_margin", 0.05))
    c.temperature_start = float(sp.get("temperature_start", 1.0))
    c.temperature_end = float(sp.get("temperature_end", 0.1))
    c.temperature_moves = int(sp.get("temperature_moves", 20))
    c.low_visit_threshold = int(sp.get("low_visit_threshold", 0) or 0)
    c.draw_enabled = int(bool(draw.get("enabled", False)))
    c.draw_min_plies = int(draw.get("min_plies", 30))
    c.draw_window = int(draw.get("window", 12))
    c.draw_min_unique = int(draw.get("min_unique", 3))
    c.draw_halfmove_cap = int(draw.get("halfmove_cap", 50))
    c.draw_material_threshold = int(draw.get("material_draw_threshold", 10))
    c.draw_stalemate = int(bool(draw.get("stalemate_draw", True)))
    c.concurrent_games = int(concurrent_games)
    c.total_games = int(total_games)
    c.first_game_index = int(first_game_index)
    c.arena_nodes = int(arena_nodes)
    c.seed = int(cfg.get("seed", 1234) if seed is None else seed)
    c.virtual_loss_active = int(bool(virtual_loss_active))
    c.ssl_in_forward = int(bool(ssl_in_forward))
    c.ssl_targets = int(bool(ssl_targets))
    c.record_games = int(bool(record_games))
    cp = dict(((cfg.get("engine", {}) or {}).get("compat", {}) or {}))
    cp.update(compat or {})
    unknown = set(cp) - {"fresh_tree_per_move", "tt_merge", "raw_legal_priors", "root_reinfer"}
    if unknown:
        raise ValueError(f"unknown engine.compat keys: {sorted(unknown)}")
    c.fresh_tree_per_move = int(bool(cp.get("fresh_tree_per_move", False)))
    c.tt_merge = int(bool(cp.get("tt_merge", False)))
    c.raw_legal_priors = int(bool(cp.get("raw_legal_priors", False)))
    c.root_reinfer = int(bool(cp.get("root_reinfer", False)))
    ecfg = cfg.get("engine", {}) or {}
    c.eval_cache = int(bool(ecfg.get("eval_cache", False) if eval_cache is None else eval_cache))
    c.eval_cache_entries = int(ecfg.get("eval_cache_entries", 0) or 0)
    ts = ecfg.get("tail_split", False) if tail_split is None else tail_split
    c.tail_split = 2 if ts in ("halves", "half", 2) and ts is not True else int(bool(ts))
    return c


def move_to_uci(m: int) -> str:
    f, t, p = m & 63, (m >> 6) & 63, (m >> 12) & 7
    s = "abcdefgh"[f & 7] + str((f >> 3) + 1) + "abcdefgh"[t & 7] + str((t >> 3) + 1)
    return s + (" nbrq"[p] if p else "")


class SelfplayEngine:

    def __init__(self, backend, cfg: SelfplayCfg):
        self._L = _bind()
        self.backend = backend
        self.cfg = cfg
        self._h = self._L.m0_selfplay_create(backend.handle if backend is not None else None, C.byref(cfg))
        if not self._h:
            raise RuntimeError(f"m0_selfplay_create failed: {_lib.last_error()}")

    def step(self, steps: int = 1) -> None:
        _lib.check(self._L.m0_selfplay_step(self._h, int(steps)), "m0_selfplay_step")

    def stats(self) -> Dict[str, float]:
        s = SelfplayStats()
        _lib.check(self._L.m0_selfplay_stats_get(self._h, C.byref(s)), "m0_selfplay_stats_get")
        return {k: getattr(s, k) for k, _ in SelfplayStats._fields_}

    def running(self) -> bool:
        return bool(self._L.m0_selfplay_running(self._h))

    def poll(self) -> Optional[dict]:
        r = GameRecord()
        rc = self._L.m0_selfplay_poll(self._h, C.byref(r))
        if rc < 0:
            _lib.check(rc, "m0_selfplay_poll")
        if rc == 0:
            return None
        try:
            T = r.moves
            out = {
                "game_index": r.game_index, "moves": T, "resigned": bool(r.resigned),
                "resigner": {0: None, 1: "W", 2: "B"}[r.resigner], "draw": bool(r.draw), "result": float(r.result),
                "avg_policy_entropy": float(r.avg_policy_entropy), "avg_sims": float(r.avg_sims), "secs": float(r.secs),
                "played": ([move_to_uci(int(x)) for x in np.ctypeslib.as_array(r.played, shape=(r.total_plies,))]
                           if r.total_plies > 0 else []),
                "played_raw": (np.ctypeslib.as_array(r.played, shape=(r.total_plies,)).copy()
                               if r.total_plies > 0 else np.zeros(0, np.uint16)),
            }
            if r.s and T > 0:
                out["s"] = np.ctypeslib.as_array(r.s, shape=(T, 19, 8, 8)).copy()
                out["pi"] = np.ctypeslib.as_array(r.pi, shape=(T, 4672)).copy()
                out["legal_mask"] = np.ctypeslib.as_array(r.legal_mask, shape=(T, 4672)).copy()
            if T > 0:
                out["z"] = np.ctypeslib.as_array(r.z, shape=(T,)).copy()
                out["search_values"] = np.ctypeslib.as_array(r.search_values, shape=(T,)).copy()
            if r.ssl:
                ssl = np.ctypeslib.as_array(r.ssl, shape=(T, 17, 8, 8)).copy()
                out["ssl"] = {"piece": ssl[:, :13], "threat": ssl[:, 13], "pin": ssl[:, 14], "fork": ssl[:, 15],
                              "control": ssl[:, 16]}
        finally:
            self._L.m0_game_record_free(C.byref(r))
        return out

    def set_openings(self, fens: List[str]) -> None:
        arr = (C.c_char_p * max(1, len(fens)))(*[f.encode() for f in fens])
        _lib.check(self._L.m0_selfplay_set_openings(self._h, arr, len(fens)), "m0_selfplay_set_openings")

    def ext_select(self) -> np.ndarray:
        rows = c_int(0)
        cap = self.cfg.concurrent_games * (self.cfg.inference_batch_size + 1)
        planes = np.zeros((cap, 19, 8, 8), dtype=np.float32)
        _lib.check(self._L.m0_selfplay_ext_select(self._h, C.byref(rows), planes.ctypes.data_as(C.c_void_p), cap), "m0_selfplay_ext_select")
        return planes[: rows.value]

    def ext_expand(self, logits: np.ndarray, values: np.ndarray) -> None:
        lg = np.ascontiguousarray(logits, dtype=np.float32)
        vv = np.ascontiguousarray(values, dtype=np.float32)
        _lib.check(self._L.m0_selfplay_ext_expand(self._h, lg.ctypes.data_as(C.c_void_p), vv.ctypes.data_as(C.c_void_p),
                                                  int(lg.shape[0])), "m0_selfplay_ext_expand")

    def last_batch_nhwc(self) -> np.ndarray:
        cap = self.cfg.concurrent_games * (self.cfg.inference_batch_size + 1) + 4
        out = np.zeros((cap, 64, 32), dtype=np.float16)
        rows = c_int(0)
        _lib.check(self._L.m0_selfplay_last_batch_nhwc(self._h, out.ctypes.data_as(C.c_void_p), cap, C.byref(rows)),
                   "m0_selfplay_last_batch_nhwc")
        return out[: rows.value]

    def search_begin(self, g: int, fen: str, sims: int, dirichlet: bool, game_uid: int) -> None:
        _lib.check(self._L.m0_search_begin(self._h, g, fen.encode(), sims, int(dirichlet), game_uid), "m0_search_begin")

    def search_select(self) -> np.ndarray:
        rows = c_int(0)
        cap = self.cfg.concurrent_games * (self.cfg.inference_batch_size + 1)
        planes = np.zeros((cap, 19, 8, 8), dtype=np.float32)
        _lib.check(self._L.m0_search_select(self._h, C.byref(rows), planes.ctypes.data_as(C.c_void_p), cap), "m0_search_select")
        return planes[: rows.value]

    def search_expand(self, logits: np.ndarray, values: np.ndarray) -> None:
        lg = np.ascontiguousarray(logits, dtype=np.float32)
        vv = np.ascontiguousarray(values, dtype=np.float32)
        _lib.check(self._L.m0_search_expand(self._h, lg.ctypes.data_as(C.c_void_p), vv.ctypes.data_as(C.c_void_p),
                                            int(lg.shape[0])), "m0_search_expand")

    def search_result(self, g: int) -> dict:
        n = c_int(0); rn = c_int(0); fin = c_int(0); rq = c_double(0)
        cn = np.zeros(256, np.int32); mv = np.zeros(256, np.uint16); idx = np.zeros(256, np.int32)
        pr = np.zeros(256, np.float64); q = np.zeros(256, np.float64)
        _lib.check(self._L.m0_search_result(self._h, g, C.byref(n), cn.ctypes.data_as(C.c_void_p), mv.ctypes.data_as(C.c_void_p),
                                            idx.ctypes.data_as(C.c_void_p), pr.ctypes.data_as(C.c_void_p),
                                            q.ctypes.data_as(C.c_void_p), C.byref(rq), C.byref(rn), C.byref(fin)),
                   "m0_search_result")
        k = n.value
        return {"finished": bool(fin.value), "n": cn[:k].copy(), "moves": [move_to_uci(int(x)) for x in mv[:k]],
                "idx": idx[:k].copy(), "prior": pr[:k].copy(), "q": q[:k].copy(), "root_q": rq.value, "root_n": rn.value}

    def search_advance(self, g: int, slot: int, sims: int, dirichlet: bool) -> None:
        _lib.check(self._L.m0_search_advance(self._h, g, slot, sims, int(dirichlet)), "m0_search_advance")

    def close(self):
        if getattr(self, "_h", None):
            self._L.m0_selfplay_destroy(self._h)
            self._h = None

    def __del__(self):
        try:
            self.close()
        except Exception:
            pass


class SelfplayPool:

    def __init__(self, backend_factory, cfg_dict: dict, *, streams: int, concurrent_games: int, total_games: int = 0,
                 first_game_index: int = 0, **cfg_kw):
        import threading
        self._threading = threading
        streams = max(1, min(int(streams), int(concurrent_games)))
        self.backends, self.engines = [], []
        per = [concurrent_games // streams + (1 if i < concurrent_games % streams else 0) for i in range(streams)]
        tot = [0] * streams if total_games <= 0 else \
              [total_games // streams + (1 if i < total_games % streams else 0) for i in range(streams)]
        first = first_game_index
        try:
            for i in range(streams):
                be = backend_factory()
                self.backends.append(be)
                cfg = selfplay_cfg_from_dict(cfg_dict, concurrent_games=(min(per[i], tot[i]) if total_games > 0 else per[i]) or 1,
                                             total_games=tot[i], first_game_index=first, **cfg_kw)
                self.engines.append(SelfplayEngine(be, cfg))
                first += tot[i] if total_games > 0 else (1 << 20)
        except Exception:
            self.close()
            raise
        self._rr = 0

    def step(self, steps: int = 1) -> None:
        live = [e for e in self.engines if e.running()]
        if len(live) <= 1:
            for e in live:
                e.step(steps)
            return
        errs = []

        def run(e):
            try:
                e.step(steps)
            except Exception as ex:
                errs.append(ex)

        th = [self._threading.Thread(target=run, args=(e,)) for e in live]
        for t in th:
            t.start()
        for t in th:
            t.join()
        if errs:
            raise errs[0]

    def running(self) -> bool:
        return any(e.running() for e in self.engines)

    def poll(self) -> Optional[dict]:
        for k in range(len(self.engines)):
            e = self.engines[(self._rr + k) % len(self.engines)]
            rec = e.poll()
            if rec is not None:
                self._rr = (self._rr + k + 1) % len(self.engines)
                return rec
        return None

    def stats(self) -> Dict[str, float]:
        out: Dict[str, float] = {}
        sts = [e.stats() for e in self.engines]
        for k in sts[0]:
            v = sum(s[k] for s in sts)
            out[k] = v / len(sts) if k.startswith("ms_") or k == "steps" else v
        return out

    def close(self):
        for e in getattr(self, "engines", []):
            e.close()
        for b in getattr(self, "backends", []):
            try:
                b.close()
            except Exception:
                pass
        self.engines, self.backends = [], []


def sample_move_index(visits, temperature: float, u: float) -> int:
    L = _bind()
    v = np.ascontiguousarray(visits, dtype=np.int32)
    return int(L.m0_sample_move_index(v.ctypes.data_as(C.c_void_p), int(v.shape[0]), float(temperature), float(u)))


def playout_cap(sims: int, frac: float, u: float) -> int:
    return int(_bind().m0_playout_cap(int(sims), float(frac), float(u)))


def temperature_for(fullmove: int, t_start: float, t_end: float, t_moves: int) -> float:
    return float(_bind().m0_temperature_for(int(fullmove), float(t_start), float(t_end), int(t_moves)))


RULE_FLAGS = ["game_over", "game_over_claim", "adjudicate_draw", "checkmate", "stalemate", "insufficient",
              "can_claim_fifty", "repetition3", "can_claim_threefold", "fivefold", "seventyfive"]


def rules_probe(cfg: SelfplayCfg, fen: str, ucis: List[str]) -> dict:
    L = _bind()
    arr = (C.c_char_p * max(1, len(ucis)))(*[u.encode() for u in ucis])
    flags = c_int(0); res = C.c_float(0)
    _lib.check(L.m0_rules_probe(C.byref(cfg), fen.encode(), arr, len(ucis), C.byref(flags), C.byref(res)), "m0_rules_probe")
    out = {name: bool(flags.value >> i & 1) for i, name in enumerate(RULE_FLAGS)}
    out["result"] = float(res.value)
    return out


def encode_fens_nhwc(fens, device_index: int = 0) -> np.ndarray:
    L = _bind()
    n = len(fens)
    arr = (C.c_char_p * n)(*[f.encode() for f in fens])
    out = np.empty((n, 64, 32), np.float16)
    _lib.check(L.m0_encode_fens_nhwc(int(device_index), arr, n, out.ctypes.data_as(C.c_void_p)), "m0_encode_fens_nhwc")
    return out


def planes_to_nhwc(planes: np.ndarray) -> np.ndarray:
    p = np.asarray(planes, np.float32)
    out = np.zeros((p.shape[0], 64, 32), np.float16)
    out[:, :, :19] = p.reshape(p.shape[0], 19, 64).transpose(0, 2, 1).astype(np.float16)
    return out


def ssl_targets_fens(fens, device_index: int = 0) -> dict:
    L = _bind()
    n = len(fens)
    arr = (C.c_char_p * n)(*[f.encode() for f in fens])
    out = np.empty((n, 17, 8, 8), np.float32)
    _lib.check(L.m0_ssl_targets_fens(int(device_index), arr, n, out.ctypes.data_as(C.c_void_p)), "m0_ssl_targets_fens")
    return {"piece": out[:, :13], "threat": out[:, 13], "pin": out[:, 14], "fork": out[:, 15], "control": out[:, 16]}


class ArenaEngine(SelfplayEngine):

    def __init__(self, backend_a, backend_b, cfg: SelfplayCfg):
        self._L = _bind()
        self.backend = backend_a
        self.backend_b = backend_b
        self.cfg = cfg
        self._h = self._L.m0_arena_create(backend_a.handle, backend_b.handle, C.byref(cfg))
        if not self._h:
            raise RuntimeError(f"m0_arena_create failed: {_lib.last_error()}")


class ArenaExtEngine(SelfplayEngine):

    def __init__(self, cfg: SelfplayCfg):
        self._L = _bind()
        self.backend = None
        self.cfg = cfg
        self._h = self._L.m0_arena_create_ext(C.byref(cfg))
        if not self._h:
            raise RuntimeError(f"m0_arena_create_ext failed: {_lib.last_error()}")

    def arena_ext_select(self):
        ra, rb = c_int(0), c_int(0)
        cap = self.cfg.concurrent_games * (self.cfg.inference_batch_size + 1)
        pa = np.zeros((cap, 19, 8, 8), dtype=np.float32)
        pb = np.zeros((cap, 19, 8, 8), dtype=np.float32)
        _lib.check(self._L.m0_arena_ext_select(self._h, C.byref(ra), C.byref(rb), pa.ctypes.data_as(C.c_void_p),
                                               pb.ctypes.data_as(C.c_void_p), cap), "m0_arena_ext_select")
        return pa[: ra.value], pb[: rb.value]

    def arena_ext_expand(self, lg_a, v_a, lg_b, v_b) -> None:
        la = np.ascontiguousarray(lg_a, dtype=np.float32); va = np.ascontiguousarray(v_a, dtype=np.float32)
        lb = np.ascontiguousarray(lg_b, dtype=np.float32); vb = np.ascontiguousarray(v_b, dtype=np.float32)
        _lib.check(self._L.m0_arena_ext_expand(self._h, la.ctypes.data_as(C.c_void_p), va.ctypes.data_as(C.c_void_p), int(la.shape[0]),
                                               lb.ctypes.data_as(C.c_void_p), vb.ctypes.data_as(C.c_void_p), int(lb.shape[0])),
                   "m0_arena_ext_expand")


def arena_choose_move(visits, temp: float, ply: int, temp_plies: int, u: float) -> int:
    L = _bind()
    v = np.ascontiguousarray(visits, dtype=np.int32)
    return int(L.m0_arena_choose_move(v.ctypes.data_as(C.c_void_p), int(len(v)), float(temp), int(ply), int(temp_plies), float(u)))


def san_legal(fen: str):
    L = _bind()
    mv = np.zeros(256, np.uint16)
    san = C.create_string_buffer(256 * 8)
    n = c_int(0)
    _lib.check(L.m0_san_legal_fen(fen.encode(), mv.ctypes.data_as(C.c_void_p), san, C.byref(n)), "m0_san_legal_fen")
    raw = san.raw
    return [(move_to_uci(int(mv[i])), raw[8 * i: 8 * i + 8].split(b"\0", 1)[0].decode()) for i in range(n.value)]


def fen_after(fen: str, ucis) -> str:
    L = _bind()
    ucis = list(ucis)
    arr = (C.c_char_p * max(1, len(ucis)))(*[u.encode() for u in ucis])
    buf = C.create_string_buffer(128)
    rc = L.m0_fen_after(fen.encode(), arr, len(ucis), buf, len(buf))
    if rc == -1:
        raise ValueError(_lib.last_error())
    _lib.check(rc, "m0_fen_after")
    return buf.value.decode()


def san_game(moves_raw) -> str:
    L = _bind()
    mv = np.ascontiguousarray(moves_raw, dtype=np.uint16)
    buf = C.create_string_buffer(16 * (len(mv) + 4))
    rc = L.m0_san_game(mv.ctypes.data_as(C.c_void_p), int(len(mv)), buf, len(buf))
    if rc < 0:
        _lib.check(rc, "m0_san_game")
    return buf.value.decode().strip()
```

Measured before the change: 1.129.

## Fuse non-finite logit row detection into policy GEMM epilogue; write value directly

The policy head's final GEMM epilogue now flags rows that contain Inf/NaN logits into a per-row byte array. The tree expand kernel reads that flag instead of scanning each 4672-float logit row a second time, and external logits get the flags from a separate small kernel. The value head GEMM now writes straight to the output vector, which drops the scratch buffer and a 2D device copy. The cost is a memset before each forward and extra checks in the epilogue, plus new restrictions on which GEMM tile paths accept row flags.

```diff
diff --git a/include/m0_engine.h b/include/m0_engine.h
--- a/include/m0_engine.h
+++ b/include/m0_engine.h
@@ -162,6 +162,7 @@
 int m0_selfplay_ext_select(m0_selfplay* sp, int* rows, float* planes, int max_rows);
 int m0_selfplay_ext_expand(m0_selfplay* sp, const float* logits, const float* values, int rows);
 int m0_selfplay_last_batch_nhwc(m0_selfplay* sp, uint16_t* nhwc, int max_rows, int* rows);
+int m0_selfplay_last_row_flags(m0_selfplay* sp, uint8_t* flags, int max_rows, int* rows);
 
 m0_selfplay* m0_arena_create(m0_net* net_a, m0_net* net_b, const m0_selfplay_cfg* cfg);
 m0_selfplay* m0_arena_create_ext(const m0_selfplay_cfg* cfg);
diff --git a/matrix0_amd/csrc/capi_selfplay.hip b/matrix0_amd/csrc/capi_selfplay.hip
--- a/matrix0_amd/csrc/capi_selfplay.hip
+++ b/matrix0_amd/csrc/capi_selfplay.hip
@@ -77,6 +77,7 @@
     sp->d.x0 = dalloc<_Float16>(sp, (size_t)(nreg * sp->rows_max + 4) * 64 * 32);
     sp->logits_dev = dalloc<float>(sp, (size_t)nreg * sp->rows_max * 4672);
     sp->values_dev = dalloc<float>(sp, (size_t)nreg * sp->rows_max + 4);
+    sp->row_bad_dev = dalloc<uint8_t>(sp, (size_t)nreg * sp->rows_max + 64);
     sp->d.net_row_base = sp->rows_max;
     if (sp->cfg.ssl_in_forward && sp->net && sp->net->ssl_channels_total() > 0)
         sp->ssl_dev = dalloc<float>(sp, (size_t)sp->rows_max * sp->net->ssl_channels_total() * 64);
@@ -91,7 +92,7 @@
     }
     sp->ids_dev = dalloc<int>(sp, sp->G);
     sp->slots_dev = dalloc<int>(sp, sp->G);
-    sp->d.logits = sp->logits_dev; sp->d.values = sp->values_dev;
+    sp->d.logits = sp->logits_dev; sp->d.values = sp->values_dev; sp->d.row_bad = sp->row_bad_dev;
     sp->d.G = sp->G; sp->d.L = sp->L;
     return true;
 }
@@ -235,6 +236,7 @@
     if (rows <= 0) return;
     (void)hipMemcpyAsync(sp->logits_dev + row_base * 4672, logits, (size_t)rows * 4672 * 4, hipMemcpyHostToDevice, sp->stream);
     (void)hipMemcpyAsync(sp->values_dev + row_base, values, (size_t)rows * 4, hipMemcpyHostToDevice, sp->stream);
+    (void)launch_row_flags(sp->logits_dev + row_base * 4672, rows, sp->row_bad_dev + row_base, sp->stream);
 }
 
 static int ext_select_impl(m0_selfplay* sp, int* rows_a, int* rows_b, float* planes_a, float* planes_b, int max_rows) {
@@ -433,6 +435,20 @@
     return M0_OK;
 }
 
+int m0_selfplay_last_row_flags(m0_selfplay* sp, uint8_t* out, int max_rows, int* rows) {
+    if (!sp || !out || !rows) { m0_set_error("null argument"); return M0_ERR_INVALID; }
+    std::lock_guard<std::mutex> lk(sp->mu);
+    (void)hipSetDevice(sp->device);
+    const int r = sp->rows2[0];
+    if (r < 0 || r > sp->rows_max || r > max_rows) { m0_set_error("output buffer too small"); return M0_ERR_INVALID; }
+    *rows = r;
+    if (r > 0) {
+        if (hipMemcpyAsync(out, sp->row_bad_dev, (size_t)r, hipMemcpyDeviceToHost, sp->stream) != hipSuccess ||
+            hipStreamSynchronize(sp->stream) != hipSuccess) { m0_set_error("copy failed"); return M0_ERR_HIP; }
+    }
+    return M0_OK;
+}
+
 int m0_selfplay_last_batch_nhwc(m0_selfplay* sp, uint16_t* out, int max_rows, int* rows) {
     if (!sp || !out || !rows) { m0_set_error("null argument"); return M0_ERR_INVALID; }
     std::lock_guard<std::mutex> lk(sp->mu);
diff --git a/matrix0_amd/csrc/net.h b/matrix0_amd/csrc/net.h
--- a/matrix0_amd/csrc/net.h
+++ b/matrix0_amd/csrc/net.h
@@ -72,7 +72,7 @@
     const std::vector<size_t>& device_buffer_bytes() const { return dev_sizes_; }
 
     int forward(const float* planes_dev, const _Float16* nhwc_dev, int B, float* logits_dev, float* value_dev,
-                float* ssl_dev, hipStream_t st, std::string& err);
+                float* ssl_dev, hipStream_t st, std::string& err, uint8_t* row_bad_dev = nullptr);
     int ensure_workspace(int B, std::string& err);
     int ssl_channels_total() const;
     const m0_net_cfg& cfg() const { return cfg_; }
@@ -141,7 +141,6 @@
     float *S1_ = nullptr, *S2_ = nullptr, *G_ = nullptr;
     _Float16 *PH_ = nullptr, *PH2_ = nullptr, *VH_ = nullptr, *VH2_ = nullptr, *F1_ = nullptr, *F2_ = nullptr,
              *F3_ = nullptr, *F4_ = nullptr, *SH_ = nullptr, *SH2_ = nullptr, *SO_ = nullptr;
-    float* VAL_ = nullptr;
     float* SPK_ = nullptr;
 
     const HostTensor* get(const std::string& k, std::string& err);
diff --git a/matrix0_amd/csrc/net.hip b/matrix0_amd/csrc/net.hip
--- a/matrix0_amd/csrc/net.hip
+++ b/matrix0_amd/csrc/net.hip
@@ -497,10 +497,9 @@
     F1_ = H((size_t)Mfc * rp);
     F2_ = H((size_t)Mfc * ceil_to(2 * C_, 32)); F3_ = H((size_t)Mfc * ceil_to(C_, 32)); F4_ = H((size_t)Mfc * ceil_to(C_, 32));
     SH_ = H(nb * 64 * Cs_); SH2_ = H(nb * 64 * Cs_); SO_ = H(nb * 64 * 32);
-    VAL_ = F((size_t)Mfc * 32);
     SPK_ = F((size_t)8 * Mfc * ceil_to(2 * C_, 32));
     if (!X0_ || !XA_ || !XB_ || !AA_ || !T1_ || !T2_ || !QKV_ || !O_ || !S1_ || !S2_ || !PH_ || !PH2_ || !VH_ ||
-        !VH2_ || !F1_ || !F2_ || !F3_ || !F4_ || !SH_ || !SH2_ || !SO_ || !VAL_ || !SPK_) {
+        !VH2_ || !F1_ || !F2_ || !F3_ || !F4_ || !SH_ || !SH2_ || !SO_ || !SPK_) {
         err = "workspace hipMalloc failed";
         wsB_ = wsM_ = 0;
         return M0_ERR_HIP;
@@ -617,7 +616,7 @@
     } while (0)
 
 int Net::forward(const float* planes_dev, const _Float16* nhwc_dev, int B, float* logits_dev, float* value_dev,
-                 float* ssl_dev, hipStream_t st, std::string& err) {
+                 float* ssl_dev, hipStream_t st, std::string& err, uint8_t* row_bad_dev) {
     if (!finalized_) { err = "weights not finalized"; return M0_ERR_STATE; }
     if (B <= 0) { err = "batch must be positive"; return M0_ERR_INVALID; }
     TRY(ensure_workspace(B, err));
@@ -715,6 +714,10 @@
     const PackedGemm& plast = factored ? pfc2_ : pfc1_;
     GemmArgs pl = gemm_args(plast, factored ? F1_ : PH2_, logits_dev, Mfc);
     pl.Mvalid = B; pl.out_f32 = 1; pl.out_scale = logit_scale_;
+    if (row_bad_dev) {
+        KCHK(hipMemsetAsync(row_bad_dev, 0, (size_t)ceil_to(B, 64), st));
+        pl.row_bad = row_bad_dev;
+    }
     KCHK(run_gemm(plast, pl, st));
     if (!joint) KCHK(conv_norm_act(vh0_, vh1_n_, xa, VH2_, VH_, Mc, st));
     _Float16* vflat = joint ? VH_ : VH2_;
@@ -724,10 +727,9 @@
     GemmArgs vg = gemm_args(vgate_, F3_, F4_, Mfc, ACT_SIGMOID);
     vg.mul = F3_;
     KCHK(run_gemm(vgate_, vg, st));
-    GemmArgs v3 = gemm_args(vfc3_, F4_, VAL_, Mfc, ACT_TANH);
-    v3.out_f32 = 1;
+    GemmArgs v3 = gemm_args(vfc3_, F4_, value_dev, Mfc, ACT_TANH);
+    v3.out_f32 = 1; v3.N = 1; v3.ldo = 1; v3.Mvalid = B;
     KCHK(run_gemm(vfc3_, v3, st));
-    KCHK(hipMemcpy2DAsync(value_dev, 4, VAL_, 32 * 4, 4, B, hipMemcpyDeviceToDevice, st));
     if (ssl_dev && !ssl_.empty()) {
         const int ctot = ssl_channels_total();
         int coff = 0;
diff --git a/matrix0_amd/csrc/net_kernels.h b/matrix0_amd/csrc/net_kernels.h
--- a/matrix0_amd/csrc/net_kernels.h
+++ b/matrix0_amd/csrc/net_kernels.h
@@ -40,6 +40,7 @@
     void* out2;
     int ldo2;
     int nsplit;
+    uint8_t* row_bad;
 };
 
 struct EwArgs {
diff --git a/matrix0_amd/csrc/net_kernels.hip b/matrix0_amd/csrc/net_kernels.hip
--- a/matrix0_amd/csrc/net_kernels.hip
+++ b/matrix0_amd/csrc/net_kernels.hip
@@ -184,9 +184,12 @@
     const bool has_mul = a.mul != nullptr;
     const bool f32out = a.out_f32 != 0;
     const bool want_stats = a.out_stats != nullptr;
+    const bool want_bad = a.row_bad != nullptr && f32out;
+    uint32_t badrows = 0;
     static_for<0, NT>([&](auto ni_) __attribute__((always_inline)) {
         constexpr int ni = decltype(ni_)::value;
         const int col = colbase + ni * 32;
+        const bool col_on = col < a.N;
         const float bias = a.bias != nullptr ? a.bias[col] : 0.f;
         float s = 0.f, ss = 0.f;
         static_for<0, 2>([&](auto mi_) __attribute__((always_inline)) {
@@ -200,9 +203,11 @@
                 if (has_mul) v *= (float)a.mul[(size_t)row * ldo + col];
                 v *= oscale;
                 s += v; ss += v * v;
-                if (row < a.Mvalid) {
-                    if (f32out) reinterpret_cast<float*>(a.out)[(size_t)row * ldo + col] = v;
-                    else reinterpret_cast<_Float16*>(a.out)[(size_t)row * ldo + col] = (_Float16)v;
+                if (row < a.Mvalid && col_on) {
+                    if (f32out) {
+                        reinterpret_cast<float*>(a.out)[(size_t)row * ldo + col] = v;
+                        if (want_bad && (__float_as_uint(v) & 0x7f800000u) == 0x7f800000u) badrows |= 1u << (mi * 16 + r);
+                    } else reinterpret_cast<_Float16*>(a.out)[(size_t)row * ldo + col] = (_Float16)v;
                 }
             });
         });
@@ -215,6 +220,12 @@
             }
         }
     });
+    if (badrows != 0) {
+        static_for<0, 32>([&](auto b_) __attribute__((always_inline)) {
+            constexpr int b = decltype(b_)::value;
+            if (badrows & (1u << b)) a.row_bad[rowbase + (b >> 4) * 32 + (b & 3) + 8 * ((b & 15) >> 2)] = 1;
+        });
+    }
 }
 
 
@@ -270,6 +281,8 @@
 hipError_t launch_conv_gemm(const GemmArgs& a, int taps, hipStream_t st) {
     if (a.Mrows % 256 != 0 || a.Cin % 32 != 0 || a.Npad % 32 != 0) return hipErrorInvalidValue;
     const bool big = conv_gemm_tile_n(a.Cin, a.Npad) == 320;
+    if ((a.row_bad != nullptr || a.N != a.Npad) && (big || taps != 1 || a.gn_gamma != nullptr)) return hipErrorInvalidValue;
+    if (a.row_bad != nullptr && !a.out_f32) return hipErrorInvalidValue;
     if (a.gn_gamma != nullptr && !big) {
         if (a.epi_act == ACT_SILU) return launch_conv_gemm_gn<ACT_SILU>(a, taps, st);
         if (a.epi_act == ACT_RELU) return launch_conv_gemm_gn<ACT_RELU>(a, taps, st);
diff --git a/matrix0_amd/csrc/selfplay.hip b/matrix0_amd/csrc/selfplay.hip
--- a/matrix0_amd/csrc/selfplay.hip
+++ b/matrix0_amd/csrc/selfplay.hip
@@ -383,12 +383,13 @@
         m0_net_lock(sp->nethandle);
         int rc = M0_OK;
         if (tail_rows > 0) (void)hipEventRecord(sp->ev_sel, sp->stream);
-        rc = sp->net->forward(nullptr, sp->d.x0, main_rows, sp->logits_dev, sp->values_dev, ssl, sp->stream, err);
+        rc = sp->net->forward(nullptr, sp->d.x0, main_rows, sp->logits_dev, sp->values_dev, ssl, sp->stream, err, sp->row_bad_dev);
         if (rc == M0_OK && tail_rows > 0) {
             (void)hipStreamWaitEvent(sp->stream_tail, sp->ev_sel, 0);
             const size_t sslw = ssl ? (size_t)sp->net->ssl_channels_total() * 64 : 0;
             rc = sp->net_tail->forward(nullptr, sp->d.x0 + (size_t)main_rows * 64 * 32, tail_rows, sp->logits_dev + (size_t)main_rows * 4672,
-                                       sp->values_dev + main_rows, ssl ? ssl + (size_t)main_rows * sslw : nullptr, sp->stream_tail, err);
+                                       sp->values_dev + main_rows, ssl ? ssl + (size_t)main_rows * sslw : nullptr, sp->stream_tail, err,
+                                       sp->row_bad_dev + main_rows);
             (void)hipEventRecord(sp->ev_tail, sp->stream_tail);
             (void)hipStreamWaitEvent(sp->stream, sp->ev_tail, 0);
         }
@@ -401,7 +402,7 @@
         const size_t b = (size_t)sp->d.net_row_base;
         m0_net_lock(sp->nethandle_b);
         int rc = sp->net_b->forward(nullptr, sp->d.x0 + b * 64 * 32, sp->rows2[1], sp->logits_dev + b * 4672,
-                                    sp->values_dev + b, nullptr, sp->stream, err);
+                                    sp->values_dev + b, nullptr, sp->stream, err, sp->row_bad_dev + b);
         m0_net_unlock(sp->nethandle_b);
         if (rc != M0_OK) return rc;
         rows += sp->rows2[1];
diff --git a/matrix0_amd/csrc/selfplay_engine.h b/matrix0_amd/csrc/selfplay_engine.h
--- a/matrix0_amd/csrc/selfplay_engine.h
+++ b/matrix0_amd/csrc/selfplay_engine.h
@@ -69,6 +69,7 @@
     std::vector<RootResult> hres;
     float* logits_dev = nullptr;
     float* values_dev = nullptr;
+    uint8_t* row_bad_dev = nullptr;
     float* ssl_dev = nullptr;
     m0::Pos* ssl_pos_dev = nullptr;
     float* ssl_out_dev = nullptr;
diff --git a/matrix0_amd/csrc/tree.h b/matrix0_amd/csrc/tree.h
--- a/matrix0_amd/csrc/tree.h
+++ b/matrix0_amd/csrc/tree.h
@@ -138,6 +138,7 @@
     int net_row_base;
     _Float16* x0;
     const float* logits;
+    const uint8_t* row_bad;
     const float* values;
     int G;
     int L;
@@ -145,6 +146,7 @@
 
 hipError_t launch_select(const TreeDev& d, const TreeCfg& c, hipStream_t st);
 hipError_t launch_expand(const TreeDev& d, const TreeCfg& c, hipStream_t st);
+hipError_t launch_row_flags(const float* logits_dev, int rows, uint8_t* row_bad_dev, hipStream_t st);
 hipError_t launch_advance(const TreeDev& d, const int* game_ids_dev, const int* child_slots_dev, int count, hipStream_t st);
 
 hipError_t launch_encode_positions(const m0::Pos* pos_dev, int n, float* planes_f32_dev ,
diff --git a/matrix0_amd/csrc/tree_expand.hip b/matrix0_amd/csrc/tree_expand.hip
--- a/matrix0_amd/csrc/tree_expand.hip
+++ b/matrix0_amd/csrc/tree_expand.hip
@@ -20,11 +20,11 @@
     const float* row;
     const float* legal;
     float* store;
+    bool bad;
 };
-__device__ __forceinline__ LeafLogits logits_of_row(const float* row, float* store) { return LeafLogits{row, nullptr, store}; }
-__device__ __forceinline__ LeafLogits logits_of_cache(const float* payload) { return LeafLogits{nullptr, payload + EC_LOGITS, nullptr}; }
+__device__ __forceinline__ LeafLogits logits_of_row(const float* row, float* store, bool bad) { return LeafLogits{row, nullptr, store, bad}; }
+__device__ __forceinline__ LeafLogits logits_of_cache(const float* payload) { return LeafLogits{nullptr, payload + EC_LOGITS, nullptr, false}; }
 constexpr int CPL = M0_MAX_CHILDREN / 64;
-static_assert(M0_POLICY_SIZE % 4 == 0, "logit rows are read as 16-byte pieces");
 
 static __device__ float np_sum_f32_dev(const float* a, int n) {
     auto block = [&](const float* b, int m) -> float {
@@ -44,21 +44,6 @@
     return block(a, n2) + block(a + n2, n - n2);
 }
 
-__device__ __forceinline__ bool row_nonfinite(const float* lg, int lane) {
-    constexpr int N4 = M0_POLICY_SIZE / 4, PER_LANE = (N4 + 63) / 64;
-    const uint4* lg4 = reinterpret_cast<const uint4*>(lg);
-    uint4 v[PER_LANE];
-#pragma unroll
-    for (int k = 0; k < PER_LANE; ++k) { const int j = lane + 64 * k; v[k] = lg4[j < N4 ? j : N4 - 1]; }
-    uint32_t acc = 0;
-#pragma unroll
-    for (int k = 0; k < PER_LANE; ++k) {
-        acc |= (uint32_t)((v[k].x & 0x7f800000u) == 0x7f800000u) | (uint32_t)((v[k].y & 0x7f800000u) == 0x7f800000u) |
-               (uint32_t)((v[k].z & 0x7f800000u) == 0x7f800000u) | (uint32_t)((v[k].w & 0x7f800000u) == 0x7f800000u);
-    }
-    return acc != 0;
-}
-
 __device__ __forceinline__ void priors_raw(const float* lg, const int (&idx)[CPL], int n, int lane, ExpandScratch* X, float (&pr)[CPL]) {
 #pragma unroll
     for (int k = 0; k < CPL; ++k) { const int i = lane + 64 * k; if (i < n) X->pr[i] = lg[idx[k]]; }
@@ -227,9 +212,7 @@
                                    const LeafLogits& src, bool is_root, bool reg_children) {
     const int lane = E.lane;
     if (n <= 0) return true;
-    bool bad = false;
-    if (!src.legal) bad = row_nonfinite(src.row, lane);
-    bad = __any(bad);
+    const bool bad = src.bad;
     if (lane == 0) E.X->bad = bad ? 1 : 0;
     float pr[CPL];
     int idx[CPL];
@@ -253,7 +236,7 @@
 }
 
 __device__ __forceinline__ void expand_evaluated(const TreeDev& d, const TreeCfg& c, const ExpandEnv& E, int g, const Sample& smp,
-                                                 const uint16_t* moves, const float* lg, float v) {
+                                                 const uint16_t* moves, const float* lg, bool bad, float v) {
     const Arena& A = E.A;
     GameDev* gd = E.gd;
     const int lane = E.lane, kind = smp.kind, leaf = smp.leaf;
@@ -266,7 +249,7 @@
         cw = ec_payload(d.ec, ce);
         ec_invalidate(d.ec, ce, lane);
     }
-    const bool ok = expand_node(E, c, leaf, pos, moves, smp.nlegal, logits_of_row(lg, cw), kind == SK_ROOT_INIT,
+    const bool ok = expand_node(E, c, leaf, pos, moves, smp.nlegal, logits_of_row(lg, cw, bad), kind == SK_ROOT_INIT,
                                 !(kind == SK_ROOT_INIT && gd->root_fresh));
     if (c.eval_cache && kind == SK_EVAL && lane == 0 && A.nch[leaf] < 0) A.cbase[leaf] = -1;
     const int sig = cw ? legal_sig(moves, smp.nlegal, lane) : 0;
@@ -337,7 +320,7 @@
             const int leaf = S[s].leaf, depth = S[s].depth, row = S[s].row;
             const float* lg = d.logits + (size_t)row * M0_POLICY_SIZE;
             const float v = d.values[row];
-            if (A.nch[leaf] < 0) expand_evaluated(d, c, E, g, S[s], moves, lg, v);
+            if (A.nch[leaf] < 0) expand_evaluated(d, c, E, g, S[s], moves, lg, d.row_bad[row] != 0, v);
             ++evals;
             if (kind == SK_EVAL) {
                 backprop(A, path, depth, (double)v, lane, may_repeat, NoMirror{});
@@ -378,3 +361,32 @@
     hipLaunchKernelGGL(expand_kernel, dim3(d.G), dim3(64), 0, st, d, c);
     return hipGetLastError();
 }
+
+static_assert(M0_POLICY_SIZE % 4 == 0, "logit rows are read as 16-byte pieces");
+__device__ __forceinline__ bool row_nonfinite(const float* lg, int lane) {
+    constexpr int N4 = M0_POLICY_SIZE / 4, PER_LANE = (N4 + 63) / 64;
+    const uint4* lg4 = reinterpret_cast<const uint4*>(lg);
+    uint4 v[PER_LANE];
+#pragma unroll
+    for (int k = 0; k < PER_LANE; ++k) { const int j = lane + 64 * k; v[k] = lg4[j < N4 ? j : N4 - 1]; }
+    uint32_t acc = 0;
+#pragma unroll
+    for (int k = 0; k < PER_LANE; ++k) {
+        acc |= (uint32_t)((v[k].x & 0x7f800000u) == 0x7f800000u) | (uint32_t)((v[k].y & 0x7f800000u) == 0x7f800000u) |
+               (uint32_t)((v[k].z & 0x7f800000u) == 0x7f800000u) | (uint32_t)((v[k].w & 0x7f800000u) == 0x7f800000u);
+    }
+    return acc != 0;
+}
+
+__global__ __launch_bounds__(64) void row_flags_kernel(const float* __restrict__ logits, int rows, uint8_t* __restrict__ row_bad) {
+    const int row = blockIdx.x, lane = threadIdx.x;
+    if (row >= rows) return;
+    const bool bad = __any(row_nonfinite(logits + (size_t)row * M0_POLICY_SIZE, lane));
+    if (lane == 0) row_bad[row] = bad ? 1 : 0;
+}
+
+hipError_t launch_row_flags(const float* logits_dev, int rows, uint8_t* row_bad_dev, hipStream_t st) {
+    if (rows <= 0) return hipSuccess;
+    hipLaunchKernelGGL(row_flags_kernel, dim3(rows), dim3(64), 0, st, logits_dev, rows, row_bad_dev);
+    return hipGetLastError();
+}
diff --git a/matrix0_amd/engine.py b/matrix0_amd/engine.py
--- a/matrix0_amd/engine.py
+++ b/matrix0_amd/engine.py
@@ -80,6 +80,7 @@
     L.m0_selfplay_ext_select.argtypes = [C.c_void_p, C.POINTER(c_int), C.c_void_p, c_int]
     L.m0_selfplay_ext_expand.argtypes = [C.c_void_p, C.c_void_p, C.c_void_p, c_int]
     L.m0_selfplay_last_batch_nhwc.argtypes = [C.c_void_p, C.c_void_p, c_int, C.POINTER(c_int)]
+    L.m0_selfplay_last_row_flags.argtypes = [C.c_void_p, C.c_void_p, c_int, C.POINTER(c_int)]
     L.m0_encode_fens_nhwc.argtypes = [c_int, C.POINTER(C.c_char_p), c_int, C.c_void_p]
     L.m0_search_begin.argtypes = [C.c_void_p, c_int, C.c_char_p, c_int, c_int, c_int]
     L.m0_search_select.argtypes = [C.c_void_p, C.POINTER(c_int), C.c_void_p, c_int]
@@ -274,6 +275,14 @@
                    "m0_selfplay_last_batch_nhwc")
         return out[: rows.value]
 
+    def last_row_flags(self) -> np.ndarray:
+        cap = self.cfg.concurrent_games * (self.cfg.inference_batch_size + 1) + 4
+        out = np.zeros((cap,), dtype=np.uint8)
+        rows = c_int(0)
+        _lib.check(self._L.m0_selfplay_last_row_flags(self._h, out.ctypes.data_as(C.c_void_p), cap, C.byref(rows)),
+                   "m0_selfplay_last_row_flags")
+        return out[: rows.value]
+
     def search_begin(self, g: int, fen: str, sims: int, dirichlet: bool, game_uid: int) -> None:
         _lib.check(self._L.m0_search_begin(self._h, g, fen.encode(), sims, int(dirichlet), game_uid), "m0_search_begin")
 
```

Result: no change. 1.131 (median of 6 runs) (+0.1%).
